# athas/raytracers

Hardware: AMD Instinct MI355X
Metric: Mray/s (primary+secondary) on rgbbox & irreg 1000x1000 (higher is better)
Workload: dtype f32

## Files before the change

include/rt_mi355x.h:

```cpp
#ifndef RT_MI355X_H
#define RT_MI355X_H

#include <stdint.h>

#ifdef __cplusplus
extern "C" {
#endif

typedef struct rt_context rt_context;
typedef struct rt_scene rt_scene;
typedef struct rt_prepared rt_prepared;

enum {
  RT_VARIANT_AUTO = 0,
  RT_VARIANT_PIXEL = 1,
  RT_VARIANT_PERSISTENT = 2,
  RT_VARIANT_POOLED = 3
};

int rt_context_create(rt_context **out, int device, void *hip_stream, int use_caller_stream);
int rt_device_count(void);
int rt_context_create_multi(rt_context **out, const int *devices, int ndev);
int rt_context_num_devices(const rt_context *ctx);
const char *rt_context_gather_mode(rt_context *ctx);
int rt_context_rccl_ranks(rt_context *ctx);
void rt_context_destroy(rt_context *ctx);
const char *rt_last_error(const rt_context *ctx);
const char *rt_context_last_launch(const rt_context *ctx);
int rt_context_entry_counts(rt_context *ctx, uint64_t *lists, uint64_t *fallbacks, int64_t *waves, uint64_t *per_wave, int64_t cap_waves);
int rt_context_entry_info(rt_context *ctx, int32_t *colour_lds, int32_t *flags_const, uint64_t *tables_built, uint64_t *tables_kept);
int rt_context_sync(rt_context *ctx);
int rt_context_set_variant(rt_context *ctx, int variant);
int rt_context_set_option(rt_context *ctx, const char *name, int64_t value);
int rt_context_device_info(const rt_context *ctx, int *device, int *num_cu, int *lds_bytes, char *name, int name_len);

int rt_scene_rgbbox(rt_context *ctx, rt_scene **out);
int rt_scene_irreg(rt_context *ctx, rt_scene **out);
int rt_scene_floor(rt_context *ctx, rt_scene **out, int n, float k);
int rt_scene_from_spheres(rt_context *ctx, rt_scene **out, const float *spheres7, int64_t n,
                          const float look_from[3], const float look_at[3], float fov);
int64_t rt_scene_num_spheres(const rt_scene *scene);
int rt_scene_free(rt_context *ctx, rt_scene *scene);

int rt_prepare_scene(rt_context *ctx, rt_prepared **out, int64_t h, int64_t w, const rt_scene *scene);
int rt_prepared_free(rt_context *ctx, rt_prepared *ps);
int64_t rt_prepared_num_spheres(const rt_prepared *ps);
int32_t rt_prepared_height(const rt_prepared *ps);
int rt_prepared_get_bvh(rt_context *ctx, const rt_prepared *ps, float *L7, float *bmin, float *bmax,
                        int32_t *left, int32_t *right, int32_t *parent);
int rt_prepared_get_camera(rt_context *ctx, const rt_prepared *ps, float cam12[12]);

int rt_prepare_scene_device(rt_context *ctx, rt_prepared **out, int64_t h, int64_t w, const float *spheres7_dev, int64_t n,
                            const float look_from[3], const float look_at[3], float fov);
int rt_prepared_update_spheres(rt_context *ctx, rt_prepared *ps, const float *spheres7_dev, int64_t n);

int rt_render(rt_context *ctx, const rt_prepared *ps, int64_t h, int64_t w, int32_t *out_dev);
int rt_render_part(rt_context *ctx, const rt_prepared *ps, int64_t h, int64_t w, int32_t max_depth,
                   int32_t rows_per_tile, int32_t part, int32_t nparts, int32_t *out_dev);
int rt_render_image(rt_context *ctx, const rt_prepared *objs, int64_t width, int64_t height, const float cam12[12],
                    int32_t max_depth, int32_t rows_per_tile, int32_t part, int32_t nparts, int32_t *out_dev);
int rt_render_batch(rt_context *ctx, const rt_prepared *ps, int64_t h, int64_t w, int32_t max_depth, int32_t rows_per_tile,
                    int32_t part, int32_t nparts, int32_t nframes, const float *cams12, int64_t frame_stride, int32_t *out_dev);
int rt_render_part_inplace(rt_context *ctx, const rt_prepared *ps, int64_t h, int64_t w, int32_t max_depth, int32_t rows_per_tile,
                           int32_t part, int32_t nparts, int32_t nframes, const float *cams12, int64_t frame_stride,
                           int32_t *image_dev);
int rt_ipc_export(rt_context *ctx, void *dev, unsigned char handle64[64]);
int rt_ipc_import(rt_context *ctx, const unsigned char handle64[64], void **out_dev);
int rt_ipc_close(rt_context *ctx, void *imported_dev);
int64_t rt_part_rows(int64_t h, int32_t rows_per_tile, int32_t part, int32_t nparts);
int rt_place_part(rt_context *ctx, int64_t h, int64_t w, int32_t rows_per_tile, int32_t part, int32_t nparts,
                  const int32_t *part_dev, int32_t *image_dev);

int rt_place_parts(rt_context *ctx, int64_t h, int64_t w, int32_t rows_per_tile, int32_t nparts, int64_t pad_rows,
                   const int32_t *stacked_dev, int32_t *image_dev);
int rt_place_parts_strided(rt_context *ctx, int64_t h, int64_t w, int32_t rows_per_tile, int32_t nparts,
                           int64_t part_stride, const int32_t *stacked_dev, int32_t *image_dev);

int rt_place_parts_batch(rt_context *ctx, int64_t h, int64_t w, int32_t rows_per_tile, int32_t nparts, int64_t part_stride,
                         int32_t nframes, int64_t frame_stride_in, int64_t frame_stride_out, const int32_t *stacked_dev,
                         int32_t *images_dev);

int rt_render_stats(rt_context *ctx, const rt_prepared *ps, int64_t h, int64_t w, int32_t max_depth,
                    uint64_t stats3[3]);

int rt_render_trace(rt_context *ctx, const rt_prepared *ps, int64_t h, int64_t w, int32_t max_depth,
                    uint64_t *records, int32_t max_waves, int32_t *num_waves);

int rt_render_timed(rt_context *ctx, const rt_prepared *ps, int64_t h, int64_t w, int32_t max_depth,
                    int32_t rows_per_tile, int32_t part, int32_t nparts, int32_t *out_dev,
                    int32_t warmup, int32_t iters, float *ms_out);

int rt_trace_rays(rt_context *ctx, const rt_prepared *ps, int64_t n, const float *rays_dev, int32_t max_depth,
                  float *colour3_dev, int32_t *pixel_dev);
int rt_intersect_rays(rt_context *ctx, const rt_prepared *ps, int64_t n, const float *rays_dev, float t_min, float t_max,
                      int32_t *index_dev, float *hit7_dev);
int rt_occluded_rays(rt_context *ctx, const rt_prepared *ps, int64_t n, const float *rays_dev, float t_min, float t_max,
                     uint8_t *occluded_dev);
int rt_intersect_rays_ranged(rt_context *ctx, const rt_prepared *ps, int64_t n, const float *rays_dev, const float *t_min_dev,
                             const float *t_max_dev, int32_t *index_dev, float *hit7_dev);
int rt_occluded_rays_ranged(rt_context *ctx, const rt_prepared *ps, int64_t n, const float *rays_dev, const float *t_min_dev,
                            const float *t_max_dev, uint8_t *occluded_dev);
int rt_multi_hit_rays(rt_context *ctx, const rt_prepared *ps, int64_t n, const float *rays_dev, float t_min, float t_max,
                      int32_t k, int32_t *count_dev, int32_t *index_dev, uint8_t *root_dev, float *hit7_dev);
int rt_multi_hit_rays_ranged(rt_context *ctx, const rt_prepared *ps, int64_t n, const float *rays_dev,
                             const float *t_min_dev, const float *t_max_dev, int32_t k,
                             int32_t *count_dev, int32_t *index_dev, uint8_t *root_dev, float *hit7_dev);
int rt_sweep_spheres(rt_context *ctx, const rt_prepared *ps, int64_t n, const float *rays_dev, float radius, float t_min, float t_max,
                     int32_t k, int32_t *count_dev, int32_t *index_dev, uint8_t *start_dev, float *hit7_dev);
int rt_sweep_spheres_ranged(rt_context *ctx, const rt_prepared *ps, int64_t n, const float *rays_dev, const float *radius_dev,
                            const float *t_min_dev, const float *t_max_dev, const int32_t *exclude_dev, int32_t k,
                            int32_t *count_dev, int32_t *index_dev, uint8_t *start_dev, float *hit7_dev);
enum { RT_PATH_ESCAPED = 0, RT_PATH_ABSORBED = 1, RT_PATH_TRUNCATED = 2 };
int rt_trace_paths(rt_context *ctx, const rt_prepared *ps, int64_t n, const float *rays_dev, int32_t max_depth, int32_t k,
// ... 55 lines not shown
```

raytracers_amd/_lib.py:

```python
import ctypes as C
import os

HERE = os.path.dirname(os.path.abspath(__file__))
LIB_NAME = "libray_mi355x.so"
LIB_PATH = os.path.join(HERE, LIB_NAME)

RT_SYMBOLS = [
    "rt_context_create", "rt_device_count", "rt_context_create_multi", "rt_context_num_devices", "rt_context_gather_mode", "rt_context_rccl_ranks",
    "rt_context_destroy", "rt_last_error", "rt_context_last_launch", "rt_context_entry_counts", "rt_context_entry_info", "rt_context_sync", "rt_context_set_variant",
    "rt_context_set_option", "rt_context_device_info",
    "rt_scene_rgbbox", "rt_scene_irreg", "rt_scene_floor", "rt_scene_from_spheres", "rt_scene_num_spheres",
    "rt_scene_free",
    "rt_prepare_scene", "rt_prepared_free", "rt_prepared_num_spheres", "rt_prepared_height", "rt_prepared_get_bvh",
    "rt_prepared_get_camera", "rt_prepare_scene_device", "rt_prepared_update_spheres",
    "rt_render", "rt_render_part", "rt_render_image", "rt_render_batch", "rt_render_part_inplace", "rt_ipc_export", "rt_ipc_import", "rt_ipc_close", "rt_part_rows", "rt_place_part", "rt_place_parts", "rt_place_parts_strided", "rt_place_parts_batch", "rt_render_stats", "rt_render_trace",
    "rt_render_timed",
    "rt_trace_rays", "rt_intersect_rays", "rt_occluded_rays", "rt_intersect_rays_ranged", "rt_occluded_rays_ranged",
    "rt_multi_hit_rays", "rt_multi_hit_rays_ranged", "rt_sweep_spheres", "rt_sweep_spheres_ranged", "rt_trace_paths", "rt_trace_paths_shaped", "rt_nearest_spheres", "rt_nearest_spheres_ranged", "rt_prepared_get_sphere_ids",
    "rt_spheres_within_count", "rt_spheres_within_fill", "rt_contact_pairs_count", "rt_contact_pairs_fill", "rt_contact_clusters",
    "rt_spheres_in_boxes_count", "rt_spheres_in_boxes_fill",
    "rt_spheres_in_planes_count", "rt_spheres_in_planes_fill",
    "rt_spheres_along_rays_count", "rt_spheres_along_rays_fill",
    "rt_visible_pairs", "rt_visible_pairs_shaped",
    "rt_camera_rays",
    "rt_device_alloc", "rt_device_free", "rt_copy_to_host", "rt_copy_to_device",
]
FUTHARK_SYMBOLS = [
    "futhark_context_config_new", "futhark_context_config_free", "futhark_context_config_set_debugging",
    "futhark_context_config_set_logging", "futhark_context_config_set_profiling",
    "futhark_context_config_set_device", "futhark_context_config_set_num_threads", "futhark_context_config_set_cache_file",
    "futhark_context_new", "futhark_context_free", "futhark_context_get_error", "futhark_context_sync",
    "futhark_context_report", "futhark_context_clear_caches", "futhark_context_pause_profiling",
    "futhark_context_unpause_profiling",
    "futhark_entry_rgbbox", "futhark_entry_irreg", "futhark_entry_prepare_scene", "futhark_entry_render",
    "futhark_values_i32_2d", "futhark_free_i32_2d", "futhark_shape_i32_2d", "futhark_new_i32_2d", "futhark_values_raw_i32_2d",
    "futhark_free_opaque_prepared_scene", "futhark_free_opaque_scene",
]


def _load():
    try:
        import torch
    except ImportError:
        pass
    if not os.path.exists(LIB_PATH):
        raise ImportError(
            f"{LIB_PATH} is missing: build the HIP library first (`make` at the repo root, or "
            "`python -c 'import __graft_entry__ as g; g.build()'`). raytracers_amd has no CPU fallback.")
    lib = C.CDLL(LIB_PATH, mode=C.RTLD_GLOBAL)
    vp, i32, i64 = C.c_void_p, C.c_int32, C.c_int64
    pf = C.POINTER(C.c_float)
    sig = {
        "rt_context_create": (C.c_int, [C.POINTER(vp), C.c_int, vp, C.c_int]),
        "rt_device_count": (C.c_int, []),
        "rt_context_create_multi": (C.c_int, [C.POINTER(vp), C.POINTER(C.c_int), C.c_int]),
        "rt_context_num_devices": (C.c_int, [vp]),
        "rt_context_gather_mode": (C.c_char_p, [vp]),
        "rt_context_rccl_ranks": (C.c_int, [vp]),
        "rt_context_destroy": (None, [vp]),
        "rt_last_error": (C.c_char_p, [vp]),
        "rt_context_last_launch": (C.c_char_p, [vp]),
        "rt_context_entry_counts": (C.c_int, [vp, C.POINTER(C.c_uint64), C.POINTER(C.c_uint64), C.POINTER(i64), C.POINTER(C.c_uint64), i64]),
        "rt_context_entry_info": (C.c_int, [vp, C.POINTER(i32), C.POINTER(i32), C.POINTER(C.c_uint64), C.POINTER(C.c_uint64)]),
        "rt_context_sync": (C.c_int, [vp]),
        "rt_context_set_variant": (C.c_int, [vp, C.c_int]),
        "rt_context_set_option": (C.c_int, [vp, C.c_char_p, i64]),
        "rt_context_device_info": (C.c_int, [vp, C.POINTER(C.c_int), C.POINTER(C.c_int), C.POINTER(C.c_int),
                                             C.c_char_p, C.c_int]),
        "rt_scene_rgbbox": (C.c_int, [vp, C.POINTER(vp)]),
        "rt_scene_irreg": (C.c_int, [vp, C.POINTER(vp)]),
        "rt_scene_floor": (C.c_int, [vp, C.POINTER(vp), C.c_int, C.c_float]),
        "rt_scene_from_spheres": (C.c_int, [vp, C.POINTER(vp), vp, i64, pf, pf, C.c_float]),
        "rt_scene_num_spheres": (i64, [vp]),
        "rt_scene_free": (C.c_int, [vp, vp]),
        "rt_prepare_scene": (C.c_int, [vp, C.POINTER(vp), i64, i64, vp]),
        "rt_prepared_free": (C.c_int, [vp, vp]),
        "rt_prepared_num_spheres": (i64, [vp]),
        "rt_prepared_height": (i32, [vp]),
        "rt_prepared_get_bvh": (C.c_int, [vp, vp, vp, vp, vp, vp, vp, vp]),
        "rt_prepared_get_camera": (C.c_int, [vp, vp, vp]),
        "rt_prepare_scene_device": (C.c_int, [vp, C.POINTER(vp), i64, i64, vp, i64, pf, pf, C.c_float]),
        "rt_prepared_update_spheres": (C.c_int, [vp, vp, vp, i64]),
        "rt_render": (C.c_int, [vp, vp, i64, i64, vp]),
        "rt_render_part": (C.c_int, [vp, vp, i64, i64, i32, i32, i32, i32, vp]),
        "rt_render_image": (C.c_int, [vp, vp, i64, i64, vp, i32, i32, i32, i32, vp]),
        "rt_render_batch": (C.c_int, [vp, vp, i64, i64, i32, i32, i32, i32, i32, vp, i64, vp]),
        "rt_render_part_inplace": (C.c_int, [vp, vp, i64, i64, i32, i32, i32, i32, i32, vp, i64, vp]),
        "rt_ipc_export": (C.c_int, [vp, vp, vp]),
        "rt_ipc_import": (C.c_int, [vp, vp, C.POINTER(vp)]),
        "rt_ipc_close": (C.c_int, [vp, vp]),
        "rt_part_rows": (i64, [i64, i32, i32, i32]),
        "rt_place_part": (C.c_int, [vp, i64, i64, i32, i32, i32, vp, vp]),
        "rt_place_parts": (C.c_int, [vp, i64, i64, i32, i32, i64, vp, vp]),
        "rt_place_parts_strided": (C.c_int, [vp, i64, i64, i32, i32, i64, vp, vp]),
        "rt_place_parts_batch": (C.c_int, [vp, i64, i64, i32, i32, i64, i32, i64, i64, vp, vp]),
        "rt_render_stats": (C.c_int, [vp, vp, i64, i64, i32, vp]),
        "rt_render_trace": (C.c_int, [vp, vp, i64, i64, i32, vp, i32, C.POINTER(i32)]),
        "rt_render_timed": (C.c_int, [vp, vp, i64, i64, i32, i32, i32, i32, vp, i32, i32, vp]),
        "rt_device_alloc": (C.c_int, [vp, C.POINTER(vp), i64]),
        "rt_device_free": (C.c_int, [vp, vp]),
        "rt_copy_to_host": (C.c_int, [vp, vp, vp, i64]),
        "rt_copy_to_device": (C.c_int, [vp, vp, vp, i64]),
        "rt_trace_rays": (C.c_int, [vp, vp, i64, vp, i32, vp, vp]),
        "rt_intersect_rays": (C.c_int, [vp, vp, i64, vp, C.c_float, C.c_float, vp, vp]),
        "rt_occluded_rays": (C.c_int, [vp, vp, i64, vp, C.c_float, C.c_float, vp]),
        "rt_intersect_rays_ranged": (C.c_int, [vp, vp, i64, vp, vp, vp, vp, vp]),
        "rt_occluded_rays_ranged": (C.c_int, [vp, vp, i64, vp, vp, vp, vp]),
        "rt_multi_hit_rays": (C.c_int, [vp, vp, i64, vp, C.c_float, C.c_float, i32, vp, vp, vp, vp]),
        "rt_multi_hit_rays_ranged": (C.c_int, [vp, vp, i64, vp, vp, vp, i32, vp, vp, vp, vp]),
        "rt_sweep_spheres": (C.c_int, [vp, vp, i64, vp, C.c_float, C.c_float, C.c_float, i32, vp, vp, vp, vp]),
        "rt_sweep_spheres_ranged": (C.c_int, [vp, vp, i64, vp, vp, vp, vp, vp, i32, vp, vp, vp, vp]),
        "rt_trace_paths": (C.c_int, [vp, vp, i64, vp, i32, i32, vp, vp, vp, vp, vp, vp, vp]),
        "rt_trace_paths_shaped": (C.c_int, [vp, vp, i64, vp, i32, i32, vp, vp, vp, vp, vp, vp, vp, i32]),
        "rt_nearest_spheres": (C.c_int, [vp, vp, i64, vp, C.c_float, i32, vp, vp, vp]),
        "rt_nearest_spheres_ranged": (C.c_int, [vp, vp, i64, vp, vp, i32, vp, vp, vp]),
        "rt_prepared_get_sphere_ids": (C.c_int, [vp, vp, vp]),
        "rt_spheres_within_count": (C.c_int, [vp, vp, i64, vp, C.c_float, vp, vp, vp]),
        "rt_spheres_within_fill": (C.c_int, [vp, vp, i64, vp, C.c_float, vp, vp, vp, i64, vp, vp, vp]),
        "rt_contact_pairs_count": (C.c_int, [vp, vp, C.c_float, vp]),
        "rt_contact_pairs_fill": (C.c_int, [vp, vp, C.c_float, vp, i64, vp, vp]),
        "rt_contact_clusters": (C.c_int, [vp, vp, C.c_float, vp, vp, vp, vp]),
        "rt_spheres_in_boxes_count": (C.c_int, [vp, vp, i64, vp, C.c_float, vp, vp, vp]),
        "rt_spheres_in_boxes_fill": (C.c_int, [vp, vp, i64, vp, C.c_float, vp, vp, vp, i64, vp, vp, vp]),
        "rt_spheres_in_planes_count": (C.c_int, [vp, vp, i64, vp, C.c_int32, C.c_float, vp, vp, vp]),
        "rt_spheres_in_planes_fill": (C.c_int, [vp, vp, i64, vp, C.c_int32, C.c_float, vp, vp, vp, i64, vp, vp, vp]),
        "rt_spheres_along_rays_count": (C.c_int, [vp, vp, i64, vp, C.c_float, vp, C.c_float, C.c_float, vp, vp, vp, vp, vp]),
        "rt_spheres_along_rays_fill": (C.c_int, [vp, vp, i64, vp, C.c_float, vp, C.c_float, C.c_float, vp, vp, vp, vp, vp, i64, vp, vp, vp, vp]),
        "rt_visible_pairs": (C.c_int, [vp, vp, i64, vp, i64, vp, i32, C.c_float, C.c_float, vp, vp]),
        "rt_visible_pairs_shaped": (C.c_int, [vp, vp, i64, vp, i64, vp, i32, C.c_float, C.c_float, vp, vp, i32]),
        "rt_camera_rays": (C.c_int, [vp, vp, i64, i64, vp, vp]),
    }
    for name, (res, args) in sig.items():
        fn = getattr(lib, name)
        fn.restype = res
        fn.argtypes = args
    return lib


lib = _load()
```

raytracers_amd/api.py:

```python
import ctypes as C

import numpy as np

from ._lib import lib

VARIANT_AUTO, VARIANT_PIXEL, VARIANT_PERSISTENT, VARIANT_POOLED = 0, 1, 2, 3
MAX_DEPTH = 50
PATH_ESCAPED, PATH_ABSORBED, PATH_TRUNCATED = 0, 1, 2
PAIRS_TARGETS, PAIRS_DIRECTIONS = 0, 1
ROWS_PER_TILE = 8


class RtError(RuntimeError):
    pass


class Context:

    def __init__(self, device=-1, stream=None, devices=None):
        h = C.c_void_p()
        if devices is not None:
            arr = (C.c_int * len(devices))(*[int(d) for d in devices])
            rc = lib.rt_context_create_multi(C.byref(h), arr, len(devices))
        else:
            rc = lib.rt_context_create(C.byref(h), int(device), C.c_void_p(stream or 0), 0 if stream is None else 1)
        if rc != 0 or not h.value:
            raise RtError(f"rt_context_create failed (code {rc}): no usable HIP device; "
                          "raytracers_amd has no CPU fallback")
        self._h = h

    def _check(self, rc):
        if rc != 0:
            raise RtError(lib.rt_last_error(self._h).decode() or f"error code {rc}")

    def close(self):
        if getattr(self, "_h", None):
            lib.rt_context_destroy(self._h)
            self._h = None

    def __del__(self):
        try:
            self.close()
        except Exception:
            pass

    def sync(self):
        self._check(lib.rt_context_sync(self._h))

    @property
    def num_devices(self):
        return int(lib.rt_context_num_devices(self._h))

    @property
    def gather_mode(self):
        return lib.rt_context_gather_mode(self._h).decode()

    @property
    def last_launch(self):
        return lib.rt_context_last_launch(self._h).decode()

    def entry_counts(self):
        lists, falls, nw = C.c_uint64(), C.c_uint64(), C.c_int64()
        self._check(lib.rt_context_entry_counts(self._h, C.byref(lists), C.byref(falls), C.byref(nw), None, 0))
        per = np.zeros((nw.value, 2), np.uint64)
        if nw.value:
            self._check(lib.rt_context_entry_counts(self._h, None, None, None, per.ctypes.data_as(C.POINTER(C.c_uint64)), nw.value))
        return {"lists": lists.value, "fallbacks": falls.value, "waves": nw.value, "per_wave": per}

    def entry_info(self):
        col, const, built, kept = C.c_int32(), C.c_int32(), C.c_uint64(), C.c_uint64()
        self._check(lib.rt_context_entry_info(self._h, C.byref(col), C.byref(const), C.byref(built), C.byref(kept)))
        return {"colour_lds": bool(col.value), "flags_const": bool(const.value), "tables_built": built.value, "tables_kept": kept.value}

    @property
    def rccl_ranks(self):
        return int(lib.rt_context_rccl_ranks(self._h))

    def set_variant(self, v):
        self._check(lib.rt_context_set_variant(self._h, int(v)))

    def set_option(self, name, value):
        self._check(lib.rt_context_set_option(self._h, name.encode(), int(value)))

    def device_info(self):
        dev, cus, lds = C.c_int(), C.c_int(), C.c_int()
        name = C.create_string_buffer(64)
        self._check(lib.rt_context_device_info(self._h, C.byref(dev), C.byref(cus), C.byref(lds), name, 64))
        return {"device": dev.value, "num_cu": cus.value, "lds_bytes": lds.value, "arch": name.value.decode()}

    def _scene(self, fn, *args):
        h = C.c_void_p()
        self._check(fn(self._h, C.byref(h), *args))
        return Scene(self, h)

    def rgbbox(self):
        return self._scene(lib.rt_scene_rgbbox)

    def irreg(self):
        return self._scene(lib.rt_scene_irreg)

    def floor(self, n, k):
        return self._scene(lib.rt_scene_floor, int(n), float(k))

    def scene(self, name):
        if name == "rgbbox":
            return self.rgbbox()
        if name == "irreg":
            return self.irreg()
        if name == "big":
            return self.floor(1000, 6000.0)
        raise ValueError(f"unknown scene {name!r}")

    def scene_from_spheres(self, spheres7, look_from, look_at, fov):
        s = np.ascontiguousarray(spheres7, dtype=np.float32)
        if s.ndim != 2 or s.shape[1] != 7:
            raise ValueError("spheres7 must be (n, 7): pos.xyz, colour.rgb, radius")
        lf = (C.c_float * 3)(*look_from)
        la = (C.c_float * 3)(*look_at)
        h = C.c_void_p()
        self._check(lib.rt_scene_from_spheres(self._h, C.byref(h), s.ctypes.data, s.shape[0], lf, la, float(fov)))
        return Scene(self, h)

    def alloc_i32(self, count):
        return DeviceBuffer(self, int(count) * 4)


class DeviceBuffer:
    def __init__(self, ctx, nbytes):
        self.ctx, self.nbytes = ctx, nbytes
        p = C.c_void_p()
        ctx._check(lib.rt_device_alloc(ctx._h, C.byref(p), nbytes))
        self.ptr = p.value

    def as_torch(self, shape):
        import torch
        n = int(np.prod(shape))
        assert n * 4 <= self.nbytes
        iface = {"shape": tuple(int(x) for x in shape), "typestr": "<i4", "data": (int(self.ptr), False), "version": 2}
        holder = type("_CudaArray", (), {"__cuda_array_interface__": iface})()
        return torch.as_tensor(holder, device=torch.device("cuda", self.ctx.device_info()["device"]))

    def to_host(self, shape, dtype=np.int32):
        out = np.empty(shape, dtype=dtype)
        assert out.nbytes <= self.nbytes
        self.ctx._check(lib.rt_copy_to_host(self.ctx._h, out.ctypes.data, self.ptr, out.nbytes))
        return out

    def free(self):
        if self.ptr and self.ctx._h:
            lib.rt_device_free(self.ctx._h, self.ptr)
        self.ptr = None

    def __del__(self):
        try:
            self.free()
# ... 846 lines not shown
```

raytracers_amd/csrc/api.cpp:

```cpp
#include <hip/hip_runtime.h>

#include <algorithm>
#include <chrono>
#include <cmath>
#include <cstdio>
#include <cstdlib>
#include <cstring>
#include <memory>
#include <string>
#include <vector>

#include "../../include/rt_mi355x.h"
#include "rt_device.hpp"
#include "rt_host.hpp"
#include "rt_internal.hpp"

namespace rti {
int fail(rt_context *ctx, const std::string &msg) {
  if (ctx) ctx->err = msg;
  return 1;
}
int hip_fail(rt_context *ctx, hipError_t e, const char *what) {
  return fail(ctx, std::string(what) + ": " + hipGetErrorString(e));
}
// ... 367 lines not shown
    v->sort_inflight_px = false;
  }
  return true;
}
void drain_streams(rt_context *ctx) {
  (void)hipStreamSynchronize(ctx->stream);
  if (ctx->sort_stream) (void)hipStreamSynchronize(ctx->sort_stream);
  if (ctx->sort_stream_px) (void)hipStreamSynchronize(ctx->sort_stream_px);
}

int ensure_spill(rt_context *ctx, int stride) {
  const size_t need = sizeof(unsigned) * static_cast<size_t>(stride) * static_cast<size_t>(std::max(1, ctx->num_cu)) * 20;
  if (ctx->spill_bytes >= need) return 0;
  drain_streams(ctx);
  if (ctx->spill_dev) (void)hipFree(ctx->spill_dev);
  ctx->spill_dev = nullptr; ctx->spill_bytes = 0;
  RT_HIP(ctx, hipMalloc(reinterpret_cast<void **>(&ctx->spill_dev), need));
  ctx->spill_bytes = need;
  return 0;
}

bool rt_scene_exceeds_l2(const rt_prepared *ps) { return static_cast<int64_t>(ps->n) * 80 > (int64_t(32) << 20); }

void set_cull(const rt_context *ctx, const rt_prepared *ps, const Plan &pl, const float *cams_dev, rtk::KParams *p) {
  if (ctx->cull == 0 || !ps->cull.ok || pl.variant != RT_VARIANT_POOLED || (pl.waves != 16 && pl.waves != 4)) return;
  if (ctx->cull < 0 && pl.lds_nodes == p->n_nodes && pl.lds_sph == p->n_sph) return;
  if (cams_dev == nullptr ? !rt::cull_origin_ok(ps->cull, &p->cam.ox) : (cams_dev != ctx->cams_dev || ctx->cams_host == nullptr)) return;
  for (int f = 0; cams_dev != nullptr && f < p->nframes; ++f)
    if (!rt::cull_origin_ok(ps->cull, ctx->cams_host + 12 * f)) return;
  p->cull = 1;
  p->cull_c2 = ps->cull.c2;
  p->cull_kappa = ps->cull.kappa;
}

void set_dark(const rt_context *ctx, bool instrumented, rtk::KParams *p) {
  p->dark = (ctx->dark_stop != 0 && p->cost == nullptr && (!instrumented || ctx->dark_stop > 0)) ? 1 : 0;
}

void set_leaf_box(const rt_context *ctx, const rt_prepared *ps, const Plan &pl, const float *cams_dev, bool instrumented, rtk::KParams *p) {
  p->leaf_box = 0;
  if (ctx->leaf_box == 0 || !ps->leaf.ok || pl.variant != RT_VARIANT_POOLED || (instrumented && ctx->leaf_box <= 0)) return;
  if (pl.lds_nodes != p->n_nodes || pl.lds_sph != p->n_sph) return;
  if (cams_dev == nullptr ? !rt::leaf_box_camera_ok(ps->leaf, &p->cam.ox) : (cams_dev != ctx->cams_dev || ctx->cams_host == nullptr)) return;
  for (int f = 0; cams_dev != nullptr && f < p->nframes; ++f)
    if (!rt::leaf_box_camera_ok(ps->leaf, ctx->cams_host + 12 * f)) return;
  rtk::PooledKey k{};
  if (!rtk::choose_pooled(*p, instrumented, pl.waves, 0, &k) || !rtk::pooled_leaf_box(k)) return;
  p->leaf_box = 1;
}

int set_entry(rt_context *ctx, const Plan &pl, TileOrder *to, rtk::KParams *p, int *entry, bool *build) {
  p->entry = nullptr;
  *entry = 0;
  *build = false;
  rtk::PooledKey k{};
  if (ctx->entry_lists == 0 || pl.variant != RT_VARIANT_POOLED || p->n_nodes < 1 || !rtk::choose_pooled(*p, false, pl.waves, 0, &k) || !rtk::pooled_entry_ok(k)) return 0;
  if (ctx->entry_lists < 0 && p->nparts > 1 && p->rpt_log2 < 3) return 0;
  if (ctx->entry_lists < 0 && (ctx->leaf_box == 0 || ctx->dark_stop == 0)) return 0;
  if (p->cams != nullptr && (p->order != nullptr || !(p->nshards == 1 || p->interleave))) return 0;
  *entry = rtk::pooled_entry_bits(rtk::kEntryLists, p->leaf_box, p->dark, rtk::pooled_col_lds_bytes(p->n_nodes, p->n_sph, p->capb, p->capl, p->ray_planes),
                                  static_cast<size_t>(std::min(ctx->lds_bytes, 160 * 1024)), ctx->col_lds != 0);
  const int filter = p->leaf_box != 0 && rtk::pooled_leaf_box(k) ? 1 : 0;
  if (to != nullptr && to->entry != nullptr && p->cams == nullptr && ctx->entry_keep != 0 && (to->entry_ctx == nullptr || to->entry_ctx == ctx)) {
    *build = !(to->entry_valid && to->entry_filter == filter);
    to->entry_valid = false;
    to->entry_filter = filter;
    to->entry_ctx = ctx;
    p->entry = to->entry;
    return 0;
  }
  *build = true;
  const size_t need = sizeof(unsigned) * rtk::kEntryDw * static_cast<size_t>(p->cams != nullptr ? p->nframes : 1) * static_cast<size_t>(p->nchunks);
  if (ctx->entry_bytes < need) {
    drain_streams(ctx);
    pool_free(ctx, reinterpret_cast<char *>(ctx->entry_dev), ctx->entry_bytes);
    ctx->entry_dev = nullptr; ctx->entry_bytes = 0;
    char *blk = nullptr;
    size_t bytes = need;
    RT_HIP(ctx, pool_alloc(ctx, &blk, &bytes));
    ctx->entry_dev = reinterpret_cast<unsigned *>(blk);
    ctx->entry_bytes = bytes;
  }
  p->entry = ctx->entry_dev;
  return 0;
}

std::string pooled_launch_name(const rtk::KParams &p, int waves, int rays = 0) {
  rtk::PooledKey k{};
  return rtk::choose_pooled(p, false, waves, rays, &k) ? rtk::pooled_name(k) : "none";
}
const char *pooled_launch_nodes(const rtk::KParams &p, int waves) {
  rtk::PooledKey k{};
  return rtk::choose_pooled(p, false, waves, 0, &k) && rtk::pooled_presort(k) ? "sign-ordered" : "planes";
}

void frame_params(const rt_prepared *ps, int64_t h, int64_t w, int rows_per_tile, int part, int nparts, int max_depth, const float *cam12, rtk::KParams *p) {
  scene_params(ps, p);
  std::memcpy(&p->cam, cam12 ? static_cast<const void *>(cam12) : static_cast<const void *>(&ps->cam), sizeof(p->cam));
  p->w = static_cast<int>(w); p->h = static_cast<int>(h);
  p->rows_local = static_cast<int>(rt::part_rows(h, rows_per_tile, part, nparts));
  p->rows_per_tile = rows_per_tile; p->part = part; p->nparts = nparts;
  p->rpt_log2 = (rows_per_tile & (rows_per_tile - 1)) == 0 ? __builtin_ctz(rows_per_tile) : -1;
  p->tiles_x = (p->w + 7) / 8;
  p->tiles_y = (p->rows_local + 7) / 8;
  p->max_depth = max_depth;
  p->nframes = 1;
}

bool twenty_waves(const rt_context *ctx, const Plan &pl) { return pl.waves * (pl.grid_full / std::max(1, ctx->num_cu)) == 20; }

int pooled_shape_params(rt_context *ctx, const rt_prepared *ps, const Plan &pl, rtk::KParams *p) {
  p->static_first = ctx->static_first;
  p->lds_nodes = pl.lds_nodes; p->lds_sph = pl.lds_sph;
  p->smax = pl.smax; p->lmax = pl.lmax;
  p->thr_shade = ctx->thr_shade; p->thr_leaf = ctx->thr_leaf;
  p->capb = pl.capb; p->capl = pl.capl; p->ray_planes = pl.ray_planes;
  if (pl.spill_stride > 0) {
    if (int rc = ensure_spill(ctx, pl.spill_stride)) return rc;
    p->spill = ctx->spill_dev;
    p->spill_stride = pl.spill_stride;
  }
  p->prio_depth = ctx->prio_depth;
  p->box2 = ctx->box2;
  p->look_max = ctx->look_max > 0 ? ctx->look_max : (twenty_waves(ctx, pl) ? 16 : (p->nframes > 1 || p->nchunks > 16384) ? 32 : 64);
  p->tl_log2 = ps->tl_depth;
  return 0;
}

int xcd_rule(const rt_context *ctx, const rt_prepared *ps, const Plan &pl, int nframes) {
  if (ctx->xcd_queues >= 0) return ctx->xcd_queues;
  return nframes == 1 && pl.variant == RT_VARIANT_POOLED && twenty_waves(ctx, pl) && rt_scene_exceeds_l2(ps) ? 1 : 2;
}
void set_counters(rtk::KParams *p, int xq, int grid) {
  p->nshards = xq && (p->nframes == 1 || xq == 2) && grid % rtk::kMaxShards == 0 ? rtk::kMaxShards : 1;
  p->interleave = p->nshards > 1 && xq == 2;
}
int order_shards(const rtk::KParams &p) { return p.interleave ? 1 : p.nshards; }
bool counters_follow(rtk::KParams *p, int xq, int grid) {
  const int ns = p->nshards, il = p->interleave, shards = order_shards(*p);
  set_counters(p, xq, grid);
  if (order_shards(*p) == shards) return true;
  p->nshards = ns;
  p->interleave = il;
  return false;
}

bool px_static_ok(const rt_context *ctx, const rtk::KParams &p, const Plan &pl) {
  return ctx->pixel_order == 2 ||
         (ctx->pixel_order == 1 && ctx->deep_class < 0 && p.max_depth > 4 && pl.waves == 16 && ctx->adaptive_order == 1 && p.nchunks <= ctx->px_max_tiles &&
          (p.nchunks >= 1024 || (pl.lds_nodes == p.n_nodes && pl.lds_sph == p.n_sph)));
}
bool px_list_launch(const rt_context *ctx, const rtk::KParams &p, const Plan &pl, const TileOrder *v) {
  return v && v->valid && v->px_valid && p.nframes == 1 && pl.waves == 16 && ctx->adaptive_order == 1 && (p.nshards == 1 || p.interleave) &&
         v->px_elems >= static_cast<size_t>(p.rows_local) * p.w && px_static_ok(ctx, p, pl);
}

bool same_shape(const TileOrder &o, const rtk::KParams &p) {
  return o.h == p.h && o.w == p.w && o.rows_per_tile == p.rows_per_tile && o.part == p.part && o.nparts == p.nparts && o.max_depth == p.max_depth &&
         o.ntiles == p.nchunks && o.nshards == order_shards(p);
}

int find_view(rt_context *ctx, const rt_prepared *ps, const rtk::KParams &p, const Plan &pl, TileOrder **out) {
  TileOrder *to = nullptr;
  for (auto &o : ps->orders)
    if (same_shape(o, p) && std::memcmp(o.cam, &p.cam, sizeof o.cam) == 0) to = &o;
  if (!to) {
// ... 221 lines not shown
  bool stream_was_idle = ctx->synced_since_render;
  ctx->synced_since_render = false;
  if (!stream_was_idle && ctx->eager_sort && nframes == 1) {
    stream_was_idle = hipStreamQuery(ctx->stream) == hipSuccess;
    (void)hipGetLastError();
  }
  rtk::KParams p{};
  frame_params(ps, h, w, rows_per_tile, part, nparts, max_depth, cam12, &p);
  p.out = out_dev;
  p.stats = ctx->stats_dev;
  if (p.rows_local == 0) {
    ctx->last_launch = "family=none (no rows)";
    return 0;
  }
  const int64_t frame_elems = inplace ? h * w : static_cast<int64_t>(p.rows_local) * p.w;
  if (nframes < 1 || (nframes > 1 && (frame_stride < frame_elems || frame_stride * nframes >= (int64_t(1) << 31))))
    return fail(ctx, "bad batch: nframes >= 1, frame_stride >= rows * w (in place: h * w), nframes * frame_stride < 2^31");
  if (rti::tiles_of(p.rows_local, w) * nframes >= rti::kMaxPositions)
    return fail(ctx, "bad batch: tiles per frame x frames < 2^26 (a frame has ceil(rows / 8) x ceil(w / 8) tiles of 8 x 8 pixels)");
  if (inplace) {
    p.out = out_dev + static_cast<int64_t>(part) * rows_per_tile * w;
    p.out_skip = static_cast<int>(static_cast<int64_t>(nparts - 1) * rows_per_tile * w);
  }
  if (max_depth == 0) return clear_frames(ctx, p, out_dev, nframes, frame_stride, inplace);
  Ticks tick;
  Plan pl{};
  if (stats) pl.variant = RT_VARIANT_PIXEL;
  else {
    const int64_t ntiles1 = static_cast<int64_t>((w + 7) / 8) * ((p.rows_local + 7) / 8);
    const bool huge = rt_scene_exceeds_l2(ps);
    const bool wide = ctx->wide_waves == 2 || (ctx->wide_waves == 1 && ntiles1 * nframes >= (huge ? 40000 : 100000) && (nframes > 1 || ntiles1 > ctx->px_max_tiles));
    if (int rc = make_plan(ctx, ps, &pl, ntiles1 * nframes, 0, wide)) return rc;
  }
  tick("plan");
  if (nframes > 1 && pl.variant != RT_VARIANT_POOLED) {
    std::vector<float> hc;
    if (cams_dev) {
      hc.resize(static_cast<size_t>(nframes) * 12);
      RT_HIP(ctx, hipMemcpyAsync(hc.data(), cams_dev, hc.size() * 4, hipMemcpyDeviceToHost, ctx->stream));
      RT_HIP(ctx, hipStreamSynchronize(ctx->stream));
    }
    for (int f = 0; f < nframes; ++f)
      if (int rc = enqueue_render(ctx, ps, h, w, max_depth, rows_per_tile, part, nparts, out_dev + f * frame_stride, stats,
                                  cams_dev ? hc.data() + 12 * f : cam12, 1, 0, nullptr, inplace))
        return rc;
    return 0;
  }
  if (pl.variant == RT_VARIANT_PIXEL) {
    RT_HIP(ctx, rtk::launch_pixel(p, stats, ctx->stream));
    ctx->last_launch = stats ? "family=pixel (instrumented)" : "family=pixel";
    return 0;
  }
  p.nframes = nframes;
  p.frame_stride = static_cast<int>(frame_stride);
  p.cams = reinterpret_cast<const rtk::Cam *>(cams_dev);
  p.queue = ctx->queue_dev;
  p.nchunks = p.tiles_x * p.tiles_y;
  const int64_t tiles_per_wave = static_cast<int64_t>(p.nchunks) * nframes / std::max(1, pl.grid * pl.waves);
  p.tpt_log2 = ctx->tpt_log2 >= 0 ? ctx->tpt_log2 : (nframes > 1 ? (tiles_per_wave >= 48 && !twenty_waves(ctx, pl) ? 2 : tiles_per_wave >= 24 ? 1 : 0) : 0);
  const int xq = xcd_rule(ctx, ps, pl, nframes);
  set_counters(&p, pl.variant == RT_VARIANT_POOLED ? xq : 0, pl.grid);
  if (int rc = pooled_shape_params(ctx, ps, pl, &p)) return rc;
  p.solo = ctx->solo;
  if (pl.variant != RT_VARIANT_POOLED) {
    RT_HIP(ctx, rtk::launch_persistent(p, false, pl.grid, pl.waves, ctx->stream));
    ctx->last_launch = "family=persistent";
    return 0;
  }
  if (ps->n >= (int64_t(1) << 22)) return fail(ctx, "pooled kernel: at most 2^22 spheres (work items and hit keys carry the leaf index in 22 bits)");
  if (p.rpt_log2 < 0) return fail(ctx, "pooled kernel: rows_per_tile must be a power of two");
  if (int rc = get_uv(ctx, w, h, &p.u_tab, &p.v_tab)) return rc;
  tick("uv tables");
  TileOrder *to = nullptr;
  if (ctx->adaptive_order && !p.cams)
    if (int rc = find_view(ctx, ps, p, pl, &to)) return rc;
  Tickets t;
  if (int rc = choose_tickets(ctx, ps, to, xq, tick, p, pl, &t)) return rc;
  set_cull(ctx, ps, pl, cams_dev, &p);
  set_dark(ctx, false, &p);
  set_leaf_box(ctx, ps, pl, cams_dev, false, &p);
  int entry = 0;
  bool build_entry = false;
  if (int rc = set_entry(ctx, pl, to, &p, &entry, &build_entry)) return rc;
  if (p.entry) {
    if (build_entry) {
      RT_HIP(ctx, rtk::launch_tile_entry(p, false, pl.waves, ctx->stream));
      ctx->entry_tables_built++;
    } else {
      ctx->entry_tables_kept++;
    }
    if (to != nullptr && p.entry == to->entry) to->entry_valid = true;
    if (ctx->entry_count) {
      const size_t nw = static_cast<size_t>(pl.grid) * static_cast<size_t>(pl.waves), bytes = nw * 2 * sizeof(unsigned long long);
      if (ctx->entry_counts_bytes < bytes) {
        drain_streams(ctx);
        if (ctx->entry_counts_dev) (void)hipFree(ctx->entry_counts_dev);
        ctx->entry_counts_dev = nullptr; ctx->entry_counts_bytes = 0;
        RT_HIP(ctx, hipMalloc(reinterpret_cast<void **>(&ctx->entry_counts_dev), bytes));
        ctx->entry_counts_bytes = bytes;
      }
      RT_HIP(ctx, hipMemsetAsync(ctx->entry_counts_dev, 0, bytes, ctx->stream));
      p.trace = ctx->entry_counts_dev;
      entry = (entry & ~rtk::kEntryModeMask) | rtk::kEntryCount;
    }
  }
  ctx->entry_counts_waves = (entry & rtk::kEntryModeMask) == rtk::kEntryCount ? static_cast<int64_t>(pl.grid) * pl.waves : 0;
  ctx->last_entry = entry;
  tick("before launch");
  RT_HIP(ctx, rtk::launch_pooled(p, false, pl.grid, pl.waves, ctx->stream, 0, entry));
  tick("launch_pooled");
  char buf[352];
  std::snprintf(buf, sizeof buf, "family=pooled tickets=%s%s instantiation=%s frames=%d tiles=%d grid=%d waves=%d counters=%d%s deep_class=%d deep_split=%d recording=%d nodes=%s,entry=%s,dark=%d,leaf_box=%d",
                p.px_hdr ? "pixel-list" : t.first_order ? "tiles-bit-reversed" : (p.order ? "tiles-ordered" : "tiles-raster"), t.borrowed ? "(borrowed)" : "",
                pooled_launch_name(p, pl.waves).c_str(), p.nframes, p.nchunks, pl.grid, pl.waves, p.nshards, p.interleave ? "(turns)" : "", p.px_hdr ? 0 : p.deep_class,
                p.px_hdr ? 0 : p.deep_split, p.cost ? (p.cost_px ? 2 : 1) : 0, pooled_launch_nodes(p, pl.waves), p.entry ? "lists" : "root", p.dark, p.leaf_box);
  ctx->last_launch = buf;
  if (to && p.cost) {
    to->sort_pending = true;
    to->sort_px = p.cost_px != nullptr;
    to->rec_out_skip = p.out_skip;
    if (ctx->eager_sort && (stream_was_idle || ctx->sync_policy))
      if (int rc = sort_view(ctx, ps, to, p, pl)) return rc;
    tick("record: eager sorts");
  }
  return 0;
}
using rti::enqueue_render;

extern "C" void rt_context_destroy(rt_context *ctx);

extern "C" int rt_context_create(rt_context **out, int device, void *hip_stream, int use_caller_stream) {
  if (!out) return 1;
  *out = nullptr;
  auto ctx = std::make_unique<rt_context>();
  int count = 0;
  hipError_t e = hipGetDeviceCount(&count);
  if (e != hipSuccess || count <= 0) {
    std::fprintf(stderr, "libray_mi355x: no usable HIP device (%s); this library has no CPU path\n",
                 e == hipSuccess ? "device count is 0" : hipGetErrorString(e));
    return 2;
  }
  if (device < 0) {
    if (hipGetDevice(&device) != hipSuccess) device = 0;
  }
  if (device >= count) return 3;
  if (hipSetDevice(device) != hipSuccess) return 4;
  ctx->device = device;
  hipDeviceProp_t prop;
  if (hipGetDeviceProperties(&prop, device) != hipSuccess) return 5;
  auto bail = [&](int code) {
    rt_context_destroy(ctx.release());
    return code;
  };
  ctx->num_cu = prop.multiProcessorCount;
  ctx->lds_bytes = static_cast<int>(prop.maxSharedMemoryPerMultiProcessor ? prop.maxSharedMemoryPerMultiProcessor
                                                                           : prop.sharedMemPerBlock);
  ctx->name = prop.gcnArchName;
  if (use_caller_stream) {
    ctx->stream = static_cast<hipStream_t>(hip_stream);
  } else {
    if (hipStreamCreateWithFlags(&ctx->stream, hipStreamNonBlocking) != hipSuccess) return bail(6);
    ctx->own_stream = true;
  }
  if (hipMalloc(reinterpret_cast<void **>(&ctx->queue_dev), sizeof(unsigned) * rtk::kQueueDwords) != hipSuccess) return bail(7);
  if (hipMemset(ctx->queue_dev, 0, sizeof(unsigned) * rtk::kQueueDwords) != hipSuccess) return bail(7);
  if (hipMalloc(reinterpret_cast<void **>(&ctx->stats_dev), 256) != hipSuccess) return bail(7);
  if (hipMemset(ctx->stats_dev, 0, 256) != hipSuccess) return bail(7);
  if (hipStreamSynchronize(nullptr) != hipSuccess) return bail(7);
  if (hipMalloc(reinterpret_cast<void **>(&ctx->arena), kArenaGranules * kGranule) != hipSuccess) return bail(7);
  ctx->arena_used.assign(kArenaGranules, 0);
  if (hipHostMalloc(reinterpret_cast<void **>(&ctx->pinned), rtk::gpu_build_pinned_bytes(), hipHostMallocDefault) != hipSuccess)
    return bail(7);
  if (hipHostMalloc(reinterpret_cast<void **>(&ctx->stage), kStageBytes, hipHostMallocDefault) != hipSuccess) return bail(7);
  if (hipStreamCreateWithFlags(&ctx->sort_stream, hipStreamNonBlocking) != hipSuccess) return bail(6);
  if (hipStreamCreateWithFlags(&ctx->sort_stream_px, hipStreamNonBlocking) != hipSuccess) return bail(6);
  if (hipEventCreateWithFlags(&ctx->rec_event, hipEventDisableTiming) != hipSuccess) return bail(6);
  if (hipMalloc(reinterpret_cast<void **>(&ctx->order_scratch), sizeof(int) * rtk::kOrderScratchInts) != hipSuccess) return bail(7);
  if (hipMalloc(reinterpret_cast<void **>(&ctx->px_scratch), sizeof(int) * rtk::px_scratch_ints()) != hipSuccess) return bail(7);
  if (hipHostMalloc(reinterpret_cast<void **>(&ctx->class_slab), sizeof(int) * kClassSlotInts * kClassSlots * kClassChunks, hipHostMallocDefault) != hipSuccess) return bail(7);
  rtk::warm_render_kernels();
  rtk::warm_build_kernels();
  if (rtk::warm_scratch(ctx->stream, ctx->order_scratch) != hipSuccess) return bail(6);
  if (const char *v = std::getenv("RT_VARIANT")) ctx->variant = std::atoi(v);
  if (const char *v = std::getenv("RT_XCD_QUEUES")) ctx->xcd_queues = std::max(-1, std::min(2, std::atoi(v)));
  if (const char *v = std::getenv("RT_TPT_LOG2")) ctx->tpt_log2 = std::max(-1, std::min(4, std::atoi(v)));
  if (const char *v = std::getenv("RT_STATIC_FIRST")) ctx->static_first = std::atoi(v) != 0;
  *out = ctx.release();
  return 0;
}

extern "C" void rt_context_destroy(rt_context *ctx) {
  if (!ctx) return;
  if (ctx->group) rti::group_destroy(ctx);
  (void)hipSetDevice(ctx->device);
  drain_streams(ctx);
  if (ctx->sort_stream) (void)hipStreamDestroy(ctx->sort_stream);
  if (ctx->sort_stream_px) (void)hipStreamDestroy(ctx->sort_stream_px);
  if (ctx->rec_event) (void)hipEventDestroy(ctx->rec_event);
  for (auto &t : ctx->uv) pool_free(ctx, reinterpret_cast<char *>(t.u), t.bytes);
  for (auto &t : ctx->first_orders) pool_free(ctx, reinterpret_cast<char *>(t.order), t.bytes);
  if (ctx->class_slab) (void)hipHostFree(ctx->class_slab);
  if (ctx->cams_dev) (void)hipFree(ctx->cams_dev);
  if (ctx->cams_host) (void)hipHostFree(ctx->cams_host);
  if (ctx->cams_event) (void)hipEventDestroy(ctx->cams_event);
  if (ctx->queue_dev) (void)hipFree(ctx->queue_dev);
  if (ctx->spill_dev) (void)hipFree(ctx->spill_dev);
  pool_free(ctx, reinterpret_cast<char *>(ctx->entry_dev), ctx->entry_bytes);
  if (ctx->entry_counts_dev) (void)hipFree(ctx->entry_counts_dev);
  if (ctx->order_scratch) (void)hipFree(ctx->order_scratch);
  if (ctx->px_scratch) (void)hipFree(ctx->px_scratch);
  if (ctx->within_scratch) (void)hipFree(ctx->within_scratch);
  if (ctx->stats_dev) (void)hipFree(ctx->stats_dev);
  for (auto &b : ctx->pool) (void)hipFree(b.p);
  if (ctx->arena) (void)hipFree(ctx->arena);
  if (ctx->pinned) (void)hipHostFree(ctx->pinned);
  if (ctx->stage) (void)hipHostFree(ctx->stage);
  if (ctx->own_stream) (void)hipStreamDestroy(ctx->stream);
  delete ctx;
}

extern "C" int rt_device_count(void) {
  int n = 0;
  return hipGetDeviceCount(&n) == hipSuccess ? n : 0;
}

extern "C" const char *rt_last_error(const rt_context *ctx) { return ctx ? ctx->err.c_str() : "null context"; }
extern "C" int rt_context_entry_counts(rt_context *ctx, uint64_t *lists, uint64_t *fallbacks, int64_t *waves, uint64_t *per_wave, int64_t cap_waves) {
  if (!ctx) return 1;
  RT_LOCK(ctx);
  RT_HIP(ctx, hipSetDevice(ctx->device));
  RT_HIP(ctx, hipStreamSynchronize(ctx->stream));
  const int64_t nw = ctx->entry_counts_waves;
  std::vector<unsigned long long> h(static_cast<size_t>(nw) * 2);
  if (nw > 0) RT_HIP(ctx, hipMemcpy(h.data(), ctx->entry_counts_dev, h.size() * sizeof(unsigned long long), hipMemcpyDeviceToHost));
  uint64_t l = 0, f = 0;
  for (int64_t i = 0; i < nw; ++i) {
    l += h[2 * i]; f += h[2 * i + 1];
    if (per_wave && i < cap_waves) { per_wave[2 * i] = h[2 * i]; per_wave[2 * i + 1] = h[2 * i + 1]; }
  }
  if (lists) *lists = l;
  if (fallbacks) *fallbacks = f;
  if (waves) *waves = nw;
  return 0;
}

extern "C" int rt_context_entry_info(rt_context *ctx, int32_t *colour_lds, int32_t *flags_const, uint64_t *tables_built, uint64_t *tables_kept) {
  if (!ctx) return 1;
  RT_LOCK(ctx);
  if (colour_lds) *colour_lds = (ctx->last_entry & rtk::kEntryColLds) != 0;
  if (flags_const) *flags_const = ctx->last_entry != 0 && (ctx->last_entry & rtk::kEntryRtFlags) == 0;
  if (tables_built) *tables_built = ctx->entry_tables_built;
  if (tables_kept) *tables_kept = ctx->entry_tables_kept;
  return 0;
}

extern "C" const char *rt_context_last_launch(const rt_context *ctx) { return ctx ? ctx->last_launch.c_str() : ""; }

extern "C" int rt_context_sync(rt_context *ctx) {
  RT_LOCK(ctx);
  if (!ctx) return 1;
  if (ctx->group) {
    const int grc = rti::group_sync(ctx);
    if (!grc) rti::group_mark_synced(ctx);
    return grc;
  }
  const auto t0 = std::chrono::steady_clock::now();
  hipError_t q;
  for (;;) {
    q = hipStreamQuery(ctx->stream);
    if (q != hipErrorNotReady) break;
    if (std::chrono::steady_clock::now() - t0 > std::chrono::microseconds(800)) {
      q = hipStreamSynchronize(ctx->stream);
      break;
    }
  }
  if (q == hipSuccess) {
    ctx->synced_since_render = true;
    return 0;
  }
  (void)hipGetLastError();
  (void)hipMemset(ctx->queue_dev, 0, sizeof(unsigned) * rtk::kQueueDwords);
  return hip_fail(ctx, q, "stream synchronisation (the ticket counters were reset)");
}

extern "C" int rt_context_set_variant(rt_context *ctx, int variant) {
  RT_LOCK(ctx);
  if (!ctx) return 1;
  if (variant < RT_VARIANT_AUTO || variant > RT_VARIANT_POOLED) return fail(ctx, "unknown variant");
  ctx->variant = variant;
  if (ctx->group) return rti::group_set_variant(ctx, variant);
  return 0;
}

extern "C" int rt_context_set_option(rt_context *ctx, const char *name, int64_t value) {
  RT_LOCK(ctx);
  if (!ctx || !name) return 1;
  if (ctx->group) {
    const int grc = rti::group_set_option(ctx, name, value);
    if (grc >= 0) return grc;
  }
  const std::string k(name);
  const int v = static_cast<int>(value);
  if (k == "waves_per_wg") {
    if (v != 0 && v != 4 && v != 8 && v != 12 && v != 16) return fail(ctx, "waves_per_wg must be 0 (auto), 4, 8, 12 or 16");
    ctx->waves_per_wg = v;
  } else if (k == "wgs_per_cu") {
    if (v < 1 || v > 8) return fail(ctx, "wgs_per_cu must be 1..8");
    ctx->wgs_per_cu = v;
  } else if (k == "thr_shade") {
    ctx->thr_shade = std::max(1, std::min(64, v));
  } else if (k == "thr_leaf") {
    ctx->thr_leaf = std::max(1, std::min(64, v));
  } else if (k == "lmax") {
    if (v < 2 || v > 32) return fail(ctx, "lmax must be 2..32");
    ctx->lmax = v;
  } else if (k == "lds_scene_bytes") {
    ctx->lds_scene_bytes = v;
  } else if (k == "lds_sph_first") {
    ctx->lds_sph_first = v != 0;
  } else if (k == "grid_div") {
    ctx->grid_div = std::max(0, std::min(64, v));
  } else if (k == "prio_depth") {
    ctx->prio_depth = std::max(0, v);
  } else if (k == "gpu_build") {
    ctx->gpu_build = v != 0;
  } else if (k == "adaptive_order") {
    ctx->adaptive_order = v;
  } else if (k == "box2") {
    ctx->box2 = v != 0;
  } else if (k == "look_max") {
    ctx->look_max = std::max(0, std::min(64, v));
  } else if (k == "handover") {
    ctx->handover = std::max(0, std::min(2, v));
  } else if (k == "donate_max") {
    ctx->donate_max = std::max(1, std::min(64, v));
  } else if (k == "solo") {
    ctx->solo = v != 0;
  } else if (k == "treelet") {
    if (v < 1 || v > rtk::kTreeletMaxDepth) return fail(ctx, "treelet (host builder: levels per treelet) must be 1 .. 5");
    ctx->treelet = v;
  } else if (k == "trace_part") {
    ctx->trace_part = v;
  } else if (k == "trace_nparts") {
    ctx->trace_nparts = v;
  } else if (k == "trace_solo") {
    ctx->trace_solo = v != 0;
  } else if (k == "ray_planes") {
    if (v != 0 && v != 2 && v != 3) return fail(ctx, "ray_planes must be 0 (auto), 2 or 3");
    ctx->ray_planes = v;
  } else if (k == "deep_class") {
    ctx->deep_class = std::min(8, std::max(-1, v));
  } else if (k == "deep_cap_log2") {
    ctx->deep_cap_log2 = std::min(8, std::max(0, v));
  } else if (k == "deep_split") {
    ctx->deep_split = std::min(6, std::max(0, v));
  } else if (k == "xcd_queues") {
    if (v < -1 || v > 2) return fail(ctx, "xcd_queues must be -1 (auto), 0 (one counter), 1 (a strip of tile columns per counter) or 2 (counters take turns)");
    ctx->xcd_queues = v;
  } else if (k == "tpt_log2") {
    if (v < -1 || v > 4) return fail(ctx, "tpt_log2 must be -1 (auto) or 0..4");
    ctx->tpt_log2 = v;
  } else if (k == "static_first") {
    ctx->static_first = v != 0;
  } else if (k == "first_order") {
    ctx->first_order = v != 0;
  } else if (k == "pixel_order") {
    ctx->pixel_order = std::max(0, std::min(2, v));
  } else if (k == "px_solo" || k == "px_w8" || k == "px_w16" || k == "px_w32") {
    ctx->px_thr[k == "px_solo" ? 0 : k == "px_w8" ? 1 : k == "px_w16" ? 2 : 3] = std::max(0, std::min(255, v));
  } else if (k == "px_g1" || k == "px_g8" || k == "px_g16" || k == "px_g32" || k == "px_g64") {
    ctx->px_g[k == "px_g1" ? 0 : k == "px_g8" ? 1 : k == "px_g16" ? 2 : k == "px_g32" ? 3 : 4] = std::max(0, std::min(100000, v));
  } else if (k == "px_max_tiles") {
    ctx->px_max_tiles = std::max(0, v);
  } else if (k == "px_ray_ns") {
    ctx->px_ray_ns = std::max(0, std::min(100000, v));
  } else if (k == "px_zip") {
    ctx->px_zip = v != 0;
  } else if (k == "px_prio") {
    ctx->px_prio = std::max(0, std::min(3, v));
  } else if (k == "px_hold") {
    ctx->px_hold = v & 0x1f;
  } else if (k == "px_solo_div") {
    ctx->px_solo_div = std::max(1, std::min(4096, v));
  } else if (k == "eager_sort") {
    drain_streams(ctx);
    ctx->eager_sort = v != 0;
  } else if (k == "borrow") {
    ctx->borrow = std::max(0, std::min(4, v));
  } else if (k == "stack_cap") {
    if (v != 0 && v != rtk::kSpillCapbTest) return fail(ctx, "stack_cap must be 0 or 192");
    ctx->stack_cap = v;
  } else if (k == "wide_waves") {
    ctx->wide_waves = std::max(0, std::min(2, v));
  } else if (k == "cull") {
    ctx->cull = std::max(-1, std::min(1, v));
  } else if (k == "dark_stop") {
    ctx->dark_stop = std::max(-1, std::min(1, v));
  } else if (k == "leaf_box") {
    ctx->leaf_box = std::max(-1, std::min(1, v));
  } else if (k == "entry_lists") {
    ctx->entry_lists = std::max(-1, std::min(1, v));
  } else if (k == "entry_count") {
    ctx->entry_count = v != 0;
  } else if (k == "entry_keep") {
    ctx->entry_keep = v == 0 ? 0 : -1;
  } else if (k == "col_lds") {
    ctx->col_lds = v == 0 ? 0 : -1;
  } else if (k == "sync_policy") {
    ctx->sync_policy = v != 0;
  } else {
    return fail(ctx, "unknown option: " + k);
  }
  return 0;
}

extern "C" int rt_context_device_info(const rt_context *ctx, int *device, int *num_cu, int *lds_bytes, char *name,
                                      int name_len) {
  RT_LOCK(const_cast<rt_context *>(ctx));
  if (!ctx) return 1;
  if (device) *device = ctx->device;
  if (num_cu) *num_cu = ctx->num_cu;
  if (lds_bytes) *lds_bytes = ctx->lds_bytes;
  if (name && name_len > 0) {
    std::strncpy(name, ctx->name.c_str(), static_cast<size_t>(name_len) - 1);
    name[name_len - 1] = 0;
  }
  return 0;
}

static int new_scene(rt_context *ctx, rt_scene **out, rt::SceneDesc &&d) {
  RT_LOCK(ctx);
  if (!ctx || !out) return fail(ctx, "null argument");
  auto *s = new rt_scene;
  s->desc = std::move(d);
  *out = s;
  return 0;
}
extern "C" int rt_scene_rgbbox(rt_context *ctx, rt_scene **out) { return new_scene(ctx, out, rt::make_rgbbox()); }
extern "C" int rt_scene_irreg(rt_context *ctx, rt_scene **out) { return new_scene(ctx, out, rt::make_floor(100, 600.0f)); }
extern "C" int rt_scene_floor(rt_context *ctx, rt_scene **out, int n, float k) {
  RT_LOCK(ctx);
  if (n < 2 || n > 4096) return fail(ctx, "floor scene: n out of range (2..4096)");
  return new_scene(ctx, out, rt::make_floor(n, k));
}
extern "C" int rt_scene_from_spheres(rt_context *ctx, rt_scene **out, const float *spheres7, int64_t n,
                                     const float look_from[3], const float look_at[3], float fov) {
  RT_LOCK(ctx);
  if (!spheres7 || !look_from || !look_at) return fail(ctx, "null argument");
  if (n < 2 || n > (int64_t(1) << rtk::kMaxSpheresLog2)) return fail(ctx, "scene needs 2 .. 2^26 spheres");
  rt::SceneDesc d;
  d.spheres.resize(static_cast<size_t>(n));
  std::memcpy(d.spheres.data(), spheres7, sizeof(rt::Sphere) * static_cast<size_t>(n));
  std::copy(look_from, look_from + 3, d.look_from);
  std::copy(look_at, look_at + 3, d.look_at);
  d.fov = fov;
  return new_scene(ctx, out, std::move(d));
}
extern "C" int64_t rt_scene_num_spheres(const rt_scene *scene) {
  return scene ? static_cast<int64_t>(scene->desc.spheres.size()) : 0;
}
extern "C" int rt_scene_free(rt_context *ctx, rt_scene *scene) {
  RT_LOCK(ctx);
  if (scene)
    for (auto &c : scene->copies) {
      (void)hipSetDevice(c.device);
      (void)hipFree(c.p);
    }
  if (ctx) (void)hipSetDevice(ctx->device);
  delete scene;
  return 0;
}

namespace {
hipError_t alloc_prepared_block(rt_context *ctx, rt_prepared *ps) {
  const size_t n = static_cast<size_t>(ps->n), ni = n - 1;
  size_t off = 0;
  auto carve = [&](size_t bytes) { const size_t at = off; off += (bytes + 255) & ~size_t(255); return at; };
  const size_t o_L7 = carve(n * 28), o_bmin = carve(ni * 12), o_bmax = carve(ni * 12), o_left = carve(ni * 4),
               o_right = carve(ni * 4), o_parent = carve(ni * 4), o_nodes = carve(ni * 32), o_nodes64 = carve(ni * 64),
               o_sph = carve(n * 16), o_col = carve(n * 16), o_ids = carve(n * 4);
  ps->block_bytes = off;
  const hipError_t e = pool_alloc(ctx, &ps->block, &ps->block_bytes);
  if (e != hipSuccess) {
    ps->block = nullptr;
// ... 190 lines not shown
    if (ps->leaf.ok) {
      *e = rtk::launch_leaf_boxes(ps->nodes64, ps->sph, static_cast<int>(n) - 1, ps->leaf.q, ps->leaf.lin, ps->leaf.abs, ctx->stream);
      if (*e == hipSuccess) *e = hipStreamSynchronize(ctx->stream);
      if (*e != hipSuccess) return 0;
    }
  } else {
    std::vector<rt::Sphere> host(n);
    *e = hipMemcpyAsync(host.data(), spheres7_dev, n * sizeof(rt::Sphere), hipMemcpyDeviceToHost, ctx->stream);
    if (*e == hipSuccess) *e = hipStreamSynchronize(ctx->stream);
    if (*e != hipSuccess) return 0;
    const rt::CullStats st = rt::cull_stats(host.data(), n);
    ps->leaf = rt::leaf_box_finish(st, n);
    if (int rc = host_build_upload(ctx, ps, host, e)) return rc;
    if (*e != hipSuccess) return 0;
    ps->cull = rt::cull_finish(st, n, 0);
  }
  ps->cull.ok = ps->cull.ok && ps->height <= static_cast<int>(log2f(static_cast<float>(n))) + 2;
  if (ctx->wide_waves != 0 && ps->height > 15 && n < (size_t(1) << 22)) return ensure_spill(ctx, 64 * (ps->height + 2));
  return 0;
}

int device_spheres_ok(rt_context *ctx, const float *spheres7_dev, int64_t n) {
  if (!spheres7_dev) return fail(ctx, "null argument");
  if (n < 2 || n > (int64_t(1) << rtk::kMaxSpheresLog2)) return fail(ctx, "scene needs 2 .. 2^26 spheres");
  if (ctx->group) return fail(ctx, "device spheres: a multi-device context is not supported (use a context on one device)");
  return 0;
}

void reset_views(rt_context *ctx, rt_prepared *ps) {
  drain_streams(ctx);
  for (auto &o : ps->orders) {
    for (hipEvent_t ev : {o.sort_event, o.sort_event_px, o.classes_event})
      if (ev) (void)hipEventSynchronize(ev);
    if (o.block) {
      if (o.block_owner == ctx) pool_free(ctx, o.block, o.block_bytes);
      else if (!o.block_owner) (void)hipFree(o.block);
      o.block = nullptr;
    }
    for (hipEvent_t ev : {o.sort_event, o.sort_event_px, o.classes_event})
      if (ev) (void)hipEventDestroy(ev);
  }
  ps->orders.clear();
}
}

extern "C" int rt_prepare_scene_device(rt_context *ctx, rt_prepared **out, int64_t h, int64_t w, const float *spheres7_dev, int64_t n,
                                       const float look_from[3], const float look_at[3], float fov) {
  RT_LOCK(ctx);
  if (!ctx || !out || !look_from || !look_at) return fail(ctx, "null argument");
  if (int rc = device_spheres_ok(ctx, spheres7_dev, n)) return rc;
  if (h <= 0 || w <= 0) return fail(ctx, "image size must be positive");
  RT_HIP(ctx, hipSetDevice(ctx->device));
  (void)hipGetLastError();
  auto ps = std::make_unique<rt_prepared>();
  ps->n = n;
  ps->home = ctx;
  ps->h = h; ps->w = w;
  rt::SceneDesc d;
  std::copy(look_from, look_from + 3, d.look_from);
  std::copy(look_at, look_at + 3, d.look_at);
  d.fov = fov;
  ps->cam = rt::scene_camera(d, h, w);
  RT_HIP(ctx, alloc_prepared_block(ctx, ps.get()));
  hipError_t e = hipSuccess;
  const int rc = build_from_device(ctx, ps.get(), spheres7_dev, &e);
  if (rc || e != hipSuccess) {
    rt_prepared_free(ctx, ps.release());
    return rc ? rc : hip_fail(ctx, e, "rt_prepare_scene_device");
  }
  *out = ps.release();
  return 0;
}

extern "C" int rt_prepared_update_spheres(rt_context *ctx, rt_prepared *ps, const float *spheres7_dev, int64_t n) {
  RT_LOCK(ctx);
  if (!ctx || !ps) return fail(ctx, "null argument");
  if (int rc = device_spheres_ok(ctx, spheres7_dev, n)) return rc;
  if (ps->home != ctx) return fail(ctx, "rt_prepared_update_spheres: only through the context that prepared the scene");
  if (n != ps->n) return fail(ctx, "rt_prepared_update_spheres: n must equal rt_prepared_num_spheres (" + std::to_string(ps->n) + ")");
  RT_LOCK_PS(ps);
  RT_HIP(ctx, hipSetDevice(ctx->device));
  (void)hipGetLastError();
  reset_views(ctx, ps);
  hipError_t e = hipSuccess;
  if (int rc = build_from_device(ctx, ps, spheres7_dev, &e)) return rc;
  if (e != hipSuccess) return hip_fail(ctx, e, "rt_prepared_update_spheres");
  return 0;
}

extern "C" int64_t rt_prepared_num_spheres(const rt_prepared *ps) { return ps ? ps->n : 0; }
extern "C" int32_t rt_prepared_height(const rt_prepared *ps) { return ps ? ps->height : 0; }

extern "C" int rt_prepared_get_bvh(rt_context *ctx, const rt_prepared *ps, float *L7, float *bmin, float *bmax,
                                   int32_t *left, int32_t *right, int32_t *parent) {
  RT_LOCK(ctx);
  if (!ctx || !ps) return fail(ctx, "null argument");
  RT_HIP(ctx, hipSetDevice(ctx->device));
  RT_HIP(ctx, hipStreamSynchronize(ctx->stream));
  const size_t n = static_cast<size_t>(ps->n), ni = n - 1;
  if (L7) RT_HIP(ctx, hipMemcpy(L7, ps->L7, n * 28, hipMemcpyDeviceToHost));
  if (bmin) RT_HIP(ctx, hipMemcpy(bmin, ps->bmin, ni * 12, hipMemcpyDeviceToHost));
  if (bmax) RT_HIP(ctx, hipMemcpy(bmax, ps->bmax, ni * 12, hipMemcpyDeviceToHost));
  if (left) RT_HIP(ctx, hipMemcpy(left, ps->left, ni * 4, hipMemcpyDeviceToHost));
  if (right) RT_HIP(ctx, hipMemcpy(right, ps->right, ni * 4, hipMemcpyDeviceToHost));
  if (parent) RT_HIP(ctx, hipMemcpy(parent, ps->parent, ni * 4, hipMemcpyDeviceToHost));
  return 0;
}

extern "C" int rt_prepared_get_camera(rt_context *ctx, const rt_prepared *ps, float cam12[12]) {
  RT_LOCK(ctx);
  if (!ctx || !ps || !cam12) return fail(ctx, "null argument");
  std::memcpy(cam12, &ps->cam, sizeof(rt::Camera));
  return 0;
}

static int render_entry(rt_context *ctx, const rt_prepared *ps, int64_t h, int64_t w, int32_t max_depth, int32_t rows_per_tile,
                        int32_t part, int32_t nparts, int32_t *out_dev, const float *cam12) {
  RT_LOCK(ctx);
  if (ctx && ctx->group) {
    if (!ps) return fail(ctx, "null prepared scene");
    if (part != 0 || nparts != 1) return fail(ctx, "a multi-device context renders whole frames: it partitions them itself");
    if (max_depth < 0) return fail(ctx, "negative max_depth");
    return rti::group_render(ctx, ps, h, w, max_depth, out_dev, cam12);
  }
  return enqueue_render(ctx, ps, h, w, max_depth, rows_per_tile, part, nparts, out_dev, false, cam12);
}

extern "C" int rt_render(rt_context *ctx, const rt_prepared *ps, int64_t h, int64_t w, int32_t *out_dev) {
  return render_entry(ctx, ps, h, w, 50, 8, 0, 1, out_dev, nullptr);
}

extern "C" int rt_render_part(rt_context *ctx, const rt_prepared *ps, int64_t h, int64_t w, int32_t max_depth,
                              int32_t rows_per_tile, int32_t part, int32_t nparts, int32_t *out_dev) {
  return render_entry(ctx, ps, h, w, max_depth, rows_per_tile, part, nparts, out_dev, nullptr);
}

extern "C" int rt_render_image(rt_context *ctx, const rt_prepared *objs, int64_t width, int64_t height, const float cam12[12],
                               int32_t max_depth, int32_t rows_per_tile, int32_t part, int32_t nparts, int32_t *out_dev) {
  return render_entry(ctx, objs, height, width, max_depth, rows_per_tile, part, nparts, out_dev, cam12);
}

int rti::stage_cams(rt_context *ctx, const float *cams12, int32_t nframes, const float **cams_dev) {
  RT_LOCK(ctx);
  *cams_dev = nullptr;
  if (!cams12) return 0;
  RT_HIP(ctx, hipSetDevice(ctx->device));
  const size_t bytes = sizeof(float) * 12 * static_cast<size_t>(nframes);
  if (bytes > ctx->cams_bytes) {
    RT_HIP(ctx, hipStreamSynchronize(ctx->stream));
    if (ctx->cams_dev) (void)hipFree(ctx->cams_dev);
    if (ctx->cams_host) (void)hipHostFree(ctx->cams_host);
    ctx->cams_dev = nullptr;
    ctx->cams_host = nullptr;
    ctx->cams_bytes = 0;
    ctx->cams_event_valid = false;
    RT_HIP(ctx, hipMalloc(reinterpret_cast<void **>(&ctx->cams_dev), bytes));
    RT_HIP(ctx, hipHostMalloc(reinterpret_cast<void **>(&ctx->cams_host), bytes, hipHostMallocDefault));
    ctx->cams_bytes = bytes;
  } else if (ctx->cams_event_valid) {
    RT_HIP(ctx, hipEventSynchronize(ctx->cams_event));
  }
  std::memcpy(ctx->cams_host, cams12, bytes);
  RT_HIP(ctx, hipMemcpyAsync(ctx->cams_dev, ctx->cams_host, bytes, hipMemcpyHostToDevice, ctx->stream));
  if (!ctx->cams_event) RT_HIP(ctx, hipEventCreateWithFlags(&ctx->cams_event, hipEventDisableTiming));
  RT_HIP(ctx, hipEventRecord(ctx->cams_event, ctx->stream));
  ctx->cams_event_valid = true;
// ... 276 lines not shown
```

raytracers_amd/csrc/lane_core.h:

```cpp
#pragma once
#include <math.h>
#include <stdint.h>

#if defined(__HIPCC__)
#define RT_HD __host__ __device__ __forceinline__
#else
#define RT_HD inline
#endif

namespace rtk {

constexpr float kTMax = 1000000000.0f;
constexpr float kEps = 0.1f;
constexpr float kNoHit = __builtin_inff();

struct Cam {
  float ox, oy, oz, lx, ly, lz, hx, hy, hz, vx, vy, vz;
};

struct Ray {
  float ox, oy, oz;
  float dx, dy, dz;
  float ix, iy, iz;
  float a;
// ... 263 lines not shown
      const float d = k == 0 ? q[j].dx : k == 1 ? q[j].dy : q[j].dz;
      const float i = 1.0f / d;
      pos = pos & (d > 0.0f) & (i > 0.0f) & (i < kNoHit);
      neg = neg & (d < 0.0f) & (i < 0.0f) & (i > -kNoHit);
      lo = j == 0 || i < lo ? i : lo;
      hi = j == 0 || i > hi ? i : hi;
    }
    if (MUT != 3) ok = ok & (pos | neg);
    t->imin[k] = lo; t->imax[k] = hi;
  }
  return ok;
}

template <int MUT = 0>
RT_HD int tile_verdict(const TileRays &t, const float lo[3], const float hi[3]) {
  float tmin_lo = 0.0f, tmin_hi = 0.0f, tmax_lo = kTMax, tmax_hi = kTMax;
  for (int k = 0; k < 3; ++k) {
    const bool neg = t.imax[k] < 0.0f;
    const float cn = (neg ? hi[k] : lo[k]) - t.o[k], cf = (neg ? lo[k] : hi[k]) - t.o[k];
    const float na = cn * t.imin[k], nb = cn * t.imax[k], fa = cf * t.imin[k], fb = cf * t.imax[k];
    tmin_lo = fmaxf(na < nb ? na : nb, tmin_lo);
    tmin_hi = fmaxf(na < nb ? nb : na, tmin_hi);
    tmax_lo = fminf(fa < fb ? fa : fb, tmax_lo);
    tmax_hi = fminf(fa < fb ? fb : fa, tmax_hi);
  }
  if (tmax_lo > tmin_hi) return kTileAllHit;
  if (MUT == 1 ? tmax_hi < tmin_lo : tmax_hi <= tmin_lo) return kTileAllMiss;
  return kTileMixed;
}

template <int MUT, int MAXI, int MAXL>
RT_HD bool tile_frontier(const TileRays &t, const float root_lo[3], const float root_hi[3], const float *nodes64, int n_nodes, bool filter,
                         int *inner, int *n_inner, int *leaf, int *n_leaf) {
  *n_inner = 0; *n_leaf = 0;
  if (n_nodes < 1 || tile_verdict<MUT>(t, root_lo, root_hi) != kTileAllHit) return false;
  int stack[kEntryStack], sp = 0, ni = 0, nl = 0;
  stack[sp++] = 0;
  while (sp > 0) {
    const int node = stack[--sp];
    const float *const rec = nodes64 + 16 * (size_t)node;
    int child[2], verdict[2];
    bool uniform = true;
    for (int s = 0; s < 2; ++s) {
      int32_t w;
      __builtin_memcpy(&w, rec + 4 * s + 3, 4);
      child[s] = w >> 8;
      verdict[s] = tile_verdict<MUT>(t, rec + 8 * s, rec + 8 * s + 4);
      if (child[s] < 0 && !filter) verdict[s] = kTileAllHit;
      uniform = uniform & (verdict[s] != kTileMixed);
    }
    if (!uniform) {
      if (node == 0 || ni >= MAXI) return false;
      inner[ni++] = node;
      continue;
    }
    for (int s = 0; s < 2; ++s) {
      if (verdict[s] != kTileAllHit) continue;
      if (child[s] < 0) {
        if (nl >= MAXL) return false;
        leaf[nl++] = ~child[s];
      } else {
        if (sp >= kEntryStack) return false;
        stack[sp++] = child[s];
      }
    }
  }
  *n_inner = ni; *n_leaf = nl;
  return true;
}

template <int MUT = 0>
RT_HD void tile_entry(const TileRays &t, bool rays_ok, const float root_lo[3], const float root_hi[3], const float *nodes64, int n_nodes, bool filter,
                      int ref_shift, int node_mul, uint32_t out[kEntryDw]) {
  int inner[1], leaf[kEntryLeaves], ni = 0, nl = 0;
  const bool ok = rays_ok && tile_frontier<MUT, 1, kEntryLeaves>(t, root_lo, root_hi, nodes64, n_nodes, filter, inner, &ni, leaf, &nl);
  for (int i = 0; i < kEntryDw; ++i) out[i] = 0u;
  if (!ok) return;
  out[0] = kEntryValid | (ni ? kEntryInner : 0u) | (uint32_t)nl << kEntryCountShift;
  if (ni) out[1] = (uint32_t)(inner[0] * node_mul) << ref_shift;
  for (int i = 0; i < kEntryLeaves; ++i)
    if (i < nl) out[2 + i] = (uint32_t)~leaf[i] << ref_shift;
}

}
```

raytracers_amd/csrc/render_kernels.hip:

```cpp
#include <hip/hip_runtime.h>

#include <mutex>
#include <type_traits>
#include <utility>

#include "lane_core.h"
#include "rt_device.hpp"
#include "treelet.h"

#ifdef RT_ISA_MARKS
#define RT_MARK(name) asm volatile("; RT_MARK " name)
#else
#define RT_MARK(name)
#endif

namespace rtk {

__device__ __forceinline__ int global_row(const KParams &p, int lrow) {
  const int k = lrow / p.rows_per_tile;
  return (k * p.nparts + p.part) * p.rows_per_tile + (lrow - k * p.rows_per_tile);
}

__device__ __forceinline__ size_t out_index(const KParams &p, int lrow, int col) {
  return (size_t)lrow * p.w + col + (size_t)(lrow / p.rows_per_tile) * (size_t)p.out_skip;
// ... 381 lines not shown
            q3 = buf_load16(rs_nodes, ni16 * 4 + 48);
          }
          const int cl8 = f2i(q0.w), cr8 = f2i(q1.w);
          const unsigned ml = (unsigned)f2i(q2.w), mr = (unsigned)f2i(q3.w);
          const float limc = CULL ? cull_limit(__uint_as_float(lds_load4(key_lds + 4u)), w2, cull_kappa) : kTMax;
          const unsigned long long m_hl = bal(box_hit_clamped(r, q0.x, q0.y, q0.z, q1.x, q1.y, q1.z, limc));
          const unsigned long long m_hr = bal(box_hit_clamped(r, q2.x, q2.y, q2.z, q3.x, q3.y, q3.z, limc));
          const bool reach = has && tl_reached(ml, mr, pos, (unsigned)(m_hl >> gsh), (unsigned)(m_hr >> gsh));
          const unsigned long long m_reach = bal(reach), m_exit = m_reach & bal(tl_frontier(ml));
          const unsigned long long m_ln = bal(cl8 < 0), m_rn = bal(cr8 < 0);
          const unsigned long long m_inl = m_exit & ~m_ln & m_hl, m_inr = m_exit & ~m_rn & m_hr;
          const unsigned long long m_lfl = m_reach & m_ln, m_lfr = m_reach & m_rn;
          const int c_inl = __popcll(m_inl), c_lfl = __popcll(m_lfl);
          const int b_box = (int)box_lds + 4 * nbox, b_leaf = (int)leaf_lds + 4 * nleaf, dump = (int)dump_lds;
          const int a_l = sel_mask(m_lfl, sel_mask(m_inl, dump, b_box + 4 * lane_rank(m_inl)), b_leaf + 4 * lane_rank(m_lfl));
          const int a_r = sel_mask(m_lfr, sel_mask(m_inr, dump, b_box + 4 * lane_rank_from(m_inr, c_inl)),
                                   b_leaf + 4 * lane_rank_from(m_lfr, c_lfl));
          lds_store(a_l, (unsigned)cl8);
          lds_store(a_r, (unsigned)cr8);
          nbox = uni(nbox + c_inl + __popcll(m_inr));
          nleaf = uni(nleaf + c_lfl + __popcll(m_lfr));
          if (TRACE) { __builtin_amdgcn_s_waitcnt(0); tc_tre += clock64() - tc_op; tn_tre++; }
        }
      }
      __builtin_amdgcn_fence(__ATOMIC_ACQ_REL, "wavefront");
      key = *key_ptr;
    }
    const float best = __uint_as_float((unsigned)(key >> 32));
    const bool hit = key != kKeyInit;
    const int wj = hit ? (int)((unsigned)key >> 1) : 0;
    float4 c, s;
    const unsigned long long m_win = bal(hit && cand_j == wj);
    if (m_win != 0ull) {
      const int src = uni((int)__builtin_ctzll(m_win));
      auto rl = [&](float v) { return __int_as_float(__builtin_amdgcn_readlane(__float_as_int(v), src)); };
      s = make_float4(rl(cand_s.x), rl(cand_s.y), rl(cand_s.z), rl(cand_s.w));
      c = make_float4(rl(cand_c.x), rl(cand_c.y), rl(cand_c.z), rl(cand_c.w));
    } else {
      c = buf_load16(rs_col, wj * 16);
      s = lds_load16(sph_lds + 16u * (unsigned)(wj < lds_sph ? wj : 0));
      if (wj >= lds_sph) s = buf_load16(rs_sph, wj * 16);
    }
    cand_j = -1;
    if (!hit) {
      s = make_float4(0.f, 0.f, 0.f, 1.f);
      c = make_float4(0.f, 0.f, 0.f, 0.f);
    }
    bool have = hit;
    float t = best;
    if (hit && !rehit_is_best(best, ((unsigned)key & 1u) != 0u)) have = rehit_full(r, best, s.x, s.y, s.z, s.w, &t);
    int32_t pixel = 0;
    const bool more = shade_ray<false>(r, have, t, s.x, s.y, s.z, c.x, c.y, c.z, c.w, lr, lg, lb, depth, max_depth, &pixel);
    if (!more | (dark & light_is_dead(lr, lg, lb))) {
      if (lane == 0) {
        pp->out[pix] = pixel;
        if (pp->cost != nullptr) {
          if (pp->cost_px != nullptr) pp->cost_px[pix] = (unsigned char)(depth < 254 ? depth + 1 : 255);
          if (depth >= 2) atomicMax(&pp->cost[ptile], depth + 1);
        }
      }
      trace_flush();
      return;
    }
  }
}

__device__ __forceinline__ int launch_dark() {
  return *reinterpret_cast<const volatile __attribute__((address_space(4))) int *>(&((KParamsArg)__builtin_amdgcn_kernarg_segment_ptr())->dark);
}

__device__ __forceinline__ unsigned long long launch_leaf_off() {
  KParamsArg kp = (KParamsArg)__builtin_amdgcn_kernarg_segment_ptr();
  asm volatile("" : "+s"(kp));
  return (unsigned long long)(unsigned)kp->leaf_box - 1ull;
}

template <int THREADS, bool ALL_LDS, bool STATS, bool SOLO, int TAIL = 0, bool ORD = false, bool CULL = false, int SPILL = 0, int RAYS = 0, int ENTRY = 0>
__global__ __launch_bounds__(THREADS, THREADS == 256 ? 5 : (THREADS / 64 + 3) / 4) void pooled_kernel(KParams p) {
  constexpr bool COLD = TAIL == 1, DONATE = TAIL == 2;
  constexpr bool ANY = RAYS == kRaysAny;
  constexpr bool ECOUNT = (ENTRY & kEntryModeMask) == kEntryCount;
  constexpr bool ECONST = ENTRY != 0 && (ENTRY & kEntryRtFlags) == 0;
  constexpr bool ECOL = (ENTRY & kEntryColLds) != 0;
  static_assert(!ENTRY || ((ENTRY & kEntryModeMask) == kEntryLists || ECOUNT), "ENTRY: lists, or the counting twin");
  static_assert(!ENTRY || (THREADS == 1024 && ALL_LDS && !STATS && !SOLO && TAIL == 0 && !ORD && !CULL && SPILL == 0 && RAYS == 0), "ENTRY: the plain 16-wave kernel of a scene in LDS only");
  static_assert(!RAYS || (!STATS && !SOLO && TAIL == 0 && !ORD && !CULL), "RAYS: the plain instantiations only");
  static_assert(!ORD || TAIL != 1, "ORD: no COLD variant");
  static_assert(!CULL || !ALL_LDS, "CULL: instantiated for the general scene path only");
  constexpr bool PRESORT = pooled_presort(ALL_LDS, SOLO, TAIL, ORD, RAYS);
  constexpr bool LEAFBOX = pooled_leaf_box(THREADS, ALL_LDS, STATS, SOLO, CULL, RAYS);
  extern __shared__ float4 smem[];
  const int lane = threadIdx.x & 63;
  const int wave = threadIdx.x >> 6;
  const int plane = p.lds_nodes;
  const int sph_base = ECOL ? (plane * (kPsNodeBytes / 4) + 3) >> 2 : 4 * plane;
  const int per_wave_dw = pooled_wave_dw(p.ray_planes, p.capb, p.capl);
  const int col_base = sph_base + p.lds_sph;
  unsigned *const wbase = reinterpret_cast<unsigned *>(smem + (ECOL ? col_base + p.n_sph : col_base)) + wave * per_wave_dw;
  unsigned long long *const wkey = reinterpret_cast<unsigned long long *>(wbase);
  int *const wcnt = reinterpret_cast<int *>(wbase + 128);
  unsigned *const wdump = wbase + 192;
  float4 *const wray = reinterpret_cast<float4 *>(wbase + kPooledWaveFixedDw);
  unsigned *const wbox = wbase + kPooledWaveFixedDw + 256 * p.ray_planes;
  unsigned *const wleaf = wbox + p.capb;
  const __amdgpu_buffer_rsrc_t rs_nodes = make_rsrc(p.nodes64, (unsigned)p.n_nodes * 64u);
  const __amdgpu_buffer_rsrc_t rs_sph = make_rsrc(p.sph, (unsigned)p.n_sph * 16u);
  const __amdgpu_buffer_rsrc_t rs_col = make_rsrc(p.col, (unsigned)p.n_sph * 16u);

  if constexpr (PRESORT) {
    auto ref_of = [](float w) { const int c = f2i(w) >> 8; return (unsigned)(c < 0 ? c : c * kPsNodeBytes) << kPsItemShift; };
    for (int i = threadIdx.x; i < plane; i += THREADS) {
      const float4 ll = p.nodes64[4 * i], lh = p.nodes64[4 * i + 1], rl = p.nodes64[4 * i + 2], rh = p.nodes64[4 * i + 3];
      presort_pack(reinterpret_cast<unsigned *>(smem) + (kPsNodeBytes / 4) * i, &ll.x, &lh.x, &rl.x, &rh.x, ref_of(ll.w), ref_of(lh.w));
    }
  } else {
    for (int i = threadIdx.x; i < 4 * plane; i += THREADS) smem[(i & 3) * plane + (i >> 2)] = p.nodes64[i];
  }
  for (int i = threadIdx.x; i < p.lds_sph; i += THREADS) smem[sph_base + i] = p.sph[i];
  if constexpr (ECOL)
    for (int i = threadIdx.x; i < p.n_sph; i += THREADS) smem[col_base + i] = p.col[i];
  for (int i = lane; i < per_wave_dw; i += 64) wbase[i] = 0u;
  unsigned *const wg_words = reinterpret_cast<unsigned *>(smem + sph_base + p.lds_sph) + 193;
  if (DONATE && threadIdx.x == 0) wg_words[1] = THREADS / 64;
  __syncthreads();
  wkey[lane] = kKeyInit;

  Ray r = {};
  float lr = 1.0f, lg = 1.0f, lb = 1.0f;
  int depth = 0;
  int pix = -1;
  unsigned long long n_rays = 0, n_box = 0, n_sph = 0;
  int nbox = 0, nleaf = 0;
  unsigned ec_lists = 0u, ec_fall = 0u;
  static_assert(!SPILL || (THREADS == 256 && !ALL_LDS && !SOLO && TAIL == 0 && !ORD), "SPILL: the plain and CULL kernels of the four-wave workgroups");
  unsigned *const wspill = wbase + 193;
  auto spill_region = [&]() { return p.spill + (size_t)(blockIdx.x * (THREADS / 64) + wave) * (size_t)p.spill_stride; };
  unsigned q_next = 0, q_end = 0;
  int q_tile = 0;
  int q_col0 = 0, q_row0 = 0;
  int q_frame_off = 0;
  Cam q_cam = p.cam;
  int ptile = 0;
  bool exhausted = false;
  bool hold = false;
  const bool deep_on = p.nframes == 1 && p.order != nullptr && p.deep_class > 0;
  const unsigned nwaves = gridDim.x * (THREADS / 64);
  const int ns_log2 = p.nshards > 1 ? 3 : 0;
  auto queue_const = [&]() {
    QueueConst qc;
    qc.ns_log2 = ns_log2; qc.tiles_x = p.tiles_x; qc.tiles_y = p.tiles_y; qc.nframes = p.nframes;
    qc.interleave = p.interleave;
    qc.ds = p.deep_split; qc.tpt = p.tpt_log2; qc.cap_log2 = p.deep_cap_log2; qc.ntiles = p.nchunks;
    qc.order = (!ORD && deep_on) ? p.order : nullptr; qc.deep_class = p.deep_class;
    qc.px = ORD ? p.px_hdr : nullptr;
    qc.home_waves = nwaves >> ns_log2;
    qc.q_static = p.static_first ? qc.home_waves : 0u;
    return qc;
  };
  unsigned q_state = queue_state_init((int)(blockIdx.x & ((1u << ns_log2) - 1u)), p.static_first != 0);
  bool q_enter = false;
  unsigned long long tr_t0 = 0, tr_exh = 0, tr_c0 = 0, tr_ops[3] = {0, 0, 0}, tr_items[2] = {0, 0};
  unsigned long long tr_cyc[5] = {0, 0, 0, 0, 0}, tr_nt = 0, tr_nb2 = 0;
  int tr_maxdepth = 0, tr_maxbox = 0, tr_maxleaf = 0;
  if (STATS) {
    tr_t0 = wall_clock64();
    tr_c0 = clock64();
  }

  unsigned q_cls = kPxClasses - 1;
  unsigned q_base = 0, q_ent = 0;
  if constexpr (ORD) {
    const bool solo_ok = SOLO && p.solo && p.tl_log2 == kTreeletDepth;
    for (;;) {
      TicketSpan sp;
      const QueueConst qc = queue_const();
      const unsigned wave_rank = (unsigned)uni((int)((unsigned)wave * (gridDim.x >> ns_log2) + (blockIdx.x >> ns_log2)));
      const bool got = queue_draw(q_state, qc, wave_rank, [&](int shard) {
        unsigned v = 0;
        if (lane == 0) v = atomicAdd(&p.queue[kQueueStride * shard], 1u);
        return (unsigned)__builtin_amdgcn_readfirstlane(v);
      }, &sp);
      if (!got) {
        exhausted = true;
        break;
      }
      if (sp.cls != 0u || !solo_ok) {
        q_next = sp.q_next;
        q_end = sp.q_end;
        q_cls = sp.cls;
        q_enter = true;
        break;
      }
      if constexpr (SOLO) {
        const unsigned e = p.px_list[sp.q_next];
        const int col = (int)(e & 0xffffu), lrow = (int)(e >> 16);
        const int k = lrow >> p.rpt_log2;
        const int grow = ((k * p.nparts + p.part) << p.rpt_log2) + (lrow & ((1 << p.rpt_log2) - 1));
        Ray pr;
        primary_dir_uv(p.cam, p.u_tab[col], p.v_tab[grow], pr);
        solo_trace<kSoloCull, STATS>((KParamsArg)__builtin_amdgcn_kernarg_segment_ptr(), (unsigned)(size_t)smem, (unsigned)(size_t)wbase, pr.ox, pr.oy, pr.oz,
                   pr.dx, pr.dy, pr.dz, 1.0f, 1.0f, 1.0f, lrow * p.w + col + k * p.out_skip, 0, (lrow >> 3) * p.tiles_x + (col >> 3));
      }
    }
  }
  if (!ORD && SOLO && deep_on && p.deep_split == 6 && p.tl_log2 == kTreeletDepth) {
    for (;;) {
      TicketSpan sp;
      const QueueConst qc = queue_const();
      const unsigned wave_rank = (unsigned)uni((int)((unsigned)wave * (gridDim.x >> ns_log2) + (blockIdx.x >> ns_log2)));
      const bool got = queue_draw(q_state, qc, wave_rank, [&](int shard) {
        unsigned v = 0;
        if (lane == 0) v = atomicAdd(&p.queue[kQueueStride * shard], 1u);
        return (unsigned)__builtin_amdgcn_readfirstlane(v);
      }, &sp);
      if (!got) {
        exhausted = true;
        break;
      }
      if (sp.q_end - sp.q_next != 1u) {
        q_next = sp.q_next;
        q_end = sp.q_end;
        q_enter = true;
        break;
      }
      const int tile = p.order[sp.q_next >> 6], within = (int)(sp.q_next & 63u);
      const int ty = tile / p.tiles_x;
      const int col = (tile - ty * p.tiles_x) * 8 + (within & 7), lrow = ty * 8 + (within >> 3);
      if (col < p.w && lrow < p.rows_local) {
        const int k = lrow >> p.rpt_log2;
        const int grow = ((k * p.nparts + p.part) << p.rpt_log2) + (lrow & ((1 << p.rpt_log2) - 1));
        Ray pr;
        primary_dir_uv(p.cam, p.u_tab[col], p.v_tab[grow], pr);
        solo_trace<kSoloCull, STATS>((KParamsArg)__builtin_amdgcn_kernarg_segment_ptr(), (unsigned)(size_t)smem, (unsigned)(size_t)wbase, pr.ox, pr.oy, pr.oz,
                   pr.dx, pr.dy, pr.dz, 1.0f, 1.0f, 1.0f, lrow * p.w + col + k * p.out_skip, 0, tile);
      }
    }
  }
  for (;;) {
    RT_MARK("CHOICE_BEGIN");
    __builtin_amdgcn_fence(__ATOMIC_ACQ_REL, "wavefront");
    if constexpr (SPILL) {
      if (nbox == 0) {
        const int nspill = uni((int)*wspill);
        if (__builtin_expect(nspill != 0, 0)) {
          const int n = nspill < 128 ? nspill : 128;
          const unsigned *const src = spill_region() + (nspill - n);
          __builtin_amdgcn_fence(__ATOMIC_ACQUIRE, "agent");
          for (int i = lane; i < n; i += 64) wbox[i] = __hip_atomic_load(&src[i], __ATOMIC_RELAXED, __HIP_MEMORY_SCOPE_AGENT);
          if (lane == 0) *wspill = (unsigned)(nspill - n);
          nbox = uni(n);
          __builtin_amdgcn_fence(__ATOMIC_ACQ_REL, "wavefront");
        }
      }
    }
    if (STATS) {
      tr_maxbox = nbox > tr_maxbox ? nbox : tr_maxbox;
      tr_maxleaf = nleaf > tr_maxleaf ? nleaf : tr_maxleaf;
    }
    bool leaf_op = nleaf >= 64;
    if (nbox < 64 && nleaf < 64) {
     bool drain = false;
     const int thr = p.thr_shade;
     const unsigned long long m_live = bal(pix >= 0);
     if (hold && m_live == 0ull) {
       hold = false;
       __builtin_amdgcn_s_setprio(0);
     }
     const bool vacant = (pix < 0) & !exhausted & !hold;
     const bool spilled = SPILL && uni((int)*wspill) != 0;
     if (nbox == 0 || (!spilled && nbox < p.look_max && (int)__popcll(m_live | bal(vacant)) >= thr)) {
      const bool done = (pix >= 0) & (wcnt[lane] == 0);
      const int ns = __popcll(bal(done | vacant));
      if (ns >= thr || nbox == 0) {
        if (nleaf > 0) {
          drain = true;
        } else {
          if (ns == 0) break;
          RT_MARK("SHADE_BEGIN");
          bool root = false;
          if (STATS) tr_ops[2]++;
          const unsigned long long tr_s0 = STATS ? clock64() : 0ull;
          if constexpr (ANY) {
            if (done) {
              p.occluded[pix] = wkey[lane] == kKeyAnyHit ? 1 : 0;
              pix = -1;
            }
          } else if (done) {
            if (STATS) tr_maxdepth = depth > tr_maxdepth ? depth : tr_maxdepth;
            const unsigned long long key = wkey[lane];
            const float best = __uint_as_float((unsigned)(key >> 32));
            const bool hit = key != kKeyInit;
            const int bestj = (int)((unsigned)key >> 1);
            const int wj = hit ? bestj : 0;
            float4 c, s;
            if constexpr (ECOL) c = smem[col_base + wj];
            else c = buf_load16(rs_col, wj * 16);
            if (ALL_LDS) {
              s = smem[sph_base + wj];
            } else {
              s = smem[sph_base + (wj < p.lds_sph ? wj : 0)];
              if (wj >= p.lds_sph) s = buf_load16(rs_sph, wj * 16);
            }
            if (!hit) {
              s = make_float4(0.f, 0.f, 0.f, 1.f);
              c = make_float4(0.f, 0.f, 0.f, 0.f);
            }
            bool have = hit;
            float t = best;
            if (hit && !rehit_is_best(best, ((unsigned)key & 1u) != 0u)) have = rehit_full(r, best, s.x, s.y, s.z, s.w, &t);
            int32_t pixel;
            if constexpr (!SPILL) pixel = 0;
            bool more;
            if constexpr (RAYS)
              more = shade_ray_emit<false>(r, have, t, s.x, s.y, s.z, c.x, c.y, c.z, c.w, lr, lg, lb, depth, p.max_depth,
                                           [&](float cr, float cg, float cb) { store_ray_result(p, pix, cr, cg, cb); });
            else
              more = shade_ray<false>(r, have, t, s.x, s.y, s.z, c.x, c.y, c.z, c.w, lr, lg, lb, depth, p.max_depth, &pixel);
            if constexpr (!RAYS && !SPILL) {
              const bool dark = ECONST || launch_dark() != 0, dead = light_is_dead(lr, lg, lb);
              more = more & !(dark & dead);
            }
            if constexpr (!RAYS && SPILL != 0) {
              if (more && launch_dark() && light_is_dead(lr, lg, lb)) {
                more = false;
                pixel = 0;
              }
            }
            if (more) {
              root = true;
            } else if constexpr (RAYS) {
              pix = -1;
            } else {
              p.out[pix] = pixel;
              if (p.cost != nullptr) {
                if (p.cost_px != nullptr) p.cost_px[pix] = (unsigned char)(depth < 254 ? depth + 1 : 255);
                if (depth >= 2) atomicMax(&p.cost[ptile], depth + 1);
              }
              pix = -1;
            }
          }
          bool want = (pix < 0) & !exhausted & !hold;
          int slot = -1;
          uint4 ent0 = make_uint4(0u, 0u, 0u, 0u), ent1 = ent0;
          float a_lo = p.ray_tlo, a_hi = p.ray_thi;
          unsigned long long m = bal(want);
          while (ORD && m != 0ull) {
            if (__builtin_expect(q_next == q_end, 0)) {
              if (hold) break;
              TicketSpan sp;
              const QueueConst qc = queue_const();
              const unsigned wave_rank = (unsigned)uni((int)((unsigned)wave * (gridDim.x >> ns_log2) + (blockIdx.x >> ns_log2)));
              const bool got = queue_draw(q_state, qc, wave_rank, [&](int shard) {
                unsigned v = 0;
                if (lane == 0) v = atomicAdd(&p.queue[kQueueStride * shard], 1u);
                return (unsigned)__builtin_amdgcn_readfirstlane(v);
              }, &sp);
              if (!got) {
                exhausted = true;
                if (STATS) tr_exh = wall_clock64();
                break;
              }
              q_next = sp.q_next;
              q_end = sp.q_end;
              q_cls = sp.cls;
              q_enter = true;
            }
            if (__builtin_expect(q_enter, 0)) {
              q_enter = false;
              if ((p.px_hold >> q_cls) & 1) {
                hold = true;
                if (p.px_prio >= 3) __builtin_amdgcn_s_setprio(3);
                else if (p.px_prio == 2) __builtin_amdgcn_s_setprio(2);
                else if (p.px_prio == 1) __builtin_amdgcn_s_setprio(1);
              }
              q_base = q_next;
              q_ent = (unsigned)lane < q_end - q_next ? p.px_list[q_next + (unsigned)lane] : 0u;
            }
            const unsigned avail = q_end - q_next;
            const unsigned rank = (unsigned)lane_rank(m);
            const unsigned cnt = (unsigned)__popcll(m);
            const unsigned e = (unsigned)__builtin_amdgcn_ds_bpermute((int)(((q_next - q_base + rank) & 63u) << 2), (int)q_ent);
            if (want & (rank < avail)) {
              const int col = (int)(e & 0xffffu), lrow = (int)(e >> 16);
              const int k = lrow >> p.rpt_log2;
              slot = lrow * p.w + col + k * p.out_skip;
              ptile = (lrow >> 3) * p.tiles_x + (col >> 3);
              const int grow = ((k * p.nparts + p.part) << p.rpt_log2) + (lrow & ((1 << p.rpt_log2) - 1));
              primary_dir_uv(p.cam, p.u_tab[col], p.v_tab[grow], r);
              want = false;
            }
            q_next += (cnt < avail) ? cnt : avail;
            m = bal(want);
          }
          while (!ORD && m != 0ull) {
            if (__builtin_expect(q_next == q_end, 0)) {
              if (hold) break;
              TicketSpan sp;
              const QueueConst qc = queue_const();
              const unsigned wave_rank = (unsigned)uni((int)((unsigned)wave * (gridDim.x >> ns_log2) + (blockIdx.x >> ns_log2)));
              const bool got = queue_draw(q_state, qc, wave_rank, [&](int shard) {
                unsigned v = 0;
                if (lane == 0) v = atomicAdd(&p.queue[kQueueStride * shard], 1u);
                return (unsigned)__builtin_amdgcn_readfirstlane(v);
              }, &sp);
              if (!got) {
                exhausted = true;
                if (STATS) tr_exh = wall_clock64();
                break;
              }
              q_next = sp.q_next;
              q_end = sp.q_end;
              q_enter = true;
            }
            if (__builtin_expect(q_enter || (q_next & 63u) == 0u, 0)) {
              q_enter = false;
              unsigned t = q_next >> 6;
              unsigned f = 0;
              if (p.nframes > 1) {
                if (p.order != nullptr) {
                  const int *cb = p.order + p.nchunks;
                  unsigned c = 0;
                  while (c + 1 < (unsigned)kOrderClasses && t >= (unsigned)p.nframes * (unsigned)cb[c + 1]) ++c;
                  const unsigned base = (unsigned)cb[c], size = (unsigned)cb[c + 1] - base;
                  const unsigned within = t - (unsigned)p.nframes * base;
                  f = within / size;
                  t = base + (within - f * size);
// ... 33 lines not shown
                r.dx = q[3]; r.dy = q[4]; r.dz = q[5];
                if (ANY && p.ray_tlo_dev != nullptr) {
                  a_lo = p.ray_tlo_dev[i];
                  a_hi = p.ray_thi_dev[i];
                }
                slot = i;
                want = false;
              }
            } else if (want & (rank < avail)) {
              const int within = (int)((q_next + rank) & 63u);
              const int col = q_col0 + (within & 7), lrow = q_row0 + (within >> 3);
              if (col < p.w && lrow < p.rows_local) {
                const int k = lrow >> p.rpt_log2;
                slot = q_frame_off + lrow * p.w + col + k * p.out_skip;
                ptile = q_tile;
                const int grow = ((k * p.nparts + p.part) << p.rpt_log2) + (lrow & ((1 << p.rpt_log2) - 1));
                if constexpr (ENTRY) {
                  const uint4 *const ep = reinterpret_cast<const uint4 *>(p.entry) + 2 * (size_t)(p.cams != nullptr ? (int)(q_next >> 6) : q_tile);
                  ent0 = ep[0];
                  ent1 = ep[1];
                }
                primary_dir_uv(q_cam, p.u_tab[col], p.v_tab[grow], r);
                want = false;
              }
            }
            q_next += (cnt < avail) ? cnt : avail;
            m = bal(want);
          }
          if (slot >= 0) {
            lr = 1.0f; lg = 1.0f; lb = 1.0f;
            depth = 0;
            pix = slot;
            root = true;
          }
          if constexpr (COLD) {
            unsigned long long m_l = bal(pix >= 0);
            if ((hold || exhausted) && nbox == 0 && m_l != 0ull && (int)__popcll(m_l) <= p.cold && bal(root) == m_l && p.tl_log2 == kTreeletDepth) {
              while (m_l != 0ull) {
                const int src = uni((int)__builtin_ctzll(m_l));
                m_l &= m_l - 1ull;
                auto rl = [&](float v) { return __int_as_float(__builtin_amdgcn_readlane(__float_as_int(v), src)); };
                solo_trace<kSoloCull, STATS>((KParamsArg)__builtin_amdgcn_kernarg_segment_ptr(), (unsigned)(size_t)smem, (unsigned)(size_t)wbase, rl(r.ox), rl(r.oy),
                           rl(r.oz), rl(r.dx), rl(r.dy), rl(r.dz), rl(lr), rl(lg), rl(lb), __builtin_amdgcn_readlane(pix, src),
                           __builtin_amdgcn_readlane(depth, src), __builtin_amdgcn_readlane(ptile, src));
              }
              wkey[lane] = kKeyInit;
              pix = -1;
              root = false;
            }
          }
          if constexpr (DONATE) {
            if ((hold || exhausted) && p.donate > 0 && p.tl_log2 == kTreeletDepth) {
              unsigned long long m_l = bal(root);
              if (m_l != 0ull && (int)__popcll(bal(pix >= 0)) <= p.donate) {
                unsigned idle = (unsigned)uni((int)__hip_atomic_load(&wg_words[0], __ATOMIC_RELAXED, __HIP_MEMORY_SCOPE_WORKGROUP));
                while (m_l != 0ull && idle != 0u) {
                  const int w = uni((int)__builtin_ctz(idle));
                  unsigned old = 0u;
                  if (lane == 0) old = __hip_atomic_fetch_and(&wg_words[0], ~(1u << w), __ATOMIC_RELAXED, __HIP_MEMORY_SCOPE_WORKGROUP);
                  old = (unsigned)__builtin_amdgcn_readfirstlane((int)old);
                  idle = old & ~(1u << w);
                  if ((old >> w) & 1u) {
                    const int src = uni((int)__builtin_ctzll(m_l));
                    m_l &= m_l - 1ull;
                    unsigned *const ob = wbase + (w - wave) * per_wave_dw;
                    float4 *const ib = reinterpret_cast<float4 *>(ob + kPooledWaveFixedDw);
                    if (lane == src) {
                      ib[0] = make_float4(r.ox, r.oy, r.oz, r.dx);
                      ib[1] = make_float4(r.dy, r.dz, lr, lg);
                      ib[2] = make_float4(lb, __int_as_float(pix), __int_as_float(depth), __int_as_float(ptile));
                    }
                    __builtin_amdgcn_fence(__ATOMIC_RELEASE, "workgroup");
                    if (lane == src) {
                      __hip_atomic_store(&ob[195], 1u, __ATOMIC_RELAXED, __HIP_MEMORY_SCOPE_WORKGROUP);
                      pix = -1;
                      root = false;
                    }
                  }
                }
              }
            }
          }
          if (root) ray_derive(r);
          const bool root_hit = root && (ANY ? interval_ok(a_lo, a_hi) && box_hit_interval(r, p.root_lo[0], p.root_lo[1], p.root_lo[2], p.root_hi[0], p.root_hi[1], p.root_hi[2], a_lo, a_hi)
                                             : box_hit(r, p.root_lo[0], p.root_lo[1], p.root_lo[2], p.root_hi[0], p.root_hi[1], p.root_hi[2]));
          unsigned ent_hdr = 0u;
          bool push_box = root_hit;
          if constexpr (ENTRY) {
            ent_hdr = (root_hit & (slot >= 0)) ? ent0.x : 0u;
            if (__builtin_expect((int)__popcll(bal(ent_hdr != 0u)) * kEntryLeaves > p.capl - nleaf, 0)) {
              const int nl = (int)(ent_hdr >> kEntryCountShift) & 15;
              int total = 0;
              for (int k = 0; k < kEntryLeaves; ++k) total += __popcll(bal(nl > k));
              if (uni(total) > p.capl - nleaf) {
                if constexpr (ECOUNT) ec_fall += (unsigned)__popcll(bal(ent_hdr != 0u));
                ent_hdr = 0u;
              }
            }
            if constexpr (ECOUNT) ec_lists += (unsigned)__popcll(bal((ent_hdr & kEntryValid) != 0u));
            push_box = root_hit & ((ent_hdr & kEntryValid) == 0u || (ent_hdr & kEntryInner) != 0u);
          }
          if (root) {
            wkey[lane] = ANY ? any_key_seed(a_hi) : kKeyInit;
            wcnt[lane] = push_box ? 1 : 0;
            wray[lane] = make_float4(r.ox, r.oy, r.oz, r.a);
            wray[64 + lane] = make_float4(r.ix, r.iy, r.iz, CULL ? cull_weight(r, p.cull_c2) : ANY ? a_lo : 0.0f);
            if (p.ray_planes == 3) wray[128 + lane] = make_float4(r.dx, r.dy, r.dz, 0.0f);
            if (STATS) { n_rays++; n_box++; }
          }
          const unsigned long long m_root = bal(push_box);
          if constexpr (!ENTRY) {
            if (root_hit) wbox[nbox + lane_rank(m_root)] = (unsigned)lane << 2 | (PRESORT ? sign_offsets(r) << 5 : 0u);
            nbox = uni(nbox + __popcll(m_root));
          } else {
            const unsigned low = (unsigned)lane << 2 | (PRESORT ? sign_offsets(r) << 5 : 0u);
            if (push_box) wbox[nbox + lane_rank(m_root)] = ((ent_hdr & kEntryValid) != 0u ? ent0.y : 0u) | low;
            nbox = uni(nbox + __popcll(m_root));
            const unsigned lf[kEntryLeaves] = {ent0.z, ent0.w, ent1.x, ent1.y, ent1.z, ent1.w};
            const int nl = (ent_hdr & kEntryValid) != 0u ? (int)(ent_hdr >> kEntryCountShift) & 15 : 0;
            for (int k = 0; k < kEntryLeaves; ++k) {
              const unsigned long long m_k = bal(nl > k);
              if (m_k == 0ull) break;
              if (nl > k) wleaf[nleaf + lane_rank(m_k)] = lf[k] | low;
              nleaf = uni(nleaf + __popcll(m_k));
            }
          }
          if (p.prio_depth > 0 && !hold) {
            const bool live = pix >= 0;
            if (bal(live && depth >= 4 * p.prio_depth) != 0ull) __builtin_amdgcn_s_setprio(3);
            else if (bal(live && depth >= 2 * p.prio_depth) != 0ull) __builtin_amdgcn_s_setprio(2);
            else if (bal(live && depth >= p.prio_depth) != 0ull) __builtin_amdgcn_s_setprio(1);
            else __builtin_amdgcn_s_setprio(0);
          }
          if (STATS) tr_cyc[4] += clock64() - tr_s0;
          RT_MARK("SHADE_END");
          continue;
        }
      }
     }
     leaf_op = drain | (nbox == 0);
    }
    if (leaf_op) {
      RT_MARK("LEAF_BEGIN");
      if (STATS) { tr_ops[1]++; tr_items[1] += nleaf < 64 ? nleaf : 64; }
      const unsigned long long tr_l0 = STATS ? clock64() : 0ull;
      const int top = nleaf - 1 - lane;
      const unsigned item = wleaf[top < 0 ? 0 : top];
      const bool act = top >= 0;
      nleaf = uni(nleaf > 64 ? nleaf - 64 : 0);
      const int sl = (int)(item & 0xfcu) >> 2;
      const int j = ~((int)item >> (PRESORT ? kPsItemShift : 8));
      const float4 ra = wray[sl];
      Ray q;
      q.ox = ra.x; q.oy = ra.y; q.oz = ra.z; q.a = ra.w;
      if (p.ray_planes == 3) {
        const float4 rd = wray[128 + sl];
        asm volatile("" ::"v"(rd.w));
        q.dx = rd.x; q.dy = rd.y; q.dz = rd.z;
      } else {
        const int sl4 = (int)(item & 0xfcu);
        q.dx = pull(sl4, r.dx); q.dy = pull(sl4, r.dy); q.dz = pull(sl4, r.dz);
      }
      const int jj = act ? j : 0;
      float4 s;
      if (ALL_LDS) {
        s = smem[sph_base + jj];
      } else {
        s = smem[sph_base + (jj < p.lds_sph ? jj : 0)];
        if (jj >= p.lds_sph) s = buf_load16(rs_sph, jj * 16);
      }
      if (STATS) n_sph += act ? 1 : 0;
      if constexpr (ANY) {
        const float tlo = reinterpret_cast<const float *>(wray + 64 + sl)[3], thi = key_hi(wkey, sl);
        if (act && sphere_hit_any(q, tlo, thi, s.x, s.y, s.z, s.w)) wkey[sl] = kKeyAnyHit;
      } else {
        bool near_root;
        const float g = sphere_root_flag(q, s.x, s.y, s.z, s.w, &near_root);
        if (act & (g < kTMax))
          atomicMin(&wkey[sl],
                    ((unsigned long long)__float_as_uint(g) << 32) | ((unsigned)jj << 1) | (near_root ? 1u : 0u));
      }
      if (STATS) { __builtin_amdgcn_s_waitcnt(0); tr_cyc[3] += clock64() - tr_l0; }
      RT_MARK("LEAF_END");
    } else {
      auto box = [&](auto full_tag) {
        constexpr bool FULL = decltype(full_tag)::value;
        if constexpr (FULL) RT_MARK("BOXFULL_BEGIN"); else RT_MARK("BOXPART_BEGIN");
        if (STATS) { tr_ops[0]++; tr_items[0] += FULL ? 64 : nbox; }
        const int top = nbox - 1 - lane;
        const unsigned item = wbox[FULL ? top : (top < 0 ? 0 : top)];
        const unsigned long long m_act = FULL ? ~0ull : bal(top >= 0);
        nbox = uni(FULL ? nbox - 64 : 0);
        const int sl4 = (int)(item & 0xfcu);
        const int ni16 = (int)((item >> 4) & 0xfffffff0u);
        const float4 *const rayp = reinterpret_cast<const float4 *>(reinterpret_cast<const char *>(wray) + 4 * sl4);
        const float4 ra = rayp[0], ri = rayp[64];
        Ray q;
        q.ox = ra.x; q.oy = ra.y; q.oz = ra.z;
        q.ix = ri.x; q.iy = ri.y; q.iz = ri.z;
        int cl8, cr8;
// ... 147 lines not shown
        if (STATS) n_box += __popcll(m_pass & ~m_ln & (1ull << lane)) + __popcll(m_pass & ~m_rn & (1ull << lane));
        const int c_inl = __popcll(m_inl), c_lfl = __popcll(m_lfl);
        const int dump = (int)(size_t)(wdump);
        const int b_box = (int)(size_t)(wbox), b_leaf = (int)(size_t)(wleaf + nleaf);
        const int a_l = sel_mask(m_lfl, sel_mask(m_inl, dump, b_box + 4 * lane_rank(m_inl)), b_leaf + 4 * lane_rank(m_lfl));
        const int a_r = sel_mask(m_lfr, sel_mask(m_inr, dump, b_box + 4 * lane_rank_from(m_inr, c_inl)),
                                 b_leaf + 4 * lane_rank_from(m_lfr, c_lfl));
        const unsigned low = PRESORT ? item & kPsItemLow : (unsigned)sl4;
        lds_store(a_l, (unsigned)sel_mask(m_cleaf, cl8, ref) | low);
        lds_store(a_r, (unsigned)cr8 | low);
        nbox = uni(c_inl + __popcll(m_inr));
        nleaf = uni(nleaf + c_lfl + __popcll(m_lfr));
        const int d = sel_mask(m_inl, 0, 1) + sel_mask(m_inr, 0, 1) - sel_mask(bal(act & (role == 0)), 0, 1);
        lds_add_masked(bal(d != 0), (int)(size_t)wcnt + sl4, d);
        RT_MARK("BOX2_END");
      };
      const unsigned long long tr_b0 = STATS ? clock64() : 0ull;
      int tr_kind = 0;
      if constexpr (SPILL) {
        if (__builtin_expect(nbox > SPILL, 0)) {
          const int S = (nbox >> 1) & ~63;
          const int nspill = uni((int)*wspill);
          unsigned *const dst = spill_region() + nspill;
          for (int i = lane; i < S; i += 64) __hip_atomic_store(&dst[i], wbox[i], __ATOMIC_RELAXED, __HIP_MEMORY_SCOPE_AGENT);
          for (int i = lane; i < nbox - S; i += 64) {
            const unsigned v = wbox[S + i];
            __builtin_amdgcn_fence(__ATOMIC_ACQ_REL, "wavefront");
            wbox[i] = v;
            __builtin_amdgcn_fence(__ATOMIC_ACQ_REL, "wavefront");
          }
          __builtin_amdgcn_fence(__ATOMIC_RELEASE, "agent");
          if (lane == 0) *wspill = (unsigned)(nspill + S);
          nbox = uni(nbox - S);
        }
      }
      if (nbox >= 64) box(std::true_type{});
      else if (nbox <= 32 && p.box2) { box2(); tr_kind = 1; }
      else box(std::false_type{});
      if (STATS) {
        __builtin_amdgcn_s_waitcnt(0);
        const unsigned long long dt = clock64() - tr_b0;
        if (tr_kind == 0) tr_cyc[0] += dt;
        else if (tr_kind == 1) { tr_cyc[1] += dt; tr_nb2++; }
        else tr_cyc[2] += dt;
      }
    }
  }
  if constexpr (DONATE) {
    if (p.donate > 0 && p.tl_log2 == kTreeletDepth) {
      __builtin_amdgcn_s_setprio(0);
      __builtin_amdgcn_fence(__ATOMIC_RELEASE, "workgroup");
      if (lane == 0) __hip_atomic_fetch_add(&wg_words[1], ~0u, __ATOMIC_RELAXED, __HIP_MEMORY_SCOPE_WORKGROUP);
      bool offered = false;
      for (;;) {
        if (!offered) {
          if (lane == 0) __hip_atomic_fetch_or(&wg_words[0], 1u << wave, __ATOMIC_RELAXED, __HIP_MEMORY_SCOPE_WORKGROUP);
          offered = true;
        }
        const unsigned active = (unsigned)uni((int)__hip_atomic_load(&wg_words[1], __ATOMIC_RELAXED, __HIP_MEMORY_SCOPE_WORKGROUP));
        __builtin_amdgcn_fence(__ATOMIC_ACQUIRE, "workgroup");
        const unsigned full = (unsigned)uni((int)__hip_atomic_load(&wbase[195], __ATOMIC_RELAXED, __HIP_MEMORY_SCOPE_WORKGROUP));
        __builtin_amdgcn_fence(__ATOMIC_ACQUIRE, "workgroup");
        if (full != 0u) {
          const float4 a = wray[0], b = wray[1], c = wray[2];
          __builtin_amdgcn_fence(__ATOMIC_ACQ_REL, "workgroup");
          if (lane == 0) __hip_atomic_store(&wbase[195], 0u, __ATOMIC_RELAXED, __HIP_MEMORY_SCOPE_WORKGROUP);
          offered = false;
          __builtin_amdgcn_s_setprio(2);
          solo_trace<kSoloCull, STATS>((KParamsArg)__builtin_amdgcn_kernarg_segment_ptr(), (unsigned)(size_t)smem, (unsigned)(size_t)wbase, a.x, a.y, a.z, a.w,
                     b.x, b.y, b.z, b.w, c.x, __float_as_int(c.y), __float_as_int(c.z), __float_as_int(c.w));
          __builtin_amdgcn_s_setprio(0);
          continue;
        }
        if (active == 0u) break;
        __builtin_amdgcn_s_sleep(16);
      }
    }
  }
  queue_leave(p, nwaves, lane);
  if constexpr (ECOUNT) {
    if (lane == 0 && p.trace != nullptr) {
      unsigned long long *const rec = p.trace + 2 * (size_t)(blockIdx.x * (THREADS / 64) + wave);
      rec[0] = ec_lists; rec[1] = ec_fall;
    }
  }
  if (STATS) {
    atomicAdd(&p.stats[0], n_rays);
    atomicAdd(&p.stats[1], n_box);
    atomicAdd(&p.stats[2], n_sph);
    if (p.trace != nullptr) {
      const unsigned long long t_end = wall_clock64(), c_end = clock64();
      int md = tr_maxdepth;
      for (int o = 32; o > 0; o >>= 1) { const int other = __shfl_xor(md, o); md = other > md ? other : md; }
      if (lane == 0) {
        unsigned long long *rec = p.trace + (size_t)(blockIdx.x * (THREADS / 64) + wave) * kTraceWords;
        rec[0] = tr_t0; rec[1] = tr_exh; rec[2] = t_end;
        rec[3] = tr_ops[0] | (tr_ops[1] << 21) | (tr_ops[2] << 42);
        rec[4] = c_end - tr_c0;
        rec[5] = tr_nt | (tr_nb2 << 32);
        rec[8] = tr_cyc[0]; rec[9] = tr_cyc[1]; rec[10] = tr_cyc[2]; rec[11] = tr_cyc[3]; rec[12] = tr_cyc[4];
        rec[6] = (tr_items[0] << 32) | tr_items[1];
        rec[7] = (unsigned long long)md | ((unsigned long long)tr_maxbox << 16) | ((unsigned long long)tr_maxleaf << 32);
      }
    }
  }
}

constexpr int kOrderThreads = 128;
constexpr int kOrderBins = 64;

__device__ __forceinline__ int order_bin(int v) { return kOrderBins - 1 - min(kOrderBins - 1, max(v, 0)); }

struct OrderChunk {
  Shard sh;
  int begin, end;
};
__device__ __forceinline__ OrderChunk order_chunk(int ntiles, int tiles_x, int nshards, int nblocks) {
  OrderChunk c;
  const int s = (int)blockIdx.x / nblocks, b = (int)blockIdx.x - s * nblocks;
  c.sh = shard_of(s, nshards > 1 ? 3 : 0, tiles_x, ntiles / tiles_x);
  const int n = c.sh.ntiles;
  const int per_block = (n + nblocks - 1) / nblocks, b0 = min(n, b * per_block), b1 = min(n, b0 + per_block);
  const int per = (b1 - b0 + kOrderThreads - 1) / kOrderThreads;
  c.begin = min(b1, b0 + (int)threadIdx.x * per);
  c.end = min(b1, c.begin + per);
  return c;
}
__device__ __forceinline__ void order_count(const OrderChunk &c, const int *cost, int tiles_x, int (*hist)[kOrderThreads]) {
  const int t = threadIdx.x;
  for (int b = 0; b < kOrderBins; ++b) hist[b][t] = 0;
  for (int i0 = c.begin; i0 < c.end; i0 += 8) {
    int v[8];
#pragma unroll
    for (int u = 0; u < 8; ++u) v[u] = i0 + u < c.end ? cost[shard_tile(c.sh, i0 + u, tiles_x)] : 0;
#pragma unroll
    for (int u = 0; u < 8; ++u)
      if (i0 + u < c.end) hist[order_bin(v[u])][t] += 1;
  }
  __syncthreads();
}
__global__ __launch_bounds__(kOrderThreads) void tile_count_kernel(const int *cost, int ntiles, int tiles_x, int nshards, int nblocks, int *counts) {
  __shared__ int hist[kOrderBins][kOrderThreads];
  const OrderChunk c = order_chunk(ntiles, tiles_x, nshards, nblocks);
  order_count(c, cost, tiles_x, hist);
  const int t = threadIdx.x;
  if (t < kOrderBins) {
    int acc = 0;
    for (int k = 0; k < kOrderThreads; ++k) acc += hist[t][k];
    const int s = (int)blockIdx.x / nblocks, b = (int)blockIdx.x - s * nblocks;
    counts[(s * kOrderBins + t) * nblocks + b] = acc;
  }
}
__global__ __launch_bounds__(kOrderThreads) void tile_scan_kernel(int *counts, int *order, int ntiles, int nblocks) {
  __shared__ int bin_tot[kOrderBins + 1];
  const int t = threadIdx.x, s = (int)blockIdx.x;
  int *const cs = counts + s * kOrderBins * nblocks;
  if (t < kOrderBins) {
    int acc = 0;
    for (int b = 0; b < nblocks; ++b) {
      const int c = cs[t * nblocks + b];
      cs[t * nblocks + b] = acc;
      acc += c;
    }
    bin_tot[t] = acc;
  }
  __syncthreads();
// ... 231 lines not shown

hipError_t launch_pixel(const KParams &p, bool stats, hipStream_t stream) {
  const int tiles_y = (p.rows_local + 7) / 8;
  const unsigned grid = (unsigned)(p.tiles_x * tiles_y);
  if (grid == 0) return hipSuccess;
  if (stats) hipLaunchKernelGGL(pixel_kernel<true>, dim3(grid), dim3(64), 0, stream, p);
  else hipLaunchKernelGGL(pixel_kernel<false>, dim3(grid), dim3(64), 0, stream, p);
  return hipGetLastError();
}

static hipError_t allow_full_lds(const void *kfn) {
  constexpr int kMaxDev = 64, kMaxFn = 32;
  static std::mutex mu;
  static const void *fns[kMaxFn];
  static unsigned long long done[kMaxFn];
  int dev = 0;
  if (hipError_t e = hipGetDevice(&dev); e != hipSuccess) return e;
  std::lock_guard<std::mutex> lock(mu);
  int slot = -1;
  for (int i = 0; i < kMaxFn && slot < 0; ++i) {
    if (fns[i] == kfn) slot = i;
    else if (fns[i] == nullptr) { fns[i] = kfn; slot = i; }
  }
  if (slot >= 0 && dev < kMaxDev && (done[slot] >> dev & 1ull)) return hipSuccess;
  if (hipError_t e = hipFuncSetAttribute(kfn, hipFuncAttributeMaxDynamicSharedMemorySize, 160 * 1024); e != hipSuccess) return e;
  if (slot >= 0 && dev < kMaxDev) done[slot] |= 1ull << dev;
  return hipSuccess;
}

size_t persistent_lds_bytes(int lds_nodes, int lds_sph, int smax, int lmax, int waves_per_wg) {
  return (size_t)lds_nodes * 32 + (size_t)lds_sph * 16 + (size_t)waves_per_wg * (smax + 1 + lmax) * 64 * sizeof(int);
}

template <int THREADS, bool STATS>
static hipError_t launch_persistent_t(const KParams &p, int grid, hipStream_t stream) {
  const size_t lds = persistent_lds_bytes(p.lds_nodes, p.lds_sph, p.smax, p.lmax, THREADS / 64);
  auto kfn = persistent_kernel<THREADS, STATS>;
  if (hipError_t e = allow_full_lds(reinterpret_cast<const void *>(kfn)); e != hipSuccess) return e;
  hipLaunchKernelGGL(kfn, dim3(grid), dim3(THREADS), lds, stream, p);
  return hipGetLastError();
}

hipError_t launch_persistent(const KParams &p, bool stats, int grid, int waves_per_wg, hipStream_t stream) {
  if (grid <= 0) return hipSuccess;
  if (stats) return launch_persistent_t<512, true>(p, grid, stream);
  switch (waves_per_wg) {
  case 4: return launch_persistent_t<256, false>(p, grid, stream);
  case 8: return launch_persistent_t<512, false>(p, grid, stream);
  case 12: return launch_persistent_t<768, false>(p, grid, stream);
  case 16: return launch_persistent_t<1024, false>(p, grid, stream);
  default: return hipErrorInvalidValue;
  }
}

size_t pooled_lds_bytes(int lds_nodes, int lds_sph, int capb, int capl, int ray_planes, int waves_per_wg) {
  return (size_t)lds_nodes * 64 + (size_t)lds_sph * 16 + (size_t)waves_per_wg * pooled_wave_dw(ray_planes, capb, capl) * sizeof(unsigned);
}

template <int I>
static auto pooled_fn() {
  constexpr const PooledKey &k = kPooledKeys[I];
  return pooled_kernel<k.threads, k.all_lds, k.stats, k.solo, k.tail, k.ord, k.cull, k.spill, k.rays>;
}

template <int I>
static hipError_t launch_pooled_t(const KParams &p, int grid, hipStream_t stream) {
  constexpr int threads = kPooledKeys[I].threads;
  const size_t lds = pooled_lds_bytes(p.lds_nodes, p.lds_sph, p.capb, p.capl, p.ray_planes, threads / 64);
  auto kfn = pooled_fn<I>();
  if (hipError_t e = allow_full_lds(reinterpret_cast<const void *>(kfn)); e != hipSuccess) return e;
  hipLaunchKernelGGL(kfn, dim3(grid), dim3(threads), lds, stream, p);
  return hipGetLastError();
}

template <int... I>
static hipError_t launch_pooled_key(const PooledKey &k, const KParams &p, int grid, hipStream_t stream, std::integer_sequence<int, I...>) {
  hipError_t e = hipErrorInvalidValue;
  (void)((kPooledKeys[I] == k && ((e = launch_pooled_t<I>(p, grid, stream)), true)) || ...);
  return e;
}

template <int ENTRY>
static hipError_t launch_pooled_entry_t(const KParams &p, int grid, hipStream_t stream) {
  const size_t lds = (ENTRY & kEntryColLds) ? pooled_col_lds_bytes(p.n_nodes, p.n_sph, p.capb, p.capl, p.ray_planes)
                                            : pooled_lds_bytes(p.lds_nodes, p.lds_sph, p.capb, p.capl, p.ray_planes, 16);
  auto kfn = pooled_kernel<1024, true, false, false, 0, false, false, 0, 0, ENTRY>;
  if (hipError_t e = allow_full_lds(reinterpret_cast<const void *>(kfn)); e != hipSuccess) return e;
  hipLaunchKernelGGL(kfn, dim3(grid), dim3(1024), lds, stream, p);
  return hipGetLastError();
}
template <int... E>
static hipError_t launch_pooled_entry_any(const KParams &p, int grid, hipStream_t stream, int entry, std::integer_sequence<int, E...>) {
  hipError_t e = hipErrorInvalidValue;
  (void)((E == entry && ((e = launch_pooled_entry_t<E>(p, grid, stream)), true)) || ...);
  return e;
}
static hipError_t launch_pooled_entry(const PooledKey &k, const KParams &p, int grid, hipStream_t stream, int entry) {
  const int mode = entry & kEntryModeMask;
  if (!pooled_entry_ok(k) || p.entry == nullptr || p.rays != nullptr || (mode != kEntryLists && mode != kEntryCount) || (mode == kEntryCount && p.trace == nullptr))
    return hipErrorInvalidValue;
  if (!(entry & kEntryRtFlags) && !pooled_entry_flags_const(p.leaf_box, p.dark)) return hipErrorInvalidValue;
  if ((entry & kEntryColLds) && !pooled_col_fits(pooled_col_lds_bytes(p.n_nodes, p.n_sph, p.capb, p.capl, p.ray_planes), 160 * 1024)) return hipErrorInvalidValue;
  return launch_pooled_entry_any(p, grid, stream, entry,
                                 std::integer_sequence<int, kEntryLists, kEntryLists | kEntryColLds, kEntryLists | kEntryRtFlags, kEntryCount, kEntryCount | kEntryColLds,
                                                       kEntryCount | kEntryRtFlags>{});
}

__global__ __launch_bounds__(256) void tile_entry_kernel(KParams p, int ref_shift, int node_mul, int filter) {
  const unsigned pos = blockIdx.x * 256u + threadIdx.x;
  if (pos >= (p.cams != nullptr ? (unsigned)p.nframes : 1u) * (unsigned)p.nchunks) return;
  const unsigned f = pos / (unsigned)p.nchunks;
  const int tile = (int)(pos - f * (unsigned)p.nchunks);
  const int ty = tile / p.tiles_x, tx = tile - ty * p.tiles_x;
  const int col0 = tx * 8, col1 = col0 + 7 < p.w ? col0 + 7 : p.w - 1;
  const int lrow0 = ty * 8, lrow1 = lrow0 + 7 < p.rows_local ? lrow0 + 7 : p.rows_local - 1;
  auto grow = [&](int lrow) { return (((lrow >> p.rpt_log2) * p.nparts + p.part) << p.rpt_log2) + (lrow & ((1 << p.rpt_log2) - 1)); };
  const Cam cam = p.cams != nullptr ? p.cams[f] : p.cam;
  TileRays t;
  const bool ok = tile_rays(cam, p.u_tab[col0], p.u_tab[col1], p.v_tab[grow(lrow0)], p.v_tab[grow(lrow1)], &t);
  unsigned e[kEntryDw];
  tile_entry(t, ok, p.root_lo, p.root_hi, reinterpret_cast<const float *>(p.nodes64), p.n_nodes, filter != 0, ref_shift, node_mul, e);
  uint4 *const out = reinterpret_cast<uint4 *>(const_cast<unsigned *>(p.entry)) + 2 * (size_t)pos;
  out[0] = make_uint4(e[0], e[1], e[2], e[3]);
  out[1] = make_uint4(e[4], e[5], e[6], e[7]);
}
hipError_t launch_tile_entry(const KParams &p, bool stats, int waves_per_wg, hipStream_t stream) {
  PooledKey k;
  if (p.entry == nullptr || p.rays != nullptr || !choose_pooled(p, stats, waves_per_wg, 0, &k) || !pooled_entry_ok(k)) return hipErrorInvalidValue;
  const unsigned npos = (p.cams != nullptr ? (unsigned)p.nframes : 1u) * (unsigned)p.nchunks;
  if (npos == 0) return hipSuccess;
  const bool presort = pooled_presort(k);
  hipLaunchKernelGGL(tile_entry_kernel, dim3((npos + 255u) / 256u), dim3(256), 0, stream, p, presort ? kPsItemShift : 8, presort ? kPsNodeBytes : 1,
                     p.leaf_box != 0 && pooled_leaf_box(k) ? 1 : 0);
  return hipGetLastError();
}

hipError_t launch_pooled(const KParams &p, bool stats, int grid, int waves_per_wg, hipStream_t stream, int rays, int entry) {
  if (rays == kRaysAny && p.occluded == nullptr) return hipErrorInvalidValue;
  if ((p.ray_tlo_dev != nullptr || p.ray_thi_dev != nullptr) && (rays != kRaysAny || p.ray_tlo_dev == nullptr || p.ray_thi_dev == nullptr)) return hipErrorInvalidValue;
  if (grid <= 0 || (rays && p.nrays <= 0)) return hipSuccess;
  PooledKey k;
  if (!choose_pooled(p, stats, waves_per_wg, rays, &k)) return hipErrorInvalidValue;
  if (entry != 0) return rays == 0 && !stats ? launch_pooled_entry(k, p, grid, stream, entry) : hipErrorInvalidValue;
  return launch_pooled_key(k, p, grid, stream, std::make_integer_sequence<int, kNumPooledKeys>{});
}

hipError_t launch_pixel_rays(const KParams &p, hipStream_t stream) {
  if (p.nrays <= 0) return hipSuccess;
  hipLaunchKernelGGL((pixel_kernel<false, true>), dim3((unsigned)((p.nrays + 63) / 64)), dim3(64), 0, stream, p);
  return hipGetLastError();
}

__global__ __launch_bounds__(64) void scratch_warm_kernel(int *sink, int k) {
  volatile int a[8];
  a[k & 7] = k;
  a[(k + 1) & 7] = 1;
  if (a[(k + 2) & 7] == 0x5ca7c4) *sink = 1;
}
hipError_t warm_scratch(hipStream_t stream, int *sink_dev) {
  int dev = 0, cus = 256;
  if (hipGetDevice(&dev) == hipSuccess) (void)hipDeviceGetAttribute(&cus, hipDeviceAttributeMultiprocessorCount, dev);
  hipLaunchKernelGGL(scratch_warm_kernel, dim3(cus * 32), dim3(64), 0, stream, sink_dev, 1);
  return hipGetLastError();
}
template <int... I>
static void warm_pooled(std::integer_sequence<int, I...>) {
  hipFuncAttributes a;
  ((void)(pooled_warmed(kPooledKeys[I]) && hipFuncGetAttributes(&a, reinterpret_cast<const void *>(pooled_fn<I>())) == hipSuccess), ...);
}
void warm_render_kernels() {
  warm_pooled(std::make_integer_sequence<int, kNumPooledKeys>{});
  hipFuncAttributes a;
  (void)hipFuncGetAttributes(&a, reinterpret_cast<const void *>(pooled_kernel<1024, true, false, false, 0, false, false, 0, 0, kEntryLists>));
  (void)hipFuncGetAttributes(&a, reinterpret_cast<const void *>(pooled_kernel<1024, true, false, false, 0, false, false, 0, 0, kEntryLists | kEntryColLds>));
  (void)hipFuncGetAttributes(&a, (const void *)tile_entry_kernel);
  (void)hipFuncGetAttributes(&a, (const void *)px_count_kernel);
  (void)hipFuncGetAttributes(&a, (const void *)px_scan_kernel);
  (void)hipFuncGetAttributes(&a, (const void *)px_place_kernel);
  (void)hipFuncGetAttributes(&a, (const void *)px_header_kernel);
  (void)hipFuncGetAttributes(&a, (const void *)tile_count_kernel);
  (void)hipFuncGetAttributes(&a, (const void *)tile_scan_kernel);
  (void)hipFuncGetAttributes(&a, (const void *)tile_place_kernel);
}

hipError_t launch_place_part(const int32_t *part, int32_t *image, int w, int rows_local, int rows_per_tile, int part_id,
                             int nparts, hipStream_t stream) {
  const size_t total = (size_t)rows_local * w;
  if (total == 0) return hipSuccess;
  const unsigned grid = (unsigned)((total + 255) / 256 < 4096 ? (total + 255) / 256 : 4096);
  hipLaunchKernelGGL(place_part_kernel, dim3(grid), dim3(256), 0, stream, part, image, w, rows_local, rows_per_tile,
                     part_id, nparts);
  return hipGetLastError();
}

hipError_t launch_place_all(const int32_t *stacked, int32_t *image, int w, int h, int rows_per_tile, int nparts,
                            size_t part_stride, hipStream_t stream, int nframes, size_t frame_stride_in, size_t frame_stride_out) {
  const size_t nrows = (size_t)h * (size_t)nframes;
  if (nrows == 0 || w <= 0) return hipSuccess;
  const unsigned grid = (unsigned)(nrows < 16384 ? nrows : 16384);
  const bool vec = w % 4 == 0 && part_stride % 4 == 0 && frame_stride_in % 4 == 0 && frame_stride_out % 4 == 0 &&
                   (reinterpret_cast<uintptr_t>(stacked) | reinterpret_cast<uintptr_t>(image)) % 16 == 0;
  hipLaunchKernelGGL(place_all_kernel, dim3(grid), dim3(256), 0, stream, stacked, image, w, h, rows_per_tile, nparts,
                     part_stride, nframes, frame_stride_in, frame_stride_out, vec ? 1 : 0);
  return hipGetLastError();
}

}
```

raytracers_amd/csrc/rt_device.hpp:

```cpp
#pragma once
#include <hip/hip_runtime.h>
#include <stdint.h>

#include <string>

#include "lane_core.h"
#include "treelet.h"

namespace rtk {

constexpr int kTraceWords = 16;
constexpr int kStackPixel = 64;
constexpr int kPooledWaveFixedDw = 128 + 64 + 4;
constexpr int pooled_wave_dw(int ray_planes, int capb, int capl) { return kPooledWaveFixedDw + 256 * ray_planes + capb + capl; }
constexpr int kSpillCapb = 1088, kSpillCapbTest = 192;

constexpr int kQueueStride = 32;
constexpr int kMaxShards = 8;
constexpr int kQueueExit = kQueueStride * kMaxShards;
constexpr int kQueueDwords = kQueueStride * (kMaxShards + 1);
constexpr int kOrderTableDw = 16;
constexpr int order_table_ints(int ntiles) { return ntiles + kOrderTableDw * kMaxShards; }

struct Shard {
// ... 112 lines not shown
      got = t < tickets;
    } else if (tickets > c.q_static) {
      t = fetch_add(sh) + c.q_static;
      got = t < tickets;
    }
    if (got) {
      if (c.interleave) t = (t << c.ns_log2) + (unsigned)sh;
      *sp = c.px != nullptr ? px_ticket_span(t, c.px) : ticket_span(t, (unsigned)s.seg, npos, n_split, (unsigned)ndeep, c.ds, c.tpt);
      return true;
    }
    state |= 0x100u << sh;
    if ((state & all) == all) return false;
    unsigned nx = (unsigned)sh;
    do nx = (nx + 1u) & ((1u << c.ns_log2) - 1u); while ((state >> (8 + nx)) & 1u);
    state = (state & ~7u) | nx;
  }
}

struct KParams {
  const float4 *nodes;
  const float4 *nodes64;
  const float4 *sph;
  const float4 *col;
  float root_lo[3], root_hi[3];
  int n_nodes, n_sph;
  Cam cam;
  int w, h;
  int rows_local;
  int rows_per_tile, part, nparts;
  int rpt_log2;
  int tiles_x;
  int tiles_y;
  int max_depth;
  int32_t *out;
  int out_skip;
  int nframes;
  int tpt_log2;
  int frame_stride;
  const Cam *cams;
  unsigned long long *stats;
  unsigned long long *trace;
  unsigned *queue;
  int nshards;
  int interleave;
  int static_first;
  int nchunks;
  int lds_nodes;
  int lds_sph;
  int smax, lmax;
  int thr_shade, thr_leaf;
  int capb, capl;
  int ray_planes;
  int prio_depth;
  const int *order;
  int donate;
  int cold;
  int look_max;
  int box2;
  int solo;
  int tl_log2;
  int deep_class;
  int deep_split;
  int deep_cap_log2;
  int *cost;
  unsigned char *cost_px;
  const int *px_hdr;
  const unsigned *px_list;
  int px_hold;
  int px_prio;
  int cull;
  float cull_c2;
  float cull_kappa;
  int dark;
  const float *u_tab;
  const float *v_tab;
  unsigned *spill;
  int spill_stride;
  int leaf_box;
  const float *rays;
  union {
    float *colour3;
    const unsigned *entry;
  };
  int nrays;
  unsigned char *occluded;
  float ray_tlo, ray_thi;
  const float *ray_tlo_dev, *ray_thi_dev;
};

#if defined(__HIPCC__)
__device__ __forceinline__ int f2i(float f) { return __float_as_int(f); }

typedef int v4i __attribute__((ext_vector_type(4)));
__device__ __forceinline__ __amdgpu_buffer_rsrc_t make_rsrc(const void *base, unsigned bytes) {
  return __builtin_amdgcn_make_buffer_rsrc(const_cast<void *>(base), 0, (int)bytes, 0x00020000);
}
__device__ __forceinline__ float4 buf_load16(__amdgpu_buffer_rsrc_t rsrc, int byte_off) {
  const v4i v = __builtin_amdgcn_raw_buffer_load_b128(rsrc, byte_off, 0, 0);
  return make_float4(__int_as_float(v.x), __int_as_float(v.y), __int_as_float(v.z), __int_as_float(v.w));
}
__device__ __forceinline__ Ray load_ray(const float *rays, int i) {
  const float *const q = rays + (size_t)i * 6;
  Ray r;
  r.ox = q[0]; r.oy = q[1]; r.oz = q[2];
  r.dx = q[3]; r.dy = q[4]; r.dz = q[5];
  ray_derive(r);
  return r;
}
#endif

constexpr int kRaysColour = 1, kRaysAny = 2;
struct PooledKey {
  int threads;
  bool all_lds, stats, solo;
  int tail;
  bool ord, cull;
  int spill;
  int rays;
  constexpr bool operator==(const PooledKey &o) const {
    return threads == o.threads && all_lds == o.all_lds && stats == o.stats && solo == o.solo && tail == o.tail && ord == o.ord && cull == o.cull &&
           spill == o.spill && rays == o.rays;
  }
};
namespace pooled_keys {
constexpr bool T = true, F = false;
constexpr int SP = kSpillCapb - 64, ST = kSpillCapbTest - 64, RC = kRaysColour, RA = kRaysAny;
constexpr PooledKey kPooledKeys[] = {
    {1024, T, F, F, 0, F, F, 0, 0}, {1024, F, F, F, 0, F, F, 0, 0}, {1024, F, F, F, 0, F, T, 0, 0},
    {1024, T, F, T, 0, F, F, 0, 0}, {1024, F, F, T, 0, F, F, 0, 0}, {1024, F, F, T, 0, F, T, 0, 0},
    {1024, T, F, F, 1, F, F, 0, 0}, {1024, F, F, F, 1, F, F, 0, 0}, {1024, F, F, F, 1, F, T, 0, 0},
    {1024, T, F, T, 1, F, F, 0, 0}, {1024, F, F, T, 1, F, F, 0, 0}, {1024, F, F, T, 1, F, T, 0, 0},
    {1024, T, F, F, 2, F, F, 0, 0}, {1024, F, F, F, 2, F, F, 0, 0}, {1024, F, F, F, 2, F, T, 0, 0},
    {1024, T, F, T, 2, F, F, 0, 0}, {1024, F, F, T, 2, F, F, 0, 0}, {1024, F, F, T, 2, F, T, 0, 0},
    {1024, T, F, F, 0, T, F, 0, 0}, {1024, F, F, F, 0, T, F, 0, 0}, {1024, F, F, F, 0, T, T, 0, 0},
    {1024, T, F, T, 0, T, F, 0, 0}, {1024, F, F, T, 0, T, F, 0, 0}, {1024, F, F, T, 0, T, T, 0, 0},
    {1024, T, F, F, 2, T, F, 0, 0}, {1024, F, F, F, 2, T, F, 0, 0}, {1024, F, F, F, 2, T, T, 0, 0},
    {1024, T, F, T, 2, T, F, 0, 0}, {1024, F, F, T, 2, T, F, 0, 0}, {1024, F, F, T, 2, T, T, 0, 0},
    {1024, F, T, F, 0, F, F, 0, 0}, {1024, F, T, F, 0, F, T, 0, 0}, {1024, F, T, F, 0, T, F, 0, 0}, {1024, F, T, F, 0, T, T, 0, 0},
    {1024, F, T, T, 0, T, F, 0, 0}, {1024, F, T, T, 0, T, T, 0, 0}, {512, F, T, F, 0, F, F, 0, 0},
    {256, T, F, F, 0, F, F, 0, 0}, {256, F, F, F, 0, F, F, 0, 0}, {256, T, F, T, 0, F, F, 0, 0}, {256, F, F, T, 0, F, F, 0, 0},
    {512, T, F, F, 0, F, F, 0, 0}, {512, F, F, F, 0, F, F, 0, 0}, {512, T, F, T, 0, F, F, 0, 0}, {512, F, F, T, 0, F, F, 0, 0},
    {768, T, F, F, 0, F, F, 0, 0}, {768, F, F, F, 0, F, F, 0, 0}, {768, T, F, T, 0, F, F, 0, 0}, {768, F, F, T, 0, F, F, 0, 0},
    {256, F, F, F, 0, F, T, 0, 0}, {256, F, F, F, 0, F, F, SP, 0}, {256, F, F, F, 0, F, T, SP, 0}, {256, F, F, F, 0, F, F, ST, 0}, {256, F, F, F, 0, F, T, ST, 0},
    {1024, T, F, F, 0, F, F, 0, RC}, {1024, F, F, F, 0, F, F, 0, RC}, {256, F, F, F, 0, F, F, 0, RC}, {256, F, F, F, 0, F, F, SP, RC}, {256, F, F, F, 0, F, F, ST, RC},
    {1024, T, F, F, 0, F, F, 0, RA}, {1024, F, F, F, 0, F, F, 0, RA}, {256, F, F, F, 0, F, F, 0, RA}, {256, F, F, F, 0, F, F, SP, RA}, {256, F, F, F, 0, F, F, ST, RA},
};
}
using pooled_keys::kPooledKeys;
constexpr int kNumPooledKeys = sizeof(kPooledKeys) / sizeof(kPooledKeys[0]);
constexpr bool pooled_warmed(const PooledKey &k) {
  return !k.stats && k.rays == 0 && (k.threads == 1024 || (k.threads == 256 && !k.all_lds && !k.solo && k.spill != kSpillCapbTest - 64));
}

constexpr bool pooled_entry_ok(const PooledKey &k) {
  return k.threads == 1024 && k.all_lds && !k.stats && !k.solo && k.tail == 0 && !k.ord && !k.cull && k.spill == 0 && k.rays == 0;
}

inline bool choose_pooled(const KParams &p, bool stats, int waves_per_wg, int rays, PooledKey *out) {
  const bool all_lds = p.lds_nodes == p.n_nodes && p.lds_sph == p.n_sph;
  PooledKey k{64 * waves_per_wg, false, stats, false, 0, false, p.cull != 0, 0, rays};
  if (rays && (stats || p.cull || p.px_hdr != nullptr || p.order != nullptr || p.nframes != 1)) return false;
  if (p.cull && waves_per_wg != 16 && waves_per_wg != 4) return false;
  if (p.spill != nullptr) {
    if (waves_per_wg != 4 || stats || p.px_hdr != nullptr || (p.capb != kSpillCapb && p.capb != kSpillCapbTest)) return false;
    k.spill = p.capb - 64;
  } else if (p.cull && waves_per_wg == 4) {
    if (stats || p.px_hdr != nullptr) return false;
  } else if (rays) {
    if (waves_per_wg != 16 && waves_per_wg != 4) return false;
    k.all_lds = waves_per_wg == 16 && all_lds;
  } else if (stats) {
    if (waves_per_wg != 16) k.threads = 512;
    else if (p.px_hdr != nullptr) { k.ord = true; k.solo = p.solo != 0; }
  } else if (p.px_hdr != nullptr) {
    if (waves_per_wg != 16 || p.nframes != 1) return false;
    k.ord = true; k.solo = p.solo != 0; k.tail = p.donate ? 2 : 0;
    k.all_lds = all_lds && !k.cull;
  } else {
    k.solo = p.solo && p.nframes == 1 && p.order != nullptr && p.deep_class > 0 && p.deep_split == 6 && p.tl_log2 == kTreeletDepth;
    if (waves_per_wg == 16) k.tail = p.cold ? 1 : p.donate ? 2 : 0;
    else if (waves_per_wg != 4 && waves_per_wg != 8 && waves_per_wg != 12) return false;
    k.all_lds = all_lds && !k.cull;
  }
  *out = k;
  return true;
}

constexpr bool pooled_presort(bool all_lds, bool solo, int tail, bool ord, int rays) { return all_lds && !solo && tail == 0 && !ord && rays == 0; }
constexpr bool pooled_presort(const PooledKey &k) { return pooled_presort(k.all_lds, k.solo, k.tail, k.ord, k.rays); }

constexpr bool pooled_leaf_box(int threads, bool all_lds, bool stats, bool solo, bool cull, int rays) {
  return rays == 0 && !cull && (stats || (all_lds && !(threads == 256 && solo)));
}
constexpr bool pooled_leaf_box(const PooledKey &k) { return pooled_leaf_box(k.threads, k.all_lds, k.stats, k.solo, k.cull, k.rays); }

inline std::string pooled_name(const PooledKey &k) {
  std::string s = k.rays == kRaysAny ? "any" : k.ord ? "ORD" : k.tail == 1 ? "COLD" : k.tail == 2 ? "DONATE" : "";
  if (k.solo) s += s.empty() ? "SOLO" : "+SOLO";
  if (k.ord && k.tail == 2) s += "+DONATE";
  if (s.empty()) s = "plain";
  if (k.cull) s += "+CULL";
  if (k.spill) s += "+SPILL";
  return s;
}

hipError_t launch_pixel(const KParams &p, bool stats, hipStream_t stream);
hipError_t launch_pixel_rays(const KParams &p, hipStream_t stream);
hipError_t launch_persistent(const KParams &p, bool stats, int grid, int waves_per_wg, hipStream_t stream);
size_t persistent_lds_bytes(int lds_nodes, int lds_sph, int smax, int lmax, int waves_per_wg);
constexpr int kEntryLists = 1, kEntryCount = 2;
constexpr int kEntryModeMask = 3, kEntryColLds = 4, kEntryRtFlags = 8;
constexpr bool pooled_entry_flags_const(int leaf_box, int dark) { return leaf_box != 0 && dark != 0; }
constexpr size_t pooled_col_lds_bytes(int n_nodes, int n_sph, int capb, int capl, int ray_planes) {
  return (((size_t)n_nodes * kPsNodeBytes + 15) & ~(size_t)15) + (size_t)n_sph * 32 + (size_t)16 * pooled_wave_dw(ray_planes, capb, capl) * sizeof(unsigned);
}
constexpr bool pooled_col_fits(size_t col_lds_bytes, size_t lds_limit) { return col_lds_bytes <= lds_limit; }
constexpr int pooled_entry_bits(int mode, int leaf_box, int dark, size_t col_lds_bytes, size_t lds_limit, bool col_lds = true) {
  return !pooled_entry_flags_const(leaf_box, dark) ? mode | kEntryRtFlags : mode | (col_lds && pooled_col_fits(col_lds_bytes, lds_limit) ? kEntryColLds : 0);
}
hipError_t launch_pooled(const KParams &p, bool stats, int grid, int waves_per_wg, hipStream_t stream, int rays = 0, int entry = 0);
hipError_t launch_tile_entry(const KParams &p, bool stats, int waves_per_wg, hipStream_t stream);
size_t pooled_lds_bytes(int lds_nodes, int lds_sph, int capb, int capl, int ray_planes, int waves_per_wg);
struct GpuBvhOut {
  float *L7;
  float *bmin, *bmax;
  int *left, *right, *parent;
  float4 *nodes32;
  float4 *nodes64;
  float4 *sph, *col;
  int *ids;
};
void warm_render_kernels();
hipError_t warm_scratch(hipStream_t stream, int *sink_dev);
void warm_build_kernels();
size_t gpu_build_scratch_bytes(int n);
hipError_t gpu_copy_from_pinned(void *dst_dev, const void *src_pinned, size_t bytes, hipStream_t stream);
size_t gpu_build_pinned_bytes();
hipError_t gpu_build_bvh(const float *sph7_dev, int n, const GpuBvhOut &out, char *scratch, char *pinned, hipStream_t stream,
                         int *height_out, float root_lo[3], float root_hi[3]);
struct CullStatsDev {
  double c_max;
  float lo[3], hi[3];
  float r_min, r_max;
  int bad;
  int pad;
};
static_assert(sizeof(CullStatsDev) == 48, "CullStatsDev: 48 bytes");
constexpr size_t kCullStatsPinnedOffset = 256;
constexpr int kCullStatsBlocks = 1024;
constexpr size_t cull_stats_scratch_bytes() { return sizeof(CullStatsDev) * kCullStatsBlocks; }
hipError_t launch_cull_stats(const float *sph7_dev, int n, CullStatsDev *partial, CullStatsDev *out, hipStream_t stream);

hipError_t launch_leaf_boxes(float4 *nodes64, const float4 *sph, int n_nodes, float q, float lin, float abs, hipStream_t stream);

constexpr int kOrderBlocksMax = 64;
constexpr int kOrderScratchInts = kMaxShards * 64 * kOrderBlocksMax;
hipError_t launch_tile_order(int *cost, int *order, int ntiles, int tiles_x, int nshards, int *scratch, hipStream_t stream);
struct PxGeom {
  int w, rows_local, rpt_log2, out_skip, tiles_x, tiles_y;
};
struct PxPolicy {
  int thr[kPxClasses - 1];
  int g[kPxClasses];
  int ray_ns;
  int nwaves;
  int solo_cap;
  int zip;
};
constexpr int kPxBlocksMax = 2048;
constexpr size_t px_scratch_ints() { return (size_t)64 * kPxBlocksMax + 256; }
hipError_t launch_px_order(const unsigned char *cost_px, const PxGeom &g, const PxPolicy &pol, unsigned *list, int *hdr, int *scratch, hipStream_t stream);
hipError_t launch_place_part(const int32_t *part, int32_t *image, int w, int rows_local, int rows_per_tile, int part_id,
                             int nparts, hipStream_t stream);

hipError_t launch_place_all(const int32_t *stacked, int32_t *image, int w, int h, int rows_per_tile, int nparts,
                            size_t part_stride, hipStream_t stream, int nframes = 1, size_t frame_stride_in = 0,
                            size_t frame_stride_out = 0);

}
```

raytracers_amd/csrc/rt_internal.hpp:

```cpp
#pragma once
#include <hip/hip_runtime.h>

#include <cstdint>
#include <future>
#include <mutex>
#include <string>
#include <vector>

#include "../../include/rt_mi355x.h"
#include "rt_device.hpp"
#include "rt_host.hpp"

struct rt_group;

struct rt_context {
  std::recursive_mutex mu;
  int device = 0;
  hipStream_t stream = nullptr;
  bool own_stream = false;
  std::string err;
  bool synced_since_render = true;
  std::string last_launch;
  int num_cu = 0;
  int lds_bytes = 0;
  std::string name;
  int variant = RT_VARIANT_AUTO;
  int waves_per_wg = 0;
  int wgs_per_cu = 1;
  int thr_shade = 40;
  int thr_leaf = 24;
  int lmax = 8;
  int lds_scene_bytes = -1;
  int lds_sph_first = 0;
  int handover = 1;
  int donate_max = 64;
  int look_max = 0;
  int box2 = 1;
  int solo = 1;
  int treelet = rtk::kTreeletDepth;
  int trace_solo = 0;
  int trace_part = 0, trace_nparts = 1;
  int ray_planes = 0;
  int gpu_build = 1;
  int prio_depth = 4;
  int grid_div = 0;
  int adaptive_order = 1;
  int deep_class = -1;
  int deep_split = 2;
  int deep_cap_log2 = 5;
  int xcd_queues = -1;
  int tpt_log2 = -1;
  int static_first = 1;
  int first_order = 1;
  int pixel_order = 1;
  int px_thr[4] = {0, 24, 14, 9};
  int px_g[5] = {0, 0, 0, 0, 0};
  int px_max_tiles = 40000;
  int px_ray_ns = 0;
  int px_hold = 0xf;
  int px_zip = 1;
  int px_prio = 3;
  int px_solo_div = 4;
  int stack_cap = 0;
  int wide_waves = 1;
  int cull = -1;
  int dark_stop = -1;
  int leaf_box = -1;
  int eager_sort = 1;
  int borrow = 1;
  int sync_policy = 0;
  hipStream_t sort_stream = nullptr, sort_stream_px = nullptr;
  hipEvent_t rec_event = nullptr;
  unsigned *queue_dev = nullptr;
  int entry_lists = -1;
  unsigned *entry_dev = nullptr;
  size_t entry_bytes = 0;
  int entry_keep = -1;
  int col_lds = -1;
  uint64_t entry_tables_built = 0, entry_tables_kept = 0;
  int last_entry = 0;
  bool entry_count = false;
  unsigned long long *entry_counts_dev = nullptr;
  size_t entry_counts_bytes = 0;
  int64_t entry_counts_waves = 0;
  unsigned *spill_dev = nullptr;
  size_t spill_bytes = 0;
  int *order_scratch = nullptr;
  int *px_scratch = nullptr;
  char *within_scratch = nullptr;
  size_t within_bytes = 0;
  unsigned long long *stats_dev = nullptr;
  struct UvTable {
    int64_t w, h;
    float *u, *v;
    size_t bytes = 0;
  };
  std::vector<UvTable> uv;
  struct FirstOrder {
    int tiles_x, tiles_y;
    int *order;
    size_t bytes;
  };
  std::vector<FirstOrder> first_orders;
  struct Block {
    char *p;
    size_t bytes;
  };
  std::vector<Block> pool;
  char *arena = nullptr;
  std::vector<unsigned char> arena_used;
  float *cams_dev = nullptr;
  float *cams_host = nullptr;
  size_t cams_bytes = 0;
  hipEvent_t cams_event = nullptr;
  bool cams_event_valid = false;
  rt_group *group = nullptr;
  int *class_slab = nullptr;
  unsigned long long class_chunks_used = 0;
  char *pinned = nullptr;
  char *stage = nullptr;
};

struct rt_scene {
  rt::SceneDesc desc;
  struct DevCopy {
    int device;
    float *p;
  };
  mutable std::mutex mu;
  mutable std::vector<DevCopy> copies;
  mutable bool cull_done = false;
  mutable rt::CullConst cull;
  mutable rt::LeafBoxConst leaf;
};

struct TileOrder {
  int64_t h, w;
  int32_t rows_per_tile, part, nparts, max_depth;
  float cam[12];
  int ntiles = 0;
  int nshards = 1;
  char *block = nullptr;
  size_t block_bytes = 0;
  rt_context *block_owner = nullptr;
  int *cost = nullptr;
  int *order = nullptr;
  bool valid = false;
  unsigned *entry = nullptr;
  bool entry_valid = false;
  int entry_filter = 0;
  rt_context *entry_ctx = nullptr;
  unsigned char *cost_px = nullptr;
  unsigned *px_list = nullptr;
  size_t cost_px_bytes = 0, px_elems = 0;
  bool px_valid = false;
  bool sort_pending = false, sort_px = false;
  hipEvent_t sort_event = nullptr, sort_event_px = nullptr;
  bool sort_inflight = false, sort_inflight_px = false;
  int rec_out_skip = 0;
  bool px_solo = false;
  uint64_t stamp = 0;
  bool have_classes = false;
  int classes[9] = {0, 0, 0, 0, 0, 0, 0, 0, 0};
  int classes_slot = -1;
  hipEvent_t classes_event = nullptr;
  bool classes_pending = false;
};
constexpr int kClassSlotInts = 16, kClassSlots = 8;
constexpr int kClassChunks = 64;

struct rt_prepared {
  rt_context *home = nullptr;
  mutable std::recursive_mutex mu;
  mutable std::vector<TileOrder> orders;
  mutable uint64_t order_clock = 0;
  int64_t n = 0;
  int64_t h = 0, w = 0;
  rt::Camera cam{};
  int height = 0;
  int tl_depth = 1;
  rt::CullConst cull;
  rt::LeafBoxConst leaf;
  float *L7 = nullptr, *bmin = nullptr, *bmax = nullptr;
  int32_t *left = nullptr, *right = nullptr, *parent = nullptr;
  float4 *nodes = nullptr, *nodes64 = nullptr, *sph = nullptr, *col = nullptr;
  int32_t *ids = nullptr;
  char *block = nullptr;
  size_t block_bytes = 0;
  float root_lo[3] = {0, 0, 0}, root_hi[3] = {0, 0, 0};
  int *classes_pinned = nullptr;
  int classes_chunk = -1;
  rt_context *classes_owner = nullptr;
  std::vector<rt_prepared *> replicas;
  std::vector<std::future<int>> replica_jobs;
};


namespace rtk {
hipError_t launch_first_order(int *order, int *rank, int tiles_x, int tiles_y, hipStream_t stream);
hipError_t launch_uv_tables(float *u, float *v, int w, int h, hipStream_t stream);
}

namespace rti {
int fail(rt_context *ctx, const std::string &msg);
int hip_fail(rt_context *ctx, hipError_t e, const char *what);
int enqueue_render(rt_context *ctx, const rt_prepared *ps, int64_t h, int64_t w, int32_t max_depth, int32_t rows_per_tile,
                   int32_t part, int32_t nparts, int32_t *out_dev, bool stats, const float *cam12 = nullptr, int32_t nframes = 1,
                   int64_t frame_stride = 0, const float *cams_dev = nullptr, bool inplace = false);
constexpr int64_t kMaxPositions = int64_t(1) << 26;
inline int64_t tiles_of(int64_t rows, int64_t w) { return ((rows + 7) / 8) * ((w + 7) / 8); }
int group_render(rt_context *ctx, const rt_prepared *ps, int64_t h, int64_t w, int32_t max_depth, int32_t *out_dev,
                 const float *cam12, int32_t nframes = 1, int64_t frame_stride = 0, const float *cams12 = nullptr);
int stage_cams(rt_context *ctx, const float *cams12, int32_t nframes, const float **cams_dev);
#pragma GCC visibility push(hidden)
struct Plan {
  int variant;
  int lds_nodes, lds_sph, smax, lmax, waves, grid;
  int grid_full;
  int capb, capl, ray_planes;
  int spill_stride;
  size_t lds_bytes;
};
void scene_params(const rt_prepared *ps, rtk::KParams *p);
int pooled_rays_plan(rt_context *ctx, const rt_prepared *ps, int64_t n, Plan *pl);
int pooled_rays_params(rt_context *ctx, const rt_prepared *ps, const Plan &pl, rtk::KParams *pp);
int launch_pooled_rays(rt_context *ctx, const rtk::KParams &p, const Plan &pl, int rays);
hipError_t pool_alloc(rt_context *ctx, char **out, size_t *bytes_io);
void pool_free(rt_context *ctx, char *p, size_t bytes);
#pragma GCC visibility pop
void group_prepare_begin(rt_context *ctx, rt_prepared *ps, int64_t h, int64_t w, const rt_scene *scene);
int group_prepare_end(rt_context *ctx, rt_prepared *ps);
void group_prepared_free(rt_context *ctx, rt_prepared *ps);
int group_sync(rt_context *ctx);
void group_mark_synced(rt_context *ctx);
int group_set_variant(rt_context *ctx, int variant);
int group_set_option(rt_context *ctx, const char *name, int64_t value);
void group_destroy(rt_context *ctx);
}

#ifndef RT_NO_CONTEXT_LOCK
#define RT_LOCK(ctx) std::unique_lock<std::recursive_mutex> rt_lock_ = (ctx) ? std::unique_lock<std::recursive_mutex>((ctx)->mu) : std::unique_lock<std::recursive_mutex>()
#define RT_LOCK_PS(ps) std::lock_guard<std::recursive_mutex> ps_lock_((ps)->mu)
#else
#define RT_LOCK(ctx) (void)(ctx)
#define RT_LOCK_PS(ps) (void)(ps)
#endif

#define RT_HIP(ctx, call)                                             \
  do {                                                                \
    hipError_t e_ = (call);                                           \
    if (e_ != hipSuccess) return rti::hip_fail((ctx), e_, #call);     \
  } while (0)
```

Baseline: 22770.

## Add exit tables that start secondary rays at a nested sub-box below the root

Adds per-sphere exit tables built from the top levels of the BVH. A secondary ray leaving a sphere can start traversal from the deepest enclosing node plus the sibling boxes along the path, instead of from the root. These tables are stored in LDS next to the tree and used in the entry-list kernel variant. The aim is to skip the upper-level box tests for secondary rays. The cost is extra LDS use, a table-build kernel run per tree generation, and more bookkeeping in the shading loop.

```diff
diff --git a/include/rt_mi355x.h b/include/rt_mi355x.h
--- a/include/rt_mi355x.h
+++ b/include/rt_mi355x.h
@@ -29,6 +29,7 @@
 const char *rt_context_last_launch(const rt_context *ctx);
 int rt_context_entry_counts(rt_context *ctx, uint64_t *lists, uint64_t *fallbacks, int64_t *waves, uint64_t *per_wave, int64_t cap_waves);
 int rt_context_entry_info(rt_context *ctx, int32_t *colour_lds, int32_t *flags_const, uint64_t *tables_built, uint64_t *tables_kept);
+int rt_context_exit_info(rt_context *ctx, int32_t *active, int32_t *dmax, uint64_t *tables_built, uint64_t *tables_kept, uint64_t *lists, uint64_t *fallbacks);
 int rt_context_sync(rt_context *ctx);
 int rt_context_set_variant(rt_context *ctx, int variant);
 int rt_context_set_option(rt_context *ctx, const char *name, int64_t value);
diff --git a/raytracers_amd/_lib.py b/raytracers_amd/_lib.py
--- a/raytracers_amd/_lib.py
+++ b/raytracers_amd/_lib.py
@@ -7,7 +7,7 @@
 
 RT_SYMBOLS = [
     "rt_context_create", "rt_device_count", "rt_context_create_multi", "rt_context_num_devices", "rt_context_gather_mode", "rt_context_rccl_ranks",
-    "rt_context_destroy", "rt_last_error", "rt_context_last_launch", "rt_context_entry_counts", "rt_context_entry_info", "rt_context_sync", "rt_context_set_variant",
+    "rt_context_destroy", "rt_last_error", "rt_context_last_launch", "rt_context_entry_counts", "rt_context_entry_info", "rt_context_exit_info", "rt_context_sync", "rt_context_set_variant",
     "rt_context_set_option", "rt_context_device_info",
     "rt_scene_rgbbox", "rt_scene_irreg", "rt_scene_floor", "rt_scene_from_spheres", "rt_scene_num_spheres",
     "rt_scene_free",
@@ -62,6 +62,7 @@
         "rt_context_last_launch": (C.c_char_p, [vp]),
         "rt_context_entry_counts": (C.c_int, [vp, C.POINTER(C.c_uint64), C.POINTER(C.c_uint64), C.POINTER(i64), C.POINTER(C.c_uint64), i64]),
         "rt_context_entry_info": (C.c_int, [vp, C.POINTER(i32), C.POINTER(i32), C.POINTER(C.c_uint64), C.POINTER(C.c_uint64)]),
+        "rt_context_exit_info": (C.c_int, [vp, C.POINTER(i32), C.POINTER(i32), C.POINTER(C.c_uint64), C.POINTER(C.c_uint64), C.POINTER(C.c_uint64), C.POINTER(C.c_uint64)]),
         "rt_context_sync": (C.c_int, [vp]),
         "rt_context_set_variant": (C.c_int, [vp, C.c_int]),
         "rt_context_set_option": (C.c_int, [vp, C.c_char_p, i64]),
diff --git a/raytracers_amd/api.py b/raytracers_amd/api.py
--- a/raytracers_amd/api.py
+++ b/raytracers_amd/api.py
@@ -71,6 +71,13 @@
         col, const, built, kept = C.c_int32(), C.c_int32(), C.c_uint64(), C.c_uint64()
         self._check(lib.rt_context_entry_info(self._h, C.byref(col), C.byref(const), C.byref(built), C.byref(kept)))
         return {"colour_lds": bool(col.value), "flags_const": bool(const.value), "tables_built": built.value, "tables_kept": kept.value}
+
+    def exit_info(self):
+        act, dmax = C.c_int32(), C.c_int32()
+        built, kept, lists, falls = C.c_uint64(), C.c_uint64(), C.c_uint64(), C.c_uint64()
+        self._check(lib.rt_context_exit_info(self._h, C.byref(act), C.byref(dmax), C.byref(built), C.byref(kept), C.byref(lists), C.byref(falls)))
+        return {"active": bool(act.value), "dmax": dmax.value, "tables_built": built.value, "tables_kept": kept.value, "lists": lists.value,
+                "fallbacks": falls.value}
 
     @property
     def rccl_ranks(self):
diff --git a/raytracers_amd/csrc/api.cpp b/raytracers_amd/csrc/api.cpp
--- a/raytracers_amd/csrc/api.cpp
+++ b/raytracers_amd/csrc/api.cpp
@@ -473,6 +473,30 @@
     ctx->entry_bytes = bytes;
   }
   p->entry = ctx->entry_dev;
+  return 0;
+}
+
+int set_exit(rt_context *ctx, const rt_prepared *ps, const Plan &pl, rtk::KParams *p, int *entry, bool *build) {
+  p->exit_tab = nullptr; p->exit_room = 0;
+  *build = false;
+  if (ctx->exit_lists == 0 || (*entry & (rtk::kEntryColLds | rtk::kEntryRtFlags)) != rtk::kEntryColLds || pl.lds_nodes != p->n_nodes) return 0;
+  if (!rtk::pooled_exit_fits(p->n_nodes, p->n_sph, p->capb, p->capl, p->ray_planes, static_cast<size_t>(std::min(ctx->lds_bytes, 160 * 1024)))) return 0;
+  const int room = p->capb - 64 * std::max(0, ps->height - 3) - 128;
+  if (room < 64 + 63) return 0;
+  const size_t need = rtk::exit_tab_bytes(p->n_sph);
+  if (ctx->exit_bytes < need) {
+    drain_streams(ctx);
+    pool_free(ctx, reinterpret_cast<char *>(ctx->exit_dev), ctx->exit_bytes);
+    ctx->exit_dev = nullptr; ctx->exit_bytes = 0; ctx->exit_gen = 0;
+    char *blk = nullptr;
+    size_t bytes = need;
+    RT_HIP(ctx, pool_alloc(ctx, &blk, &bytes));
+    ctx->exit_dev = reinterpret_cast<float4 *>(blk);
+    ctx->exit_bytes = bytes;
+  }
+  *build = ctx->exit_gen != ps->tree_gen;
+  p->exit_tab = ctx->exit_dev; p->exit_room = room;
+  *entry |= rtk::kEntryExit;
   return 0;
 }
 
@@ -860,6 +884,18 @@
   int entry = 0;
   bool build_entry = false;
   if (int rc = set_entry(ctx, pl, to, &p, &entry, &build_entry)) return rc;
+  bool build_exit = false;
+  if (int rc = set_exit(ctx, ps, pl, &p, &entry, &build_exit)) return rc;
+  if (p.exit_tab) {
+    if (build_exit) {
+      ctx->exit_gen = 0;
+      RT_HIP(ctx, rtk::launch_exit_tables(p, ctx->exit_dev, ctx->stream));
+      ctx->exit_gen = ps->tree_gen;
+      ctx->exit_tables_built++;
+    } else {
+      ctx->exit_tables_kept++;
+    }
+  }
   if (p.entry) {
     if (build_entry) {
       RT_HIP(ctx, rtk::launch_tile_entry(p, false, pl.waves, ctx->stream));
@@ -869,7 +905,7 @@
     }
     if (to != nullptr && p.entry == to->entry) to->entry_valid = true;
     if (ctx->entry_count) {
-      const size_t nw = static_cast<size_t>(pl.grid) * static_cast<size_t>(pl.waves), bytes = nw * 2 * sizeof(unsigned long long);
+      const size_t nw = static_cast<size_t>(pl.grid) * static_cast<size_t>(pl.waves), bytes = nw * 4 * sizeof(unsigned long long);
       if (ctx->entry_counts_bytes < bytes) {
         drain_streams(ctx);
         if (ctx->entry_counts_dev) (void)hipFree(ctx->entry_counts_dev);
@@ -984,6 +1020,7 @@
   if (ctx->queue_dev) (void)hipFree(ctx->queue_dev);
   if (ctx->spill_dev) (void)hipFree(ctx->spill_dev);
   pool_free(ctx, reinterpret_cast<char *>(ctx->entry_dev), ctx->entry_bytes);
+  pool_free(ctx, reinterpret_cast<char *>(ctx->exit_dev), ctx->exit_bytes);
   if (ctx->entry_counts_dev) (void)hipFree(ctx->entry_counts_dev);
   if (ctx->order_scratch) (void)hipFree(ctx->order_scratch);
   if (ctx->px_scratch) (void)hipFree(ctx->px_scratch);
@@ -1029,6 +1066,28 @@
   if (flags_const) *flags_const = ctx->last_entry != 0 && (ctx->last_entry & rtk::kEntryRtFlags) == 0;
   if (tables_built) *tables_built = ctx->entry_tables_built;
   if (tables_kept) *tables_kept = ctx->entry_tables_kept;
+  return 0;
+}
+
+extern "C" int rt_context_exit_info(rt_context *ctx, int32_t *active, int32_t *dmax, uint64_t *tables_built, uint64_t *tables_kept, uint64_t *lists, uint64_t *fallbacks) {
+  if (!ctx) return 1;
+  RT_LOCK(ctx);
+  const bool on = (ctx->last_entry & rtk::kEntryExit) != 0;
+  if (active) *active = on;
+  if (dmax) *dmax = rtk::kExitDmax;
+  if (tables_built) *tables_built = ctx->exit_tables_built;
+  if (tables_kept) *tables_kept = ctx->exit_tables_kept;
+  uint64_t l = 0, f = 0;
+  const int64_t nw = ctx->entry_counts_waves;
+  if (on && nw > 0 && (lists || fallbacks)) {
+    RT_HIP(ctx, hipSetDevice(ctx->device));
+    RT_HIP(ctx, hipStreamSynchronize(ctx->stream));
+    std::vector<unsigned long long> h(static_cast<size_t>(nw) * 2);
+    RT_HIP(ctx, hipMemcpy(h.data(), ctx->entry_counts_dev + 2 * nw, h.size() * sizeof(unsigned long long), hipMemcpyDeviceToHost));
+    for (int64_t i = 0; i < nw; ++i) { l += h[2 * i]; f += h[2 * i + 1]; }
+  }
+  if (lists) *lists = l;
+  if (fallbacks) *fallbacks = f;
   return 0;
 }
 
@@ -1178,6 +1237,8 @@
     ctx->leaf_box = std::max(-1, std::min(1, v));
   } else if (k == "entry_lists") {
     ctx->entry_lists = std::max(-1, std::min(1, v));
+  } else if (k == "exit_lists") {
+    ctx->exit_lists = std::max(-1, std::min(1, v));
   } else if (k == "entry_count") {
     ctx->entry_count = v != 0;
   } else if (k == "entry_keep") {
@@ -1534,6 +1595,7 @@
   RT_HIP(ctx, hipSetDevice(ctx->device));
   (void)hipGetLastError();
   reset_views(ctx, ps);
+  ps->tree_gen = next_tree_gen();
   hipError_t e = hipSuccess;
   if (int rc = build_from_device(ctx, ps, spheres7_dev, &e)) return rc;
   if (e != hipSuccess) return hip_fail(ctx, e, "rt_prepared_update_spheres");
diff --git a/raytracers_amd/csrc/lane_core.h b/raytracers_amd/csrc/lane_core.h
--- a/raytracers_amd/csrc/lane_core.h
+++ b/raytracers_amd/csrc/lane_core.h
@@ -369,4 +369,79 @@
     if (i < nl) out[2 + i] = (uint32_t)~leaf[i] << ref_shift;
 }
 
-}
+constexpr int kExitDmax = 4;
+constexpr int kExitPairs = (4 << kExitDmax) / 3 - 1;
+constexpr int kExitStack = 48;
+constexpr int exit_pair_id(int i, int prefix) { return ((4 << (2 * (i - 1))) / 3 - 1) + prefix; }
+
+template <int MUT = 0>
+RT_HD void exit_tables_path(int t, const float root_lo[3], const float root_hi[3], const float *nodes64, int n_nodes, int n_sph, float *tab, int ref_mul = kPsNodeBytes / 8) {
+  constexpr int D = kExitDmax;
+  if (n_nodes < 1) return;
+  float clo[D + 1][3], chi[D + 1][3];
+  int cidx[D + 1];
+  float srec[D + 1][8];
+  for (int a = 0; a < 3; ++a) { clo[0][a] = root_lo[a]; chi[0][a] = root_hi[a]; }
+  cidx[0] = 0;
+  int depth = 0, leaf = -1, cur = 0;
+  for (int k = 1; k <= D; ++k) {
+    if (leaf >= 0) continue;
+    const int bit = (t >> (D - k)) & 1;
+    const float *const rec = nodes64 + 16 * (size_t)cur;
+    for (int s = 0; s < 2; ++s) {
+      if (s == bit) {
+        for (int a = 0; a < 3; ++a) { clo[k][a] = rec[8 * s + a]; chi[k][a] = rec[8 * s + 4 + a]; }
+      } else {
+        for (int a = 0; a < 3; ++a) { srec[k][a] = rec[8 * s + a]; srec[k][4 + a] = rec[8 * s + 4 + a]; }
+        srec[k][3] = 0.0f;
+        srec[k][7] = rec[4 * s + 3];
+      }
+    }
+    int32_t w;
+    __builtin_memcpy(&w, rec + 4 * bit + 3, 4);
+    depth = k;
+    if ((w >> 8) < 0) leaf = ~(w >> 8);
+    else { cur = w >> 8; cidx[k] = cur; }
+  }
+  if (leaf >= 0 && (t & ((1 << (D - depth)) - 1)) != 0) return;
+  for (int i = 1; 2 * i <= depth; ++i) {
+    if ((t & ((1 << (D - 2 * i)) - 1)) != 0) continue;
+    float *const out = tab + 16 * (size_t)exit_pair_id(i, t >> (D - 2 * i));
+    const float *const a = srec[2 * i - 1], *const b = srec[2 * i];
+    out[0] = a[0]; out[1] = a[1]; out[2] = a[2]; out[3] = a[7];
+    out[4] = a[4]; out[5] = a[5]; out[6] = a[6]; out[7] = b[7];
+    out[8] = b[0]; out[9] = b[1]; out[10] = b[2]; out[11] = 0.0f;
+    out[12] = b[4]; out[13] = b[5]; out[14] = b[6]; out[15] = 0.0f;
+  }
+  const int e = leaf >= 0 ? (depth - 1) & ~1 : D;
+  if (e < 2) return;
+  bool nested = true;
+  for (int a = 0; a < 3; ++a) nested = nested & (clo[e][a] > -kNoHit) & (chi[e][a] < kNoHit);
+  for (int k = 0; k < e; ++k)
+    for (int a = 0; a < 3; ++a) nested = nested & (clo[k][a] <= clo[e][a]) & (chi[k][a] >= chi[e][a]) & (clo[k][a] > -kNoHit) & (chi[k][a] < kNoHit);
+  if (MUT != 1 && !nested) return;
+  uint32_t ref[4] = {(uint32_t)cidx[e] * (uint32_t)ref_mul, 0u, 0u, 0u};
+  for (int i = 1; 2 * i <= e; ++i) ref[i] = (uint32_t)(n_nodes + exit_pair_id(i, t >> (D - 2 * i))) * (uint32_t)ref_mul;
+  const uint32_t w0 = ref[0] | ref[1] << 16, w1 = ref[2] | ref[3] << 16;
+  auto put = [&](int j) {
+    if (j < 0 || j >= n_sph) return;
+    float *const out = tab + 16 * (size_t)kExitPairs + 8 * (size_t)j;
+    for (int a = 0; a < 3; ++a) { out[a] = clo[e][a]; out[4 + a] = chi[e][a]; }
+    __builtin_memcpy(out + 3, &w0, 4);
+    __builtin_memcpy(out + 7, &w1, 4);
+  };
+  if (leaf >= 0) { put(leaf); return; }
+  int stack[kExitStack], sp = 0;
+  stack[sp++] = cur;
+  while (sp > 0) {
+    const float *const rec = nodes64 + 16 * (size_t)stack[--sp];
+    for (int s = 0; s < 2; ++s) {
+      int32_t w;
+      __builtin_memcpy(&w, rec + 4 * s + 3, 4);
+      if ((w >> 8) < 0) put(~(w >> 8));
+      else if (sp < kExitStack) stack[sp++] = w >> 8;
+    }
+  }
+}
+
+}
diff --git a/raytracers_amd/csrc/render_kernels.hip b/raytracers_amd/csrc/render_kernels.hip
--- a/raytracers_amd/csrc/render_kernels.hip
+++ b/raytracers_amd/csrc/render_kernels.hip
@@ -487,6 +487,8 @@
   constexpr bool ECOUNT = (ENTRY & kEntryModeMask) == kEntryCount;
   constexpr bool ECONST = ENTRY != 0 && (ENTRY & kEntryRtFlags) == 0;
   constexpr bool ECOL = (ENTRY & kEntryColLds) != 0;
+  constexpr bool EXIT = (ENTRY & kEntryExit) != 0;
+  static_assert(!EXIT || (ECONST && ECOL), "EXIT: the kernel with the flags compiled in and the colours in LDS only");
   static_assert(!ENTRY || ((ENTRY & kEntryModeMask) == kEntryLists || ECOUNT), "ENTRY: lists, or the counting twin");
   static_assert(!ENTRY || (THREADS == 1024 && ALL_LDS && !STATS && !SOLO && TAIL == 0 && !ORD && !CULL && SPILL == 0 && RAYS == 0), "ENTRY: the plain 16-wave kernel of a scene in LDS only");
   static_assert(!RAYS || (!STATS && !SOLO && TAIL == 0 && !ORD && !CULL), "RAYS: the plain instantiations only");
@@ -497,7 +499,7 @@
   extern __shared__ float4 smem[];
   const int lane = threadIdx.x & 63;
   const int wave = threadIdx.x >> 6;
-  const int plane = p.lds_nodes;
+  const int plane = EXIT ? p.lds_nodes + kExitPairs : p.lds_nodes;
   const int sph_base = ECOL ? (plane * (kPsNodeBytes / 4) + 3) >> 2 : 4 * plane;
   const int per_wave_dw = pooled_wave_dw(p.ray_planes, p.capb, p.capl);
   const int col_base = sph_base + p.lds_sph;
@@ -515,7 +517,9 @@
   if constexpr (PRESORT) {
     auto ref_of = [](float w) { const int c = f2i(w) >> 8; return (unsigned)(c < 0 ? c : c * kPsNodeBytes) << kPsItemShift; };
     for (int i = threadIdx.x; i < plane; i += THREADS) {
-      const float4 ll = p.nodes64[4 * i], lh = p.nodes64[4 * i + 1], rl = p.nodes64[4 * i + 2], rh = p.nodes64[4 * i + 3];
+      const float4 *src = p.nodes64 + 4 * i;
+      if constexpr (EXIT) src = i < p.lds_nodes ? src : p.exit_tab + 4 * (i - p.lds_nodes);
+      const float4 ll = src[0], lh = src[1], rl = src[2], rh = src[3];
       presort_pack(reinterpret_cast<unsigned *>(smem) + (kPsNodeBytes / 4) * i, &ll.x, &lh.x, &rl.x, &rh.x, ref_of(ll.w), ref_of(lh.w));
     }
   } else {
@@ -537,6 +541,7 @@
   unsigned long long n_rays = 0, n_box = 0, n_sph = 0;
   int nbox = 0, nleaf = 0;
   unsigned ec_lists = 0u, ec_fall = 0u;
+  unsigned ex_lists = 0u, ex_fall = 0u;
   static_assert(!SPILL || (THREADS == 256 && !ALL_LDS && !SOLO && TAIL == 0 && !ORD), "SPILL: the plain and CULL kernels of the four-wave workgroups");
   unsigned *const wspill = wbase + 193;
   auto spill_region = [&]() { return p.spill + (size_t)(blockIdx.x * (THREADS / 64) + wave) * (size_t)p.spill_stride; };
@@ -683,6 +688,7 @@
           if (ns == 0) break;
           RT_MARK("SHADE_BEGIN");
           bool root = false;
+          uint4 ent0 = make_uint4(0u, 0u, 0u, 0u), ent1 = ent0;
           if (STATS) tr_ops[2]++;
           const unsigned long long tr_s0 = STATS ? clock64() : 0ull;
           if constexpr (ANY) {
@@ -733,6 +739,11 @@
             }
             if (more) {
               root = true;
+              if constexpr (EXIT) {
+                const uint4 *const xp = reinterpret_cast<const uint4 *>(p.exit_tab + 4 * kExitPairs) + 2 * wj;
+                ent0 = xp[0];
+                ent1 = xp[1];
+              }
             } else if constexpr (RAYS) {
               pix = -1;
             } else {
@@ -746,7 +757,6 @@
           }
           bool want = (pix < 0) & !exhausted & !hold;
           int slot = -1;
-          uint4 ent0 = make_uint4(0u, 0u, 0u, 0u), ent1 = ent0;
           float a_lo = p.ray_tlo, a_hi = p.ray_thi;
           unsigned long long m = bal(want);
           while (ORD && m != 0ull) {
@@ -946,8 +956,38 @@
             }
           }
           if (root) ray_derive(r);
-          const bool root_hit = root && (ANY ? interval_ok(a_lo, a_hi) && box_hit_interval(r, p.root_lo[0], p.root_lo[1], p.root_lo[2], p.root_hi[0], p.root_hi[1], p.root_hi[2], a_lo, a_hi)
-                                             : box_hit(r, p.root_lo[0], p.root_lo[1], p.root_lo[2], p.root_hi[0], p.root_hi[1], p.root_hi[2]));
+          bool root_hit;
+          bool xl = false;
+          int xnp = 0;
+          if constexpr (!EXIT) {
+            root_hit = root && (ANY ? interval_ok(a_lo, a_hi) && box_hit_interval(r, p.root_lo[0], p.root_lo[1], p.root_lo[2], p.root_hi[0], p.root_hi[1], p.root_hi[2], a_lo, a_hi)
+                                    : box_hit(r, p.root_lo[0], p.root_lo[1], p.root_lo[2], p.root_hi[0], p.root_hi[1], p.root_hi[2]));
+          } else {
+            xl = root & (slot < 0) & ((ent0.w & 0xffffu) != 0u);
+            float blx = p.root_lo[0], bly = p.root_lo[1], blz = p.root_lo[2], bhx = p.root_hi[0], bhy = p.root_hi[1], bhz = p.root_hi[2];
+            if (xl) {
+              blx = __uint_as_float(ent0.x); bly = __uint_as_float(ent0.y); blz = __uint_as_float(ent0.z);
+              bhx = __uint_as_float(ent1.x); bhy = __uint_as_float(ent1.y); bhz = __uint_as_float(ent1.z);
+            }
+            root_hit = root && box_hit(r, blx, bly, blz, bhx, bhy, bhz);
+            const unsigned long long m_x = bal(xl);
+            if (m_x != 0ull) {
+              xnp = xl ? ((ent0.w >> 16) != 0u) + ((ent1.w & 0xffffu) != 0u) + ((ent1.w >> 16) != 0u) : 0;
+              bool back = xl & !root_hit;
+              int added = __popcll(bal(root_hit));
+              for (int k = 0; k < kExitDmax / 2; ++k) added += __popcll(bal(root_hit & (xnp > k)));
+              if (__builtin_expect(uni(nbox + added) > p.exit_room, 0)) back = xl;
+              if (__builtin_expect(bal(back) != 0ull, 0)) {
+                if (back) {
+                  root_hit = box_hit(r, p.root_lo[0], p.root_lo[1], p.root_lo[2], p.root_hi[0], p.root_hi[1], p.root_hi[2]);
+                  xl = false;
+                }
+                if constexpr (ECOUNT) ex_fall += (unsigned)__popcll(bal(back));
+              }
+              xnp = xl ? xnp : 0;
+              if constexpr (ECOUNT) ex_lists += (unsigned)__popcll(bal(xl));
+            }
+          }
           unsigned ent_hdr = 0u;
           bool push_box = root_hit;
           if constexpr (ENTRY) {
@@ -966,7 +1006,8 @@
           }
           if (root) {
             wkey[lane] = ANY ? any_key_seed(a_hi) : kKeyInit;
-            wcnt[lane] = push_box ? 1 : 0;
+            if constexpr (EXIT) wcnt[lane] = push_box ? 1 + xnp : 0;
+            else wcnt[lane] = push_box ? 1 : 0;
             wray[lane] = make_float4(r.ox, r.oy, r.oz, r.a);
             wray[64 + lane] = make_float4(r.ix, r.iy, r.iz, CULL ? cull_weight(r, p.cull_c2) : ANY ? a_lo : 0.0f);
             if (p.ray_planes == 3) wray[128 + lane] = make_float4(r.dx, r.dy, r.dz, 0.0f);
@@ -978,8 +1019,21 @@
             nbox = uni(nbox + __popcll(m_root));
           } else {
             const unsigned low = (unsigned)lane << 2 | (PRESORT ? sign_offsets(r) << 5 : 0u);
-            if (push_box) wbox[nbox + lane_rank(m_root)] = ((ent_hdr & kEntryValid) != 0u ? ent0.y : 0u) | low;
+            if constexpr (!EXIT) {
+              if (push_box) wbox[nbox + lane_rank(m_root)] = ((ent_hdr & kEntryValid) != 0u ? ent0.y : 0u) | low;
+            } else {
+              if (push_box) wbox[nbox + lane_rank(m_root)] = (xl ? (ent0.w & 0xffffu) << (kPsItemShift + 3) : (ent_hdr & kEntryValid) != 0u ? ent0.y : 0u) | low;
+            }
             nbox = uni(nbox + __popcll(m_root));
+            if constexpr (EXIT) {
+              const unsigned pr[3] = {ent0.w >> 16, ent1.w & 0xffffu, ent1.w >> 16};
+              for (int k = 0; k < kExitDmax / 2; ++k) {
+                const unsigned long long m_k = bal(xnp > k);
+                if (m_k == 0ull) break;
+                if (xnp > k) wbox[nbox + lane_rank(m_k)] = pr[k] << (kPsItemShift + 3) | low;
+                nbox = uni(nbox + __popcll(m_k));
+              }
+            }
             const unsigned lf[kEntryLeaves] = {ent0.z, ent0.w, ent1.x, ent1.y, ent1.z, ent1.w};
             const int nl = (ent_hdr & kEntryValid) != 0u ? (int)(ent_hdr >> kEntryCountShift) & 15 : 0;
             for (int k = 0; k < kEntryLeaves; ++k) {
@@ -1293,6 +1347,10 @@
     if (lane == 0 && p.trace != nullptr) {
       unsigned long long *const rec = p.trace + 2 * (size_t)(blockIdx.x * (THREADS / 64) + wave);
       rec[0] = ec_lists; rec[1] = ec_fall;
+      if constexpr (EXIT) {
+        unsigned long long *const rex = p.trace + 2 * (size_t)nwaves + 2 * (size_t)(blockIdx.x * (THREADS / 64) + wave);
+        rex[0] = ex_lists; rex[1] = ex_fall;
+      }
     }
   }
   if (STATS) {
@@ -1690,7 +1748,7 @@
 
 template <int ENTRY>
 static hipError_t launch_pooled_entry_t(const KParams &p, int grid, hipStream_t stream) {
-  const size_t lds = (ENTRY & kEntryColLds) ? pooled_col_lds_bytes(p.n_nodes, p.n_sph, p.capb, p.capl, p.ray_planes)
+  const size_t lds = (ENTRY & kEntryColLds) ? pooled_col_lds_bytes(p.n_nodes + ((ENTRY & kEntryExit) ? kExitPairs : 0), p.n_sph, p.capb, p.capl, p.ray_planes)
                                             : pooled_lds_bytes(p.lds_nodes, p.lds_sph, p.capb, p.capl, p.ray_planes, 16);
   auto kfn = pooled_kernel<1024, true, false, false, 0, false, false, 0, 0, ENTRY>;
   if (hipError_t e = allow_full_lds(reinterpret_cast<const void *>(kfn)); e != hipSuccess) return e;
@@ -1709,9 +1767,12 @@
     return hipErrorInvalidValue;
   if (!(entry & kEntryRtFlags) && !pooled_entry_flags_const(p.leaf_box, p.dark)) return hipErrorInvalidValue;
   if ((entry & kEntryColLds) && !pooled_col_fits(pooled_col_lds_bytes(p.n_nodes, p.n_sph, p.capb, p.capl, p.ray_planes), 160 * 1024)) return hipErrorInvalidValue;
+  if ((entry & kEntryExit) && ((entry & (kEntryColLds | kEntryRtFlags)) != kEntryColLds || p.exit_tab == nullptr || p.lds_nodes != p.n_nodes ||
+                               !pooled_exit_fits(p.n_nodes, p.n_sph, p.capb, p.capl, p.ray_planes, 160 * 1024)))
+    return hipErrorInvalidValue;
   return launch_pooled_entry_any(p, grid, stream, entry,
                                  std::integer_sequence<int, kEntryLists, kEntryLists | kEntryColLds, kEntryLists | kEntryRtFlags, kEntryCount, kEntryCount | kEntryColLds,
-                                                       kEntryCount | kEntryRtFlags>{});
+                                                       kEntryCount | kEntryRtFlags, kEntryLists | kEntryColLds | kEntryExit, kEntryCount | kEntryColLds | kEntryExit>{});
 }
 
 __global__ __launch_bounds__(256) void tile_entry_kernel(KParams p, int ref_shift, int node_mul, int filter) {
@@ -1743,6 +1804,18 @@
   return hipGetLastError();
 }
 
+__global__ __launch_bounds__(64) void exit_tables_kernel(KParams p, float4 *tab) {
+  const int t = (int)threadIdx.x;
+  if (t >= (1 << kExitDmax)) return;
+  exit_tables_path<0>(t, p.root_lo, p.root_hi, reinterpret_cast<const float *>(p.nodes64), p.n_nodes, p.n_sph, reinterpret_cast<float *>(tab));
+}
+hipError_t launch_exit_tables(const KParams &p, float4 *tab, hipStream_t stream) {
+  if (tab == nullptr || p.n_nodes < 1) return hipErrorInvalidValue;
+  if (hipError_t e = hipMemsetAsync(tab, 0, exit_tab_bytes(p.n_sph), stream); e != hipSuccess) return e;
+  hipLaunchKernelGGL(exit_tables_kernel, dim3(1), dim3(64), 0, stream, p, tab);
+  return hipGetLastError();
+}
+
 hipError_t launch_pooled(const KParams &p, bool stats, int grid, int waves_per_wg, hipStream_t stream, int rays, int entry) {
   if (rays == kRaysAny && p.occluded == nullptr) return hipErrorInvalidValue;
   if ((p.ray_tlo_dev != nullptr || p.ray_thi_dev != nullptr) && (rays != kRaysAny || p.ray_tlo_dev == nullptr || p.ray_thi_dev == nullptr)) return hipErrorInvalidValue;
diff --git a/raytracers_amd/csrc/rt_device.hpp b/raytracers_amd/csrc/rt_device.hpp
--- a/raytracers_amd/csrc/rt_device.hpp
+++ b/raytracers_amd/csrc/rt_device.hpp
@@ -218,8 +218,14 @@
     float *colour3;
     const unsigned *entry;
   };
-  int nrays;
-  unsigned char *occluded;
+  union {
+    int nrays;
+    int exit_room;
+  };
+  union {
+    unsigned char *occluded;
+    const float4 *exit_tab;
+  };
   float ray_tlo, ray_thi;
   const float *ray_tlo_dev, *ray_thi_dev;
 };
@@ -346,6 +352,13 @@
 size_t persistent_lds_bytes(int lds_nodes, int lds_sph, int smax, int lmax, int waves_per_wg);
 constexpr int kEntryLists = 1, kEntryCount = 2;
 constexpr int kEntryModeMask = 3, kEntryColLds = 4, kEntryRtFlags = 8;
+constexpr int kEntryExit = 16;
+constexpr int kExitItems = 1 + kExitDmax / 2;
+constexpr bool pooled_exit_fits(int n_nodes, int n_sph, int capb, int capl, int ray_planes, size_t lds_limit) {
+  return n_nodes >= 1 && (size_t)(n_nodes + kExitPairs) * (kPsNodeBytes / 8) < 65536u &&
+         (((size_t)(n_nodes + kExitPairs) * kPsNodeBytes + 15) & ~(size_t)15) + (size_t)n_sph * 32 + (size_t)16 * pooled_wave_dw(ray_planes, capb, capl) * sizeof(unsigned) <= lds_limit;
+}
+constexpr size_t exit_tab_bytes(int n_sph) { return (size_t)kExitPairs * 64 + (size_t)n_sph * 32; }
 constexpr bool pooled_entry_flags_const(int leaf_box, int dark) { return leaf_box != 0 && dark != 0; }
 constexpr size_t pooled_col_lds_bytes(int n_nodes, int n_sph, int capb, int capl, int ray_planes) {
   return (((size_t)n_nodes * kPsNodeBytes + 15) & ~(size_t)15) + (size_t)n_sph * 32 + (size_t)16 * pooled_wave_dw(ray_planes, capb, capl) * sizeof(unsigned);
@@ -356,6 +369,7 @@
 }
 hipError_t launch_pooled(const KParams &p, bool stats, int grid, int waves_per_wg, hipStream_t stream, int rays = 0, int entry = 0);
 hipError_t launch_tile_entry(const KParams &p, bool stats, int waves_per_wg, hipStream_t stream);
+hipError_t launch_exit_tables(const KParams &p, float4 *tab, hipStream_t stream);
 size_t pooled_lds_bytes(int lds_nodes, int lds_sph, int capb, int capl, int ray_planes, int waves_per_wg);
 struct GpuBvhOut {
   float *L7;
diff --git a/raytracers_amd/csrc/rt_internal.hpp b/raytracers_amd/csrc/rt_internal.hpp
--- a/raytracers_amd/csrc/rt_internal.hpp
+++ b/raytracers_amd/csrc/rt_internal.hpp
@@ -1,4 +1,5 @@
 #pragma once
+#include <atomic>
 #include <hip/hip_runtime.h>
 
 #include <cstdint>
@@ -79,6 +80,11 @@
   int col_lds = -1;
   uint64_t entry_tables_built = 0, entry_tables_kept = 0;
   int last_entry = 0;
+  int exit_lists = -1;
+  float4 *exit_dev = nullptr;
+  size_t exit_bytes = 0;
+  uint64_t exit_gen = 0;
+  uint64_t exit_tables_built = 0, exit_tables_kept = 0;
   bool entry_count = false;
   unsigned long long *entry_counts_dev = nullptr;
   size_t entry_counts_bytes = 0;
@@ -169,7 +175,13 @@
 constexpr int kClassSlotInts = 16, kClassSlots = 8;
 constexpr int kClassChunks = 64;
 
+inline uint64_t next_tree_gen() {
+  static std::atomic<uint64_t> g{0};
+  return ++g;
+}
+
 struct rt_prepared {
+  uint64_t tree_gen = next_tree_gen();
   rt_context *home = nullptr;
   mutable std::recursive_mutex mu;
   mutable std::vector<TileOrder> orders;
```

New measurement: 23670 (median of 6 runs). 1.04x the previous value.
